# jamie8johnson/cqs

Measured on AMD Instinct MI355X. Metric: queries/sec @k=20 (brute-force cosine scan + top-k, 768-d fp32), higher is better.
Workload: dtype f32; 1 GPU; BASELINE configs[1]: 1000000 x 768 fp32 unit vectors, 1 query per step, brute-force cosine top-20; mode=single, rows_per_gpu=1000000, total_rows=1000000, dim=768, k=20, parallelism=single GPU, ranks_seen=1

## Files before the change

### cqs_amd/csrc/index.hip

```cpp
#include <hip/hip_runtime.h>

#include <algorithm>
#include <atomic>
#include <cmath>
#include <cerrno>
#include <chrono>
#include <cstdio>
#include <cstdlib>
#include <cstring>
#include <mutex>
#include <new>
#include <string>
#include <thread>
#include <vector>

#include <fcntl.h>
#include <libgen.h>
#include <sys/stat.h>
#include <unistd.h>

#include "abi_guard.h"
#include "roctx.h"
#include "index_internal.h"
#include "persist_util.h"
#include "scan_bf16.h"
#include "scan_i8.h"

using cqs::kMaxK;
using cqs::kRowsPerBlock;

namespace cqs_idx {

uint64_t pad_rows(uint64_t n) { return (n + kRowsPerBlock - 1) / kRowsPerBlock * kRowsPerBlock; }

int32_t fail(cqs_hip_index* idx, int32_t code, const char* what, hipError_t e) {
    char buf[512];
    if (e != hipSuccess)
        snprintf(buf, sizeof buf, "%s: %s (%s)", what, hipGetErrorString(e), hipGetErrorName(e));
    else
        snprintf(buf, sizeof buf, "%s", what);
    if (idx) {
        idx->last_error = buf;
        if (code == CQS_HIP_ERR_DEVICE) idx->poisoned.store(true, std::memory_order_release);
    }
    return code;
}

void free_scratch(cqs_hip_index* x) {
    hipFree(x->d_q); hipFree(x->d_scores); hipFree(x->d_gmax); hipFree(x->d_work); hipFree(x->d_gaux);
    x->d_work = nullptr; x->d_gaux = nullptr;
    hipFree(x->d_out_keys); hipFree(x->d_out_counts);
    hipHostFree(x->h_q); hipHostFree(x->h_out_keys); hipHostFree(x->h_out_counts);
    x->d_q = x->d_scores = nullptr; x->d_gmax = nullptr;
    x->d_out_keys = nullptr; x->d_out_counts = nullptr;
    x->h_q = nullptr; x->h_out_keys = nullptr; x->h_out_counts = nullptr;
    x->h_out_keys_dev = nullptr; x->h_out_counts_dev = nullptr;
    x->q_cap = 0; x->k_cap = 0; x->scr_n_pad = 0;
}

int32_t ensure_scratch(cqs_hip_index* x, uint32_t b, uint32_t k) {
    const uint64_t n_pad = pad_rows(x->n);
    if (b <= x->q_cap && k <= x->k_cap && n_pad == x->scr_n_pad) return CQS_HIP_OK;
    HIP_TRY(x, hipDeviceSynchronize());
    uint32_t qc = x->q_cap > b ? x->q_cap : b;
    uint32_t kc = x->k_cap > k ? x->k_cap : k;
    free_scratch(x);
    HIP_TRY(x, hipMalloc(&x->d_q, ((size_t)qc + 256) * x->dim * sizeof(float)));
    HIP_TRY(x, hipMalloc(&x->d_scores, (size_t)qc * n_pad * sizeof(float)));
    HIP_TRY(x, hipMalloc(&x->d_work, cqs::kWorkWords * sizeof(uint32_t)));
    HIP_TRY(x, hipMemset(x->d_work, 0, cqs::kWorkWords * sizeof(uint32_t)));
    HIP_TRY(x, hipMalloc(&x->d_gmax, (size_t)qc * (n_pad / cqs::kTaskRowsSmall) * sizeof(float)));
    HIP_TRY(x, hipMalloc(&x->d_gaux, (size_t)(qc < kGauxQueries ? qc : kGauxQueries) * (n_pad / cqs::kTaskRowsSmall) * sizeof(uint64_t)));
    HIP_TRY(x, hipMalloc(&x->d_out_keys, (size_t)qc * kc * sizeof(uint64_t)));
    HIP_TRY(x, hipMalloc(&x->d_out_counts, (size_t)qc * sizeof(uint32_t)));
    HIP_TRY(x, hipHostMalloc(&x->h_q, (size_t)qc * x->dim * sizeof(float), hipHostMallocDefault));
    HIP_TRY(x, hipHostMalloc(&x->h_out_keys, (size_t)qc * kc * sizeof(uint64_t), hipHostMallocDefault));
    HIP_TRY(x, hipHostMalloc(&x->h_out_counts, (size_t)qc * sizeof(uint32_t), hipHostMallocDefault));
    if (hipHostGetDevicePointer((void**)&x->h_out_keys_dev, x->h_out_keys, 0) != hipSuccess ||
        hipHostGetDevicePointer((void**)&x->h_out_counts_dev, x->h_out_counts, 0) != hipSuccess) {
        (void)hipGetLastError();
        x->h_out_keys_dev = nullptr; x->h_out_counts_dev = nullptr;
    }
    x->q_cap = qc; x->k_cap = kc; x->scr_n_pad = n_pad;
    return CQS_HIP_OK;
}

uint32_t max_query_block(const cqs_hip_index* x) {
    const uint64_t budget = 16ull << 30;
    const uint64_t per_q = pad_rows(x->n) * sizeof(float);
    uint64_t q = per_q ? budget / per_q : 1024;
    if (q < 1) q = 1;
    if (q > 1024) q = 1024;
    return (uint32_t)q;
}

cqs::ScanArgs scan_args(const cqs_hip_index* x, const float* d_q, uint32_t b, uint32_t k, const uint32_t* d_keep,
                        uint32_t mode, float thr, size_t elem_bytes, bool gemv_only, void* dbg, const uint32_t* gate) {
    cqs::ScanArgs a;
    a.rows = x->d_rows;
    a.n = (uint32_t)x->n;
    a.n_pad = (uint32_t)pad_rows(x->n);
    a.dim = x->dim;
    a.q = d_q;
    a.b = b;
    a.scores = x->d_scores;
    a.keep = d_keep;
    a.mode = mode;
    a.threshold = thr;
    a.nontemporal = x->n * x->dim * elem_bytes > kNtBytes;
    a.linear_bins = (x->metric == CQS_HIP_METRIC_COSINE) || (mode == CQS_HIP_MODE_PIPELINE);
    a.k = k;
    a.gmax = x->d_gmax;
    a.gaux = (b <= kGauxQueries && k >= kGauxMinK) ? x->d_gaux : nullptr;
    a.work = x->d_work;
    a.n_cu = x->n_cu;
    a.dbg = dbg;
    a.gemv_only = gemv_only;
    a.tiers = cqs::plan_tiers(a.n_pad, x->n_cu, !gemv_only && cqs::uniform_groups(b, x->dim));
    a.gate = gate;
    return a;
}

int32_t scan_select(cqs_hip_index* x, const cqs::ScanArgs& a, hipStream_t st, const ShadowRows* shadow,
                    uint64_t* out_keys, uint32_t* out_counts) {
    const bool timed = !a.gate && x->timing && x->ev_used + 2 <= kMaxTimingEvents;
    if (timed) {
        while (x->ev.size() < x->ev_used + 2) {
            hipEvent_t e = nullptr;
            HIP_TRY(x, hipEventCreate(&e));
            x->ev.push_back(e);
        }
        HIP_TRY(x, hipEventRecord(x->ev[x->ev_used], st));
    }
    if (shadow && shadow->bf16) HIP_TRY(x, cqs::launch_scan_bf16(a, shadow->bf16, shadow->bq, st));
    else if (shadow) HIP_TRY(x, cqs::launch_scan_i8(a, shadow->i8, shadow->i8_scale, shadow->bq, st));
    else HIP_TRY(x, cqs::launch_scan(a, st));
    if (timed) {
        HIP_TRY(x, hipEventRecord(x->ev[x->ev_used + 1], st));
        x->ev_used += 2;
    }
    if (out_keys) HIP_TRY(x, cqs::launch_select(a, (uint32_t)x->row_base, out_keys, out_counts, st));
    return CQS_HIP_OK;
}

int32_t enqueue_search(cqs_hip_index* x, const float* d_q, uint32_t b, uint32_t k, const uint32_t* d_keep,
                       uint32_t mode, float thr, uint64_t* d_out_keys, uint32_t* d_out_counts, hipStream_t st, bool gemv_only,
                       const uint32_t* gate) {
    HIP_TRY(x, order_after_last(x, st));
    if (!gemv_only && cqs::use_mfma(b, x->dim)) {
        const size_t qbytes = (size_t)b * x->dim * sizeof(float);
        if (d_q != x->d_q) HIP_TRY(x, hipMemcpyAsync(x->d_q, d_q, qbytes, hipMemcpyDeviceToDevice, st));
        HIP_TRY(x, hipMemsetAsync((char*)x->d_q + qbytes, 0, (size_t)256 * x->dim * sizeof(float), st));
        d_q = x->d_q;
    }
    cqs::ScanArgs a = scan_args(x, d_q, b, k, d_keep, mode, thr, sizeof(float), gemv_only, x->d_dbg, gate);
    static const bool use_gaux = [] { const char* e = getenv("CQS_HIP_SELECT_AUX"); return !(e && e[0] == '0'); }();
    if (!use_gaux) a.gaux = nullptr;
    const int32_t rc = scan_select(x, a, st, nullptr, d_out_keys, d_out_counts);
    if (rc == CQS_HIP_OK) HIP_TRY(x, record_done(x, st));
    return rc;
}

hipError_t quiesce(cqs_hip_index* x) {
    hipError_t e = x->stream ? hipStreamSynchronize(x->stream) : hipSuccess;
    if (e == hipSuccess && x->done_valid) e = hipEventSynchronize(x->done);
    return e;
}

int32_t stage_keep(cqs_hip_index* x, const uint32_t* host_words, uint64_t words) {
    if (words > x->keep_words_cap) {
        HIP_TRY(x, quiesce(x));
        hipFree(x->d_keep);
        x->d_keep = nullptr;
        x->keep_words_cap = 0;
        HIP_TRY(x, hipMalloc(&x->d_keep, words * sizeof(uint32_t)));
        x->keep_words_cap = words;
    }
    HIP_TRY(x, hipMemcpyAsync(x->d_keep, host_words, words * sizeof(uint32_t), hipMemcpyHostToDevice, x->stream));
    return CQS_HIP_OK;
}

void read_combine_env(cqs_hip_index* x) {
    if (const char* ce = getenv("CQS_HIP_COMBINE")) x->combine = ce[0] != '0';
    if (const char* cw = getenv("CQS_HIP_COMBINE_WAIT_US")) x->combine_wait_us = (uint32_t)atoi(cw);
    if (const char* cb = getenv("CQS_HIP_COMBINE_BITS")) x->combine_relaxed = cb[0] == 'r';
}

int32_t create_common(uint64_t n, uint32_t dim, uint32_t metric, int32_t device, uint64_t row_base,
                      cqs_hip_index** out, cqs_hip_index** made) {
    if (!out) return CQS_HIP_ERR_INVALID;
    *out = nullptr;
    if (!cqs::scan_dim_supported(dim) || metric > CQS_HIP_METRIC_DOT) return CQS_HIP_ERR_INVALID;
    if (n + row_base > 0xFFFFFFFEull) return CQS_HIP_ERR_INVALID;
    int cnt = 0;
    if (hipGetDeviceCount(&cnt) != hipSuccess || cnt <= 0) return CQS_HIP_ERR_NO_DEVICE;
    if (device < 0 || device >= cnt) return CQS_HIP_ERR_INVALID;
    cqs_hip_index* x = new (std::nothrow) cqs_hip_index();
    if (!x) return CQS_HIP_ERR_NOMEM;
    x->device = device; x->n = n; x->dim = dim; x->metric = metric; x->row_base = row_base;
    if (hipSetDevice(device) != hipSuccess || hipStreamCreateWithFlags(&x->stream, hipStreamNonBlocking) != hipSuccess ||
        hipEventCreateWithFlags(&x->done, hipEventDisableTiming) != hipSuccess) {
        if (x->stream) hipStreamDestroy(x->stream);
        delete x;
        return CQS_HIP_ERR_DEVICE;
    }
    read_combine_env(x);
    if (getenv("CQS_HIP_DEBUG_STAMPS")) {
        const size_t bytes = (16 + 2 * cqs::kDbgWaves) * sizeof(unsigned long long);
        if (hipMalloc(&x->d_dbg, bytes) == hipSuccess) (void)hipMemset(x->d_dbg, 0, bytes);
    }
    hipDeviceProp_t prop;
    if (hipGetDeviceProperties(&prop, device) == hipSuccess && prop.multiProcessorCount > 0)
        x->n_cu = (uint32_t)prop.multiProcessorCount;
    *made = x;
    return CQS_HIP_OK;
}

}

using namespace cqs_idx;

extern "C" {

const char* cqs_hip_version(void) CQS_ABI_TRY { return "cqs-hip 0.1.0 (gfx950)"; } CQS_ABI_CATCH_VAL("cqs-hip")

int32_t cqs_hip_device_count(void) CQS_ABI_TRY {
    int cnt = 0;
    if (hipGetDeviceCount(&cnt) != hipSuccess) return 0;
    return cnt;
} CQS_ABI_CATCH_NOHANDLE

int32_t cqs_hip_device_mem(int32_t device, uint64_t* free_bytes, uint64_t* total_bytes) CQS_ABI_TRY {
    if (hipSetDevice(device) != hipSuccess) return CQS_HIP_ERR_NO_DEVICE;
    size_t f = 0, t = 0;
    if (hipMemGetInfo(&f, &t) != hipSuccess) return CQS_HIP_ERR_DEVICE;
    if (free_bytes) *free_bytes = f;
    if (total_bytes) *total_bytes = t;
    return CQS_HIP_OK;
} CQS_ABI_CATCH_NOHANDLE

}

int32_t cqs_idx::create_owned(const float* rows, uint64_t n, uint32_t dim, uint32_t metric, int32_t device,
                              uint64_t row_base, cqs_hip_index** out) {
    if (n > 0 && !rows) return CQS_HIP_ERR_INVALID;
    cqs_hip_index* x = nullptr;
    int32_t rc = create_common(n, dim, metric, device, row_base, out, &x);
    if (rc != CQS_HIP_OK) return rc;
    x->cap_rows = n ? n : 1;
    hipError_t e = hipMalloc(&x->d_rows, (size_t)x->cap_rows * dim * sizeof(float));
    if (e == hipSuccess && n)
        e = hipMemcpyAsync(x->d_rows, rows, (size_t)n * dim * sizeof(float), hipMemcpyHostToDevice, x->stream);
    if (e == hipSuccess) e = hipStreamSynchronize(x->stream);
    if (e != hipSuccess) {
        cqs_hip_index_destroy(x);
        return e == hipErrorOutOfMemory ? CQS_HIP_ERR_NOMEM : CQS_HIP_ERR_DEVICE;
    }
    *out = x;
    return CQS_HIP_OK;
}

extern "C" {

int32_t cqs_hip_index_create(const float* rows, uint64_t n, uint32_t dim, uint32_t metric, int32_t device,
                             uint64_t row_base, cqs_hip_index** out) CQS_ABI_TRY {
    cqs_hip_index* x = nullptr;
    int32_t rc = create_owned(rows, n, dim, metric, device, row_base, &x);
    if (rc != CQS_HIP_OK) return rc;
    if ((rc = shadow_auto(x)) != CQS_HIP_OK) { cqs_hip_index_destroy(x); return rc; }
    *out = x;
    return CQS_HIP_OK;
} CQS_ABI_CATCH_NOHANDLE

int32_t cqs_hip_index_create_device(const void* d_rows, uint64_t n, uint32_t dim, uint32_t metric, int32_t device,
                                    uint64_t row_base, int32_t borrow, cqs_hip_index** out) CQS_ABI_TRY {
    if (n > 0 && !d_rows) return CQS_HIP_ERR_INVALID;
    if (((uintptr_t)d_rows & 15u) != 0) return CQS_HIP_ERR_INVALID;
    cqs_hip_index* x = nullptr;
    int32_t rc = create_common(n, dim, metric, device, row_base, out, &x);
    if (rc != CQS_HIP_OK) return rc;
    if (n && hipDeviceSynchronize() != hipSuccess) { cqs_hip_index_destroy(x); return CQS_HIP_ERR_DEVICE; }
    if (borrow) {
        x->borrow = true;
        x->d_rows = (float*)d_rows;
        x->cap_rows = n;
    } else {
        x->cap_rows = n ? n : 1;
        hipError_t e = hipMalloc(&x->d_rows, (size_t)x->cap_rows * dim * sizeof(float));
        if (e == hipSuccess && n)
            e = hipMemcpyAsync(x->d_rows, d_rows, (size_t)n * dim * sizeof(float), hipMemcpyDeviceToDevice, x->stream);
        if (e == hipSuccess) e = hipStreamSynchronize(x->stream);
        if (e != hipSuccess) {
            cqs_hip_index_destroy(x);
            return e == hipErrorOutOfMemory ? CQS_HIP_ERR_NOMEM : CQS_HIP_ERR_DEVICE;
        }
    }
    if ((rc = shadow_auto(x)) != CQS_HIP_OK) { cqs_hip_index_destroy(x); return rc; }
    *out = x;
    return CQS_HIP_OK;
} CQS_ABI_CATCH_NOHANDLE

int32_t cqs_hip_index_extend(cqs_hip_index* x, const float* rows, uint64_t n_new) CQS_ABI_TRY {
    if (!x) return CQS_HIP_ERR_INVALID;
    if (x->sh) return cqs_sharded::extend(x, rows, n_new);
    std::lock_guard<std::mutex> g(x->mu);
    if (x->poisoned.load(std::memory_order_acquire)) return CQS_HIP_ERR_POISONED;
    if (x->borrow) return fail(x, CQS_HIP_ERR_INVALID, "extend: index borrows its rows");
    if (n_new == 0) return CQS_HIP_OK;
    if (!rows) return fail(x, CQS_HIP_ERR_INVALID, "extend: null rows");
    if (x->n + n_new + x->row_base > 0xFFFFFFFEull) return fail(x, CQS_HIP_ERR_INVALID, "extend: row id overflow");
    HIP_TRY(x, hipSetDevice(x->device));
    HIP_TRY(x, quiesce(x));
    const size_t row_bytes = (size_t)x->dim * sizeof(float);
    if (x->n + n_new > x->cap_rows) {
        uint64_t cap = x->cap_rows * 2;
        if (cap < x->n + n_new) cap = x->n + n_new;
        float* nd = nullptr;
        HIP_TRY(x, hipMalloc(&nd, cap * row_bytes));
        hipError_t e = hipMemcpyAsync(nd, x->d_rows, x->n * row_bytes, hipMemcpyDeviceToDevice, x->stream);
        if (e == hipSuccess) e = hipStreamSynchronize(x->stream);
        if (e != hipSuccess) {
            hipFree(nd);
            return fail(x, CQS_HIP_ERR_DEVICE, "extend: copy", e);
        }
        hipFree(x->d_rows);
        x->d_rows = nd;
        x->cap_rows = cap;
    }
    HIP_TRY(x, hipMemcpyAsync(x->d_rows + x->n * x->dim, rows, n_new * row_bytes, hipMemcpyHostToDevice, x->stream));
    HIP_TRY(x, hipStreamSynchronize(x->stream));
    const uint64_t n_old = x->n;
    x->n += n_new;
    return shadow_extend(x, n_old);
} CQS_ABI_CATCH(x)

}

namespace {
using cqs_persist::Checksum;
using cqs_persist::exists;
using cqs_persist::fsync_parent;
using cqs_persist::read_all;
using cqs_persist::write_all;

struct FlatHeader {
    char magic[8];
    uint32_t version, dim, metric, pad;
    uint64_t rows, checksum;
    uint8_t reserved[24];
};
static_assert(sizeof(FlatHeader) == 64, "header is 64 bytes");
const char kFlatMagic[8] = {'C', 'Q', 'S', 'H', 'I', 'P', 'F', '1'};

constexpr size_t kIoPiece = 64ull << 20;

struct Piece { const cqs_idx::Segment* seg; size_t off, len; };
std::vector<Piece> cut_pieces(const std::vector<cqs_idx::Segment>& segs, uint32_t dim) {
    std::vector<Piece> out;
    for (const cqs_idx::Segment& sg : segs) {
        const size_t bytes = (size_t)sg.rows * dim * sizeof(float);
        for (size_t off = 0; off < bytes; off += kIoPiece) out.push_back({&sg, off, bytes - off < kIoPiece ? bytes - off : kIoPiece});
    }
    return out;
}
struct PinPair {
    uint8_t* p[2] = {nullptr, nullptr};
    hipError_t alloc(size_t bytes) {
        for (int i = 0; i < 2; ++i) {
            hipError_t e = hipHostMalloc((void**)&p[i], bytes ? bytes : 8, hipHostMallocPortable);
            if (e != hipSuccess) return e;
        }
        return hipSuccess;
    }
    ~PinPair() { if (p[0]) hipHostFree(p[0]); if (p[1]) hipHostFree(p[1]); }
};
}

namespace cqs_idx {

int32_t save_segments(cqs_hip_index* x, const std::vector<Segment>& segs, uint32_t dim, uint32_t metric, const char* path,
                      uint64_t* out_checksum) {
    const std::string live(path), bak = live + ".bak", tmp = live + ".tmp";
    if (exists(bak)) return fail(x, CQS_HIP_ERR_INVALID, "save: stale .bak from a prior failed save; manual recovery required");
    uint64_t rows = 0;
    for (const Segment& sg : segs) rows += sg.rows;
    const size_t bytes = (size_t)rows * dim * sizeof(float);
    const std::vector<Piece> pieces = cut_pieces(segs, dim);
    PinPair pin;
    hipError_t he = pin.alloc(bytes < kIoPiece ? bytes : kIoPiece);
    if (he != hipSuccess) return fail(x, CQS_HIP_ERR_NOMEM, "save: pinned staging", he);
    const int fd = open(tmp.c_str(), O_WRONLY | O_CREAT | O_TRUNC, 0644);
    if (fd < 0) return fail(x, CQS_HIP_ERR_INVALID, "save: cannot create temp file");
    FlatHeader h{};
    memcpy(h.magic, kFlatMagic, 8);
    h.version = 1; h.dim = dim; h.metric = metric; h.rows = rows;
    bool ok = write_all(fd, &h, sizeof h);
    Checksum ck(bytes);
    auto issue = [&](size_t i) -> hipError_t {
        const Piece& pc = pieces[i];
        hipError_t e = hipSetDevice(pc.seg->device);
        if (e != hipSuccess) return e;
        return hipMemcpyAsync(pin.p[i & 1], (const uint8_t*)pc.seg->d_rows + pc.off, pc.len, hipMemcpyDeviceToHost, pc.seg->stream);
    };
    if (ok && !pieces.empty()) he = issue(0);
    for (size_t i = 0; ok && he == hipSuccess && i < pieces.size(); ++i) {
        he = hipStreamSynchronize(pieces[i].seg->stream);
        if (he != hipSuccess) break;
        if (i + 1 < pieces.size() && (he = issue(i + 1)) != hipSuccess) break;
        ck.update(pin.p[i & 1], pieces[i].len, i + 1 == pieces.size());
        ok = write_all(fd, pin.p[i & 1], pieces[i].len);
    }
    if (pieces.empty()) ck.update(nullptr, 0, true);
    for (const Segment& sg : segs) (void)hipStreamSynchronize(sg.stream);
    h.checksum = ck.finish();
    ok = ok && he == hipSuccess && lseek(fd, 0, SEEK_SET) == 0 && write_all(fd, &h, sizeof h) && fsync(fd) == 0;
    close(fd);
    if (!ok) {
        unlink(tmp.c_str());
        return he != hipSuccess ? fail(x, CQS_HIP_ERR_DEVICE, "save: device copy", he) : fail(x, CQS_HIP_ERR_INVALID, "save: write failed");
    }
    const bool backed_up = exists(live);
    if (backed_up) {
        if (rename(live.c_str(), bak.c_str()) != 0) { unlink(tmp.c_str()); return fail(x, CQS_HIP_ERR_INVALID, "save: cannot back up the live blob"); }
        fsync_parent(live);
    }
    if (rename(tmp.c_str(), live.c_str()) != 0) {
        unlink(tmp.c_str());
        if (backed_up) {
            if (rename(bak.c_str(), live.c_str()) != 0) return fail(x, CQS_HIP_ERR_INVALID, "save failed and rollback failed: rename .bak back by hand");
            fsync_parent(live);
        }
        return fail(x, CQS_HIP_ERR_INVALID, "save: rename failed");
    }
    if (backed_up) unlink(bak.c_str());
    fsync_parent(live);
    if (out_checksum) *out_checksum = h.checksum;
    return CQS_HIP_OK;
}

int32_t open_blob(const char* path, uint32_t expected_dim, uint64_t expected_rows, int* fd_out, uint64_t* rows,
                  uint32_t* metric, uint64_t* checksum) {
    const int fd = open(path, O_RDONLY);
    if (fd < 0) return CQS_HIP_ERR_INVALID;
    FlatHeader h{};
    struct stat st;
    const bool ok = read_all(fd, &h, sizeof h) && memcmp(h.magic, kFlatMagic, 8) == 0 && h.version == 1 &&
                    h.dim == expected_dim && (expected_rows == 0 || h.rows == expected_rows) && h.metric <= CQS_HIP_METRIC_DOT &&
                    fstat(fd, &st) == 0 && h.dim != 0 && h.rows <= (UINT64_MAX - sizeof h) / ((uint64_t)h.dim * 4u) &&
                    (uint64_t)st.st_size == sizeof h + h.rows * h.dim * 4u;
    if (!ok) { close(fd); return CQS_HIP_ERR_INVALID; }
    *fd_out = fd; *rows = h.rows; *metric = h.metric; *checksum = h.checksum;
    return CQS_HIP_OK;
}

int32_t read_blob_into(int fd, uint64_t checksum, uint32_t dim, const std::vector<Segment>& segs) {
    uint64_t rows = 0;
    for (const Segment& sg : segs) rows += sg.rows;
    const size_t bytes = (size_t)rows * dim * sizeof(float);
    const std::vector<Piece> pieces = cut_pieces(segs, dim);
    PinPair pin;
    hipError_t he = pin.alloc(bytes < kIoPiece ? bytes : kIoPiece);
    Checksum ck(bytes);
    bool ok = true;
    for (size_t i = 0; ok && he == hipSuccess && i < pieces.size(); ++i) {
        const Piece& pc = pieces[i];
        if (i >= 2) he = hipStreamSynchronize(pieces[i - 2].seg->stream);
        if (he != hipSuccess) break;
        ok = read_all(fd, pin.p[i & 1], pc.len);
        if (!ok) break;
        ck.update(pin.p[i & 1], pc.len, i + 1 == pieces.size());
        he = hipSetDevice(pc.seg->device);
        if (he == hipSuccess) he = hipMemcpyAsync((uint8_t*)pc.seg->d_rows + pc.off, pin.p[i & 1], pc.len, hipMemcpyHostToDevice, pc.seg->stream);
    }
    if (pieces.empty()) ck.update(nullptr, 0, true);
    for (const Segment& sg : segs) {
        const hipError_t hs = hipStreamSynchronize(sg.stream);
        if (he == hipSuccess) he = hs;
    }
    close(fd);
    if (he != hipSuccess) return he == hipErrorOutOfMemory ? CQS_HIP_ERR_NOMEM : CQS_HIP_ERR_DEVICE;
    return ok && ck.finish() == checksum ? CQS_HIP_OK : CQS_HIP_ERR_INVALID;
}

}

extern "C" {

int32_t cqs_hip_index_save(cqs_hip_index* x, const char* path, uint64_t* out_checksum) CQS_ABI_TRY {
    if (!x || !path) return CQS_HIP_ERR_INVALID;
    if (x->sh) return cqs_sharded::save(x, path, out_checksum);
    std::lock_guard<std::mutex> g(x->mu);
    if (x->poisoned.load(std::memory_order_acquire)) return CQS_HIP_ERR_POISONED;
    HIP_TRY(x, hipSetDevice(x->device));
    HIP_TRY(x, quiesce(x));
    return save_segments(x, {Segment{x->device, x->d_rows, x->n, x->stream}}, x->dim, x->metric, path, out_checksum);
} CQS_ABI_CATCH(x)

int32_t cqs_hip_index_load(const char* path, uint32_t expected_dim, uint64_t expected_rows, int32_t device,
                           uint64_t row_base, cqs_hip_index** out) CQS_ABI_TRY {
    if (!path || !out) return CQS_HIP_ERR_INVALID;
    *out = nullptr;
    int fd = -1;
    uint64_t rows = 0, checksum = 0;
    uint32_t metric = 0;
    int32_t rc = open_blob(path, expected_dim, expected_rows, &fd, &rows, &metric, &checksum);
    if (rc != CQS_HIP_OK) return rc;
    cqs_hip_index* x = nullptr;
    rc = create_common(rows, expected_dim, metric, device, row_base, out, &x);
    if (rc != CQS_HIP_OK) { close(fd); return rc; }
    x->cap_rows = rows ? rows : 1;
    if (hipMalloc(&x->d_rows, (size_t)x->cap_rows * expected_dim * sizeof(float)) != hipSuccess) {
        close(fd);
        cqs_hip_index_destroy(x);
        return CQS_HIP_ERR_NOMEM;
    }
    rc = read_blob_into(fd, checksum, expected_dim, {Segment{device, x->d_rows, rows, x->stream}});
    if (rc == CQS_HIP_OK) rc = shadow_auto(x);
    if (rc != CQS_HIP_OK) { cqs_hip_index_destroy(x); return rc; }
    *out = x;
    return CQS_HIP_OK;
} CQS_ABI_CATCH_NOHANDLE

void cqs_hip_index_destroy(cqs_hip_index* x) CQS_ABI_TRY {
    if (!x) return;
    if (x->sh) { cqs_sharded::destroy(x); return; }
    hipSetDevice(x->device);
    (void)quiesce(x);
    free_scratch(x);
    shadow_free(x);
    hipFree(x->d_keep);
    hipFree(x->d_dbg);
    if (!x->borrow) hipFree(x->d_rows);
    for (hipEvent_t e : x->ev) hipEventDestroy(e);
    if (x->done) hipEventDestroy(x->done);
    if (x->stream) hipStreamDestroy(x->stream);
    delete x;
} CQS_ABI_CATCH_VOID

uint64_t cqs_hip_index_len(const cqs_hip_index* x) CQS_ABI_TRY { return x ? (x->sh ? cqs_sharded::len(x) : x->n) : 0; } CQS_ABI_CATCH_VAL(0)
uint32_t cqs_hip_index_dim(const cqs_hip_index* x) CQS_ABI_TRY { return x ? x->dim : 0; } CQS_ABI_CATCH_VAL(0)
uint32_t cqs_hip_index_metric(const cqs_hip_index* x) CQS_ABI_TRY { return x ? x->metric : 0; } CQS_ABI_CATCH_VAL(0)
uint32_t cqs_hip_index_max_k(const cqs_hip_index* x) CQS_ABI_TRY { (void)x; return kMaxK; } CQS_ABI_CATCH_VAL(0)
int32_t cqs_hip_index_poisoned(const cqs_hip_index* x) CQS_ABI_TRY {
    if (x && x->sh) return cqs_sharded::poisoned(x);
    return x && x->poisoned.load(std::memory_order_acquire) ? 1 : 0;
} CQS_ABI_CATCH_NOHANDLE
int32_t cqs_hip_index_device(const cqs_hip_index* x) CQS_ABI_TRY { return x ? x->device : -1; } CQS_ABI_CATCH_NOHANDLE
uint64_t cqs_hip_index_row_base(const cqs_hip_index* x) CQS_ABI_TRY { return x ? x->row_base : 0; } CQS_ABI_CATCH_VAL(0)

size_t cqs_hip_index_last_error(const cqs_hip_index* x, char* buf, size_t cap) CQS_ABI_TRY {
    if (!x || !buf || cap == 0) return 0;
    if (x->sh) return cqs_sharded::last_error(x, buf, cap);
    std::lock_guard<std::mutex> g(x->mu);
    size_t m = x->last_error.size() < cap - 1 ? x->last_error.size() : cap - 1;
    memcpy(buf, x->last_error.data(), m);
    buf[m] = 0;
    return m;
} CQS_ABI_CATCH_VAL(0)

void cqs_hip_unpack_keys(const uint64_t* keys, size_t count, uint64_t* rows, float* scores) CQS_ABI_TRY {
    for (size_t i = 0; i < count; ++i) {
        const uint32_t ok = (uint32_t)(keys[i] >> 32);
        const uint32_t bits = (ok & 0x80000000u) ? (ok ^ 0x80000000u) : ~ok;
        float f;
        memcpy(&f, &bits, 4);
        if (scores) scores[i] = f;
        if (rows) rows[i] = (uint64_t)(0xFFFFFFFFu - (uint32_t)keys[i]);
    }
} CQS_ABI_CATCH_VOID

size_t cqs_hip_merge_keys(const uint64_t* lists, const uint32_t* counts, size_t n_lists, size_t stride, size_t k,
                          uint64_t* out_keys) CQS_ABI_TRY {
    std::vector<size_t> pos(n_lists, 0);
    size_t outc = 0;
    while (outc < k) {
        size_t best = n_lists;
        uint64_t bk = 0;
        for (size_t l = 0; l < n_lists; ++l) {
            if (pos[l] < counts[l]) {
                const uint64_t v = lists[l * stride + pos[l]];
                if (best == n_lists || v > bk) { best = l; bk = v; }
            }
        }
        if (best == n_lists) break;
        out_keys[outc++] = bk;
        pos[best]++;
    }
    return outc;
} CQS_ABI_CATCH_VAL(0)

int32_t cqs_hip_index_search_device(cqs_hip_index* x, const float* d_queries, uint32_t b, uint32_t k,
                                    const uint32_t* d_keep_bitset, uint32_t mode, float threshold,
                                    uint64_t* d_out_keys, uint32_t* d_out_counts, void* stream) CQS_ABI_TRY {
    CQS_ROCTX_RANGE("cqs_hip_index_search_device");
    if (!x) return CQS_HIP_ERR_INVALID;
    if (x->sh) return CQS_HIP_ERR_INVALID;
    std::lock_guard<std::mutex> g(x->mu);
    if (x->poisoned.load(std::memory_order_acquire)) return CQS_HIP_ERR_POISONED;
    if (b == 0) return CQS_HIP_OK;
    if (!d_queries || !d_out_keys || !d_out_counts) return fail(x, CQS_HIP_ERR_INVALID, "search_device: null buffer");
    if (k == 0 || k > kMaxK) return fail(x, CQS_HIP_ERR_INVALID, "search_device: k out of range");
    if (mode > CQS_HIP_MODE_PIPELINE) return fail(x, CQS_HIP_ERR_INVALID, "search_device: bad mode");
    if (b > max_query_block(x)) return fail(x, CQS_HIP_ERR_INVALID, "search_device: batch exceeds scratch budget");
    HIP_TRY(x, hipSetDevice(x->device));
    hipStream_t st = (hipStream_t)stream;
    if (x->n == 0) {
        HIP_TRY(x, hipMemsetAsync(d_out_counts, 0, (size_t)b * sizeof(uint32_t), st));
        return CQS_HIP_OK;
    }
    int32_t rc = ensure_scratch(x, b, k);
    if (rc != CQS_HIP_OK) return rc;
    const uint32_t* gate = nullptr;
    if (shadow_takes(x, b, k, false) &&
        (rc = shadow_pass(x, d_queries, b, k, d_keep_bitset, mode, threshold, d_out_keys, d_out_counts, st, &gate)) != CQS_HIP_OK)
        return rc;
    return enqueue_search(x, d_queries, b, k, d_keep_bitset, mode, threshold, d_out_keys, d_out_counts, st, false, gate);
} CQS_ABI_CATCH(x)

}

namespace cqs_idx {

static void print_debug_stamps(cqs_hip_index* x) {
    unsigned long long h[16];
    if (hipMemcpy(h, x->d_dbg, sizeof h, hipMemcpyDeviceToHost) == hipSuccess)
        fprintf(stderr, "[cqs_hip] select_finish us: zero %.2f hist %.2f decide %.2f groups %.2f scores %.2f sort %.2f emit %.2f | groups=%llu cand=%llu\n",
                0.0, (h[1] - h[0]) / 100.0, (h[2] - h[1]) / 100.0, (h[3] - h[2]) / 100.0, (h[4] - h[3]) / 100.0,
                (h[5] - h[4]) / 100.0, (h[6] - h[5]) / 100.0, h[8], h[9]);
    std::vector<unsigned long long> w(2 * cqs::kDbgWaves);
    if (hipMemcpy(w.data(), x->d_dbg + 16, w.size() * sizeof(unsigned long long), hipMemcpyDeviceToHost) != hipSuccess) return;
    std::vector<double> st, en;
    unsigned long long t0 = ~0ull;
    for (uint32_t i = 0; i < cqs::kDbgWaves; ++i) if (w[2 * i] && w[2 * i] < t0) t0 = w[2 * i];
    for (uint32_t i = 0; i < cqs::kDbgWaves; ++i)
        if (w[2 * i] && w[2 * i + 1]) { st.push_back((w[2 * i] - t0) / 100.0); en.push_back((w[2 * i + 1] - t0) / 100.0); }
    if (!st.empty()) {
        std::sort(st.begin(), st.end());
        std::sort(en.begin(), en.end());
        auto pc = [](const std::vector<double>& v, double f) { return v[(size_t)(f * (v.size() - 1))]; };
        fprintf(stderr, "[cqs_hip] scan waves=%zu start us p0 %.1f p50 %.1f p90 %.1f p100 %.1f | end us p0 %.1f p10 %.1f p50 %.1f p90 %.1f p100 %.1f | select ends %.1f\n",
                st.size(), pc(st, 0), pc(st, .5), pc(st, .9), pc(st, 1), pc(en, 0), pc(en, .1), pc(en, .5), pc(en, .9), pc(en, 1),
                (h[6] - t0) / 100.0);
    }
    (void)hipMemset(x->d_dbg + 16, 0, w.size() * sizeof(unsigned long long));
}

static int32_t host_block(cqs_hip_index* x, const cqs_combine_req* const* qs, uint32_t nq, uint32_t k, const uint32_t* d_keep,
                          uint32_t mode, float thr, bool gemv_only, std::vector<const cqs_combine_req*>* redo) {
    HIP_TRY(x, hipMemcpyAsync(x->d_q, x->h_q, (size_t)nq * x->dim * sizeof(float), hipMemcpyHostToDevice, x->stream));
    const bool direct = x->h_out_keys_dev && x->h_out_counts_dev && (size_t)nq * k <= kDirectOutKeys;
    uint64_t* const keys = direct ? x->h_out_keys_dev : x->d_out_keys;
    uint32_t* const counts = direct ? x->h_out_counts_dev : x->d_out_counts;
    int32_t rc = redo ? shadow_pass(x, x->d_q, nq, k, d_keep, mode, thr, keys, counts, x->stream, nullptr)
                      : enqueue_search(x, x->d_q, nq, k, d_keep, mode, thr, keys, counts, x->stream, gemv_only);
    if (rc != CQS_HIP_OK) return rc;
    if (redo) HIP_TRY(x, record_done(x, x->stream));
    if (!direct) {
        HIP_TRY(x, hipMemcpyAsync(x->h_out_keys, x->d_out_keys, (size_t)nq * k * sizeof(uint64_t), hipMemcpyDeviceToHost, x->stream));
        HIP_TRY(x, hipMemcpyAsync(x->h_out_counts, x->d_out_counts, (size_t)nq * sizeof(uint32_t), hipMemcpyDeviceToHost, x->stream));
    }
    const uint32_t* cert = nullptr;
    if (redo) HIP_TRY(x, shadow_verdicts(x, nq, &cert));
    HIP_TRY(x, hipStreamSynchronize(x->stream));
    if (!redo && x->d_dbg) print_debug_stamps(x);
    if (redo) redo->clear();
    uint64_t certified = 0;
    for (uint32_t i = 0; i < nq; ++i) {
        if (!qs[i]) continue;
        if (cert && !cert[i]) {
            if (redo->size() != i) memcpy(x->h_q + redo->size() * x->dim, x->h_q + (size_t)i * x->dim, (size_t)x->dim * sizeof(float));
            redo->push_back(qs[i]);
            continue;
        }
        const uint32_t c = x->h_out_counts[i] < k ? x->h_out_counts[i] : k;
        cqs_hip_unpack_keys(x->h_out_keys + (size_t)i * k, c, qs[i]->out_rows, qs[i]->out_scores);
        *qs[i]->out_count = c;
        certified += cert ? 1 : 0;
    }
    x->stat_certified.fetch_add(certified, std::memory_order_relaxed);
    if (redo) x->stat_fallbacks.fetch_add(redo->size(), std::memory_order_relaxed);
    if (redo && shadow_uses_i8(x, nq, k)) {
        x->stat_i8_certified.fetch_add(certified, std::memory_order_relaxed);
        x->stat_i8_fallbacks.fetch_add(redo->size(), std::memory_order_relaxed);
    }
    return CQS_HIP_OK;
}

static int32_t search_host_locked(cqs_hip_index* x, const cqs_combine_req* qs, uint32_t b, uint32_t k, const uint32_t* keep_bitset,
                                  uint32_t mode, float threshold, bool gemv_only) {
    if (x->inject_fail.exchange(0, std::memory_order_acq_rel) != 0)
        return fail(x, CQS_HIP_ERR_DEVICE, "search: injected device failure (test hook)");
    if (x->n == 0 || k == 0) return CQS_HIP_OK;
    HIP_TRY(x, hipSetDevice(x->device));
    HIP_TRY(x, order_after_last(x, x->stream));
    const uint32_t* d_keep = nullptr;
    uint32_t k_eff = k;
    if (keep_bitset) {
        const uint64_t words = (x->n + 31) / 32;
        uint64_t included = 0;
        for (uint64_t w = 0; w < words; ++w) {
            uint32_t v = keep_bitset[w];
            if (w == words - 1 && (x->n % 32)) v &= (1u << (x->n % 32)) - 1u;
            included += (uint64_t)__builtin_popcount(v);
        }
        if (included == 0) return CQS_HIP_OK;
        if (included < x->n) {
            if (included < k_eff) k_eff = (uint32_t)included;
            int32_t rck = stage_keep(x, keep_bitset, words);
            if (rck != CQS_HIP_OK) return rck;
            d_keep = x->d_keep;
        }
    }

    const uint32_t blk = max_query_block(x);
    std::vector<const cqs_combine_req*> staged, redo;
    for (uint32_t done = 0; done < b;) {
        const uint32_t nb = (b - done) < blk ? (b - done) : blk;
        int32_t rc = ensure_scratch(x, nb, k_eff);
        if (rc != CQS_HIP_OK) return rc;
        staged.clear();
        for (uint32_t i = 0; i < nb; ++i) {
            const float* src = qs[done + i].q;
            float* dst = x->h_q + (size_t)i * x->dim;
            bool ok = true;
            for (uint32_t d = 0; d < x->dim; ++d) ok &= std::isfinite(src[d]);
            if (ok) memcpy(dst, src, (size_t)x->dim * sizeof(float));
            else memset(dst, 0, (size_t)x->dim * sizeof(float));
            staged.push_back(ok ? &qs[done + i] : nullptr);
        }
        if (shadow_takes(x, nb, k_eff, gemv_only)) {
            if ((rc = host_block(x, staged.data(), nb, k_eff, d_keep, mode, threshold, gemv_only, &redo)) != CQS_HIP_OK) return rc;
            staged.swap(redo);
        }
        if (!staged.empty() &&
            (rc = host_block(x, staged.data(), (uint32_t)staged.size(), k_eff, d_keep, mode, threshold, gemv_only, nullptr)) != CQS_HIP_OK)
            return rc;
        done += nb;
    }
    return CQS_HIP_OK;
}

constexpr uint32_t kCombineCap = 32;

static bool same_params(const cqs_combine_req* a, const cqs_combine_req* b) {
    return a->k == b->k && a->mode == b->mode && memcmp(&a->thr, &b->thr, sizeof(float)) == 0;
}
static uint32_t count_like_front(const cqs_hip_index* x) {
    uint32_t n = 0;
    for (const cqs_combine_req* r : x->pending) n += same_params(r, x->pending.front()) ? 1u : 0u;
    return n;
}

static int32_t combine_run_single(cqs_hip_index* x, cqs_combine_req* const* batch, uint32_t nb) {
    std::lock_guard<std::mutex> dev(x->mu);
    if (x->poisoned.load(std::memory_order_acquire)) return CQS_HIP_ERR_POISONED;
    cqs_combine_req rq[kCombineCap];
    for (uint32_t i = 0; i < nb; ++i) rq[i] = *batch[i];
    const bool gemv_only = !(x->combine_relaxed && nb >= cqs::kMfmaMinQueries);
    return search_host_locked(x, rq, nb, batch[0]->k, nullptr, batch[0]->mode, batch[0]->thr, gemv_only);
}

static void combine_lead(cqs_hip_index* x, std::unique_lock<std::mutex>& lk) {
    const uint32_t target = x->expect < kCombineCap ? x->expect : kCombineCap;
    if (x->combine_wait_us && count_like_front(x) < target) {
        const auto t_end = x->last_pass_end + std::chrono::microseconds(x->combine_wait_us);
        while (count_like_front(x) < target && std::chrono::steady_clock::now() < t_end) {
            lk.unlock();
            for (int i = 0; i < 64; ++i) __builtin_ia32_pause();
            lk.lock();
        }
    }
    cqs_combine_req* batch[kCombineCap];
    uint32_t nb = 0, left_like = 0;
    {
        const cqs_combine_req head = *x->pending.front();
        std::deque<cqs_combine_req*> keep;
        for (cqs_combine_req* r : x->pending) {
            if (same_params(r, &head)) {
                if (nb < kCombineCap) { batch[nb++] = r; continue; }
                ++left_like;
            }
            keep.push_back(r);
        }
        x->pending.swap(keep);
        x->n_pending.store((uint32_t)x->pending.size(), std::memory_order_relaxed);
    }
    x->expect = nb + left_like;
    lk.unlock();

    int32_t rc = CQS_HIP_OK;
    try {
        rc = x->sh ? cqs_sharded::search_combined(x, batch, nb) : combine_run_single(x, batch, nb);
    } catch (const std::bad_alloc&) {
        rc = fail(x, CQS_HIP_ERR_NOMEM, "search: out of host memory");
    } catch (...) {
        rc = fail(x, CQS_HIP_ERR_INVALID, "search: unexpected C++ exception");
    }
    x->stat_passes.fetch_add(1, std::memory_order_relaxed);
    x->stat_queries.fetch_add(nb, std::memory_order_relaxed);
    const bool poisoned = x->sh ? cqs_sharded::poisoned(x) != 0 : x->poisoned.load(std::memory_order_acquire);

    lk.lock();
    x->last_pass_end = std::chrono::steady_clock::now();
    for (uint32_t i = 0; i < nb; ++i) {
        batch[i]->rc = (rc != CQS_HIP_OK && i > 0 && poisoned) ? CQS_HIP_ERR_POISONED : rc;
        batch[i]->done = true;
    }
    if (poisoned) {
        for (cqs_combine_req* r : x->pending) { r->rc = CQS_HIP_ERR_POISONED; r->done = true; }
        x->pending.clear();
        x->n_pending.store(0, std::memory_order_relaxed);
    } else if (!x->pending.empty()) {
        uint32_t like = 0;
        for (const cqs_combine_req* r : x->pending) like += same_params(r, batch[0]) ? 1u : 0u;
        if (nb + like > x->expect) x->expect = nb + like;
    }
}

static int32_t combine_search(cqs_hip_index* x, cqs_combine_req& r) {
    std::unique_lock<std::mutex> lk(x->cmu);
    x->pending.push_back(&r);
    x->n_pending.store((uint32_t)x->pending.size(), std::memory_order_relaxed);
    while (!r.done) {
        if (!x->leader) {
            x->leader = true;
            struct Reset {
                cqs_hip_index* x; std::unique_lock<std::mutex>& lk;
                ~Reset() { if (!lk.owns_lock()) lk.lock(); x->leader = false; x->ccv.notify_all(); }
            } reset{x, lk};
            combine_lead(x, lk);
        } else {
            x->ccv.wait(lk);
        }
    }
    return r.rc;
}

}

extern "C" {

int32_t cqs_hip_index_search(cqs_hip_index* x, const float* queries, uint32_t b, uint32_t query_dim, uint32_t k,
                             const uint32_t* keep_bitset, uint32_t mode, float threshold, uint64_t* out_rows,
                             float* out_scores, uint32_t* out_counts) CQS_ABI_TRY {
    CQS_ROCTX_RANGE("cqs_hip_index_search");
    if (!x) return CQS_HIP_ERR_INVALID;
    if (x->combine && b == 1 && !keep_bitset && queries && out_counts && out_rows && out_scores && query_dim == x->dim &&
        k >= 1 && k <= kMaxK && mode <= CQS_HIP_MODE_PIPELINE) {
        if (x->sh ? cqs_sharded::poisoned(x) != 0 : x->poisoned.load(std::memory_order_acquire))
            return CQS_HIP_ERR_POISONED;
        out_counts[0] = 0;
        bool finite = true;
        for (uint32_t d = 0; d < query_dim; ++d) finite &= std::isfinite(queries[d]);
        if (!finite) return CQS_HIP_OK;
        cqs_combine_req r{queries, k, mode, threshold, out_rows, out_scores, out_counts};
        return combine_search(x, r);
    }
    if (x->sh) return cqs_sharded::search(x, queries, b, query_dim, k, keep_bitset, mode, threshold, out_rows, out_scores, out_counts);
    std::lock_guard<std::mutex> g(x->mu);
    if (x->poisoned.load(std::memory_order_acquire)) return CQS_HIP_ERR_POISONED;
    if (b == 0) return CQS_HIP_OK;
    if (!queries || !out_counts) return fail(x, CQS_HIP_ERR_INVALID, "search: null buffer");
    for (uint32_t i = 0; i < b; ++i) out_counts[i] = 0;
    if (x->n == 0 || k == 0) return CQS_HIP_OK;
    if (query_dim != x->dim) {
        x->last_error = "search: query dimension mismatch (empty result)";
        return CQS_HIP_OK;
    }
    if (k > kMaxK) return fail(x, CQS_HIP_ERR_INVALID, "search: k > max_k");
    if (mode > CQS_HIP_MODE_PIPELINE) return fail(x, CQS_HIP_ERR_INVALID, "search: bad mode");
    if (!out_rows || !out_scores) return fail(x, CQS_HIP_ERR_INVALID, "search: null output buffer");
    std::vector<cqs_combine_req> rq(b);
    for (uint32_t i = 0; i < b; ++i)
        rq[i] = cqs_combine_req{queries + (size_t)i * x->dim, k, mode, threshold, out_rows + (size_t)i * k, out_scores + (size_t)i * k, out_counts + i};
    return search_host_locked(x, rq.data(), b, k, keep_bitset, mode, threshold, false);
} CQS_ABI_CATCH(x)

void cqs_hip_index_combine_stats(const cqs_hip_index* x, uint64_t* passes, uint64_t* queries) CQS_ABI_TRY {
    if (passes) *passes = x ? x->stat_passes.load(std::memory_order_relaxed) : 0;
    if (queries) *queries = x ? x->stat_queries.load(std::memory_order_relaxed) : 0;
} CQS_ABI_CATCH_VOID

int32_t cqs_hip_index_neighbors(cqs_hip_index* x, uint64_t target_row, uint32_t limit, uint64_t* out_rows,
                                float* out_scores, uint32_t* out_count) CQS_ABI_TRY {
    CQS_ROCTX_RANGE("cqs_hip_index_neighbors");
    if (!x || !out_count) return CQS_HIP_ERR_INVALID;
    if (x->sh) return cqs_sharded::neighbors(x, target_row, limit, out_rows, out_scores, out_count);
    std::lock_guard<std::mutex> g(x->mu);
    *out_count = 0;
    if (x->poisoned.load(std::memory_order_acquire)) return CQS_HIP_ERR_POISONED;
    if (!out_rows || !out_scores) return fail(x, CQS_HIP_ERR_INVALID, "neighbors: null output buffer");
    if (target_row < x->row_base || target_row - x->row_base >= x->n)
        return fail(x, CQS_HIP_ERR_INVALID, "neighbors: target row not in this index");
    if (limit < 1u) limit = 1u;
    if (limit > CQS_HIP_NEIGHBORS_MAX) limit = CQS_HIP_NEIGHBORS_MAX;
    if (x->n <= 1) return CQS_HIP_OK;
    const uint32_t k = (uint64_t)limit + 1u < x->n ? limit + 1u : (uint32_t)x->n;
    HIP_TRY(x, hipSetDevice(x->device));
    HIP_TRY(x, order_after_last(x, x->stream));
    int32_t rc = ensure_scratch(x, 1, k);
    if (rc != CQS_HIP_OK) return rc;
    const float* d_target = x->d_rows + (size_t)(target_row - x->row_base) * x->dim;
    rc = enqueue_search(x, d_target, 1, k, nullptr, CQS_HIP_MODE_RAW, 0.f, x->d_out_keys, x->d_out_counts, x->stream);
    if (rc != CQS_HIP_OK) return rc;
    HIP_TRY(x, hipMemcpyAsync(x->h_out_keys, x->d_out_keys, (size_t)k * sizeof(uint64_t), hipMemcpyDeviceToHost, x->stream));
    HIP_TRY(x, hipMemcpyAsync(x->h_out_counts, x->d_out_counts, sizeof(uint32_t), hipMemcpyDeviceToHost, x->stream));
    HIP_TRY(x, hipStreamSynchronize(x->stream));
    uint32_t c = x->h_out_counts[0] < k ? x->h_out_counts[0] : k, outc = 0;
    for (uint32_t i = 0; i < c && outc < limit; ++i) {
        uint64_t row;
        float score;
        cqs_hip_unpack_keys(x->h_out_keys + i, 1, &row, &score);
        if (row == target_row) continue;
        out_rows[outc] = row;
        out_scores[outc] = score;
        ++outc;
    }
    *out_count = outc;
    return CQS_HIP_OK;
} CQS_ABI_CATCH(x)

void cqs_hip_index_set_timing(cqs_hip_index* x, int32_t enable) CQS_ABI_TRY {
    if (!x) return;
    if (x->sh) { cqs_sharded::set_timing(x, enable); return; }
    std::lock_guard<std::mutex> g(x->mu);
    x->timing = enable != 0;
    x->ev_used = 0;
} CQS_ABI_CATCH_VOID

int32_t cqs_hip_index_scan_time(cqs_hip_index* x, uint32_t* launches, double* total_ms) CQS_ABI_TRY {
    if (!x || !launches || !total_ms) return CQS_HIP_ERR_INVALID;
    if (x->sh) return cqs_sharded::scan_time(x, launches, total_ms);
    std::lock_guard<std::mutex> g(x->mu);
    *launches = 0;
    *total_ms = 0.0;
    HIP_TRY(x, hipSetDevice(x->device));
    for (size_t i = 0; i + 1 < x->ev_used; i += 2) {
        HIP_TRY(x, hipEventSynchronize(x->ev[i + 1]));
        float ms = 0.f;
        HIP_TRY(x, hipEventElapsedTime(&ms, x->ev[i], x->ev[i + 1]));
        *total_ms += ms;
        *launches += 1;
    }
    x->ev_used = 0;
    return CQS_HIP_OK;
} CQS_ABI_CATCH(x)


void cqs_hip_debug_index_fail_next(cqs_hip_index* x) CQS_ABI_TRY {
    if (x) x->inject_fail.store(1, std::memory_order_release);
} CQS_ABI_CATCH_VOID

double cqs_hip_debug_client_storm(cqs_hip_index* x, const float* queries, uint32_t n_queries, uint32_t dim, uint32_t k,
                                  uint32_t n_threads, uint32_t per_thread, uint64_t* out_rows, float* out_scores,
                                  uint32_t* out_counts) CQS_ABI_TRY {
    if (!x || !queries || !n_queries || !n_threads || !out_rows || !out_scores || !out_counts) return -1.0;
    std::atomic<int32_t> bad{0};
    std::atomic<uint32_t> ready{0};
    std::atomic<bool> go{false};
    std::vector<std::thread> th;
    th.reserve(n_threads);
    for (uint32_t t = 0; t < n_threads; ++t)
        th.emplace_back([&, t]() {
            ready.fetch_add(1);
            while (!go.load(std::memory_order_acquire)) std::this_thread::yield();
            uint32_t qi = t % n_queries;
            for (uint32_t i = 0; i < per_thread; ++i) {
                const int32_t rc = cqs_hip_index_search(x, queries + (size_t)qi * dim, 1, dim, k, nullptr, CQS_HIP_MODE_RAW, 0.f,
                                                        out_rows + (size_t)qi * k, out_scores + (size_t)qi * k, out_counts + qi);
                if (rc != CQS_HIP_OK) { bad.store(rc); break; }
                qi = (qi + n_threads) % n_queries;
            }
        });
    while (ready.load() < n_threads) std::this_thread::yield();
    const auto t0 = std::chrono::steady_clock::now();
    go.store(true, std::memory_order_release);
    for (std::thread& t : th) t.join();
    const double el = std::chrono::duration<double>(std::chrono::steady_clock::now() - t0).count();
    return bad.load() ? -1.0 : el;
} CQS_ABI_CATCH_VAL(-1.0)

}
```

### cqs_amd/csrc/index_internal.h

```cpp
#pragma once
#include <hip/hip_runtime.h>

#include <atomic>
#include <chrono>
#include <condition_variable>
#include <deque>
#include <mutex>
#include <string>
#include <vector>

#include "../../include/cqs_hip.h"
#include "scan_kernels.h"

namespace cqs_sharded { struct ShardSet; }
namespace cqs_idx { struct Shadow; }

struct cqs_combine_req {
    const float* q;
    uint32_t k, mode;
    float thr;
    uint64_t* out_rows;
    float* out_scores;
    uint32_t* out_count;
    int32_t rc = 0;
    bool done = false;
};

struct cqs_hip_index {
    int device = 0;
    uint64_t n = 0;
    uint64_t cap_rows = 0;
    uint32_t dim = 0;
    uint32_t metric = 0;
    uint64_t row_base = 0;
    bool borrow = false;
    float* d_rows = nullptr;
    hipStream_t stream = nullptr;

    uint32_t q_cap = 0;
    uint64_t scr_n_pad = 0;
    uint32_t k_cap = 0;
    float* d_q = nullptr;
    float* d_scores = nullptr;
    uint32_t* d_work = nullptr;
    unsigned long long* d_dbg = nullptr;
    uint32_t n_cu = 256;
    float* d_gmax = nullptr;
    uint64_t* d_gaux = nullptr;
    uint64_t* d_out_keys = nullptr;
    uint32_t* d_out_counts = nullptr;
    uint32_t* d_keep = nullptr;
    uint64_t keep_words_cap = 0;
    float* h_q = nullptr;
    uint64_t* h_out_keys = nullptr;
    uint32_t* h_out_counts = nullptr;
    uint64_t* h_out_keys_dev = nullptr;
    uint32_t* h_out_counts_dev = nullptr;

    hipEvent_t done = nullptr;
    hipStream_t done_stream = nullptr;
    bool done_valid = false;

    bool timing = false;
    std::vector<hipEvent_t> ev;
    size_t ev_used = 0;

    cqs_sharded::ShardSet* sh = nullptr;

    mutable std::mutex mu;
    std::atomic<bool> poisoned{false};
    std::string last_error;

    std::mutex cmu;
    std::condition_variable ccv;
    std::deque<cqs_combine_req*> pending;
    std::atomic<uint32_t> n_pending{0};
    bool leader = false;
    uint32_t expect = 1;
    bool combine = true;
    bool combine_relaxed = false;
    uint32_t combine_wait_us = 100;
    std::chrono::steady_clock::time_point last_pass_end{};
    std::atomic<uint64_t> stat_passes{0}, stat_queries{0};
    std::atomic<int32_t> inject_fail{0};

    cqs_idx::Shadow* shadow = nullptr;
    std::atomic<uint64_t> stat_certified{0}, stat_fallbacks{0};
    std::atomic<uint64_t> stat_i8_certified{0}, stat_i8_fallbacks{0};
};

namespace cqs_idx {

constexpr size_t kMaxTimingEvents = 8192;
constexpr uint64_t kNtBytes = 200ull << 20;
constexpr uint32_t kGauxQueries = 32;
constexpr uint32_t kGauxMinK = 100;
constexpr size_t kDirectOutKeys = 8192;

uint64_t pad_rows(uint64_t n);
int32_t fail(cqs_hip_index* idx, int32_t code, const char* what, hipError_t e = hipSuccess);
void free_scratch(cqs_hip_index* x);
int32_t ensure_scratch(cqs_hip_index* x, uint32_t b, uint32_t k);
uint32_t max_query_block(const cqs_hip_index* x);
cqs::ScanArgs scan_args(const cqs_hip_index* x, const float* d_q, uint32_t b, uint32_t k, const uint32_t* d_keep,
                        uint32_t mode, float thr, size_t elem_bytes, bool gemv_only, void* dbg, const uint32_t* gate);
struct ShadowRows { const uint16_t* bf16; const int8_t* i8; const float* i8_scale; const float* bq; };
int32_t scan_select(cqs_hip_index* x, const cqs::ScanArgs& a, hipStream_t st, const ShadowRows* shadow,
                    uint64_t* out_keys, uint32_t* out_counts);
inline hipError_t order_after_last(cqs_hip_index* x, hipStream_t st) {
    return x->done_valid && x->done_stream != st ? hipStreamWaitEvent(st, x->done, 0) : hipSuccess;
}
inline hipError_t record_done(cqs_hip_index* x, hipStream_t st) {
    const hipError_t e = hipEventRecord(x->done, st);
    if (e == hipSuccess) { x->done_stream = st; x->done_valid = true; }
    return e;
}
int32_t enqueue_search(cqs_hip_index* x, const float* d_q, uint32_t b, uint32_t k, const uint32_t* d_keep,
                       uint32_t mode, float thr, uint64_t* d_out_keys, uint32_t* d_out_counts, hipStream_t st,
                       bool gemv_only = false, const uint32_t* gate = nullptr);
hipError_t quiesce(cqs_hip_index* x);
int32_t create_owned(const float* rows, uint64_t n, uint32_t dim, uint32_t metric, int32_t device, uint64_t row_base,
                     cqs_hip_index** out);
int32_t stage_keep(cqs_hip_index* x, const uint32_t* host_words, uint64_t words);
int32_t create_common(uint64_t n, uint32_t dim, uint32_t metric, int32_t device, uint64_t row_base,
                      cqs_hip_index** out, cqs_hip_index** made);
void read_combine_env(cqs_hip_index* x);
int32_t shadow_auto(cqs_hip_index* x);
int32_t shadow_extend(cqs_hip_index* x, uint64_t n_old);
void shadow_free(cqs_hip_index* x);
bool shadow_takes(const cqs_hip_index* x, uint32_t b, uint32_t k, bool gemv_only);
bool shadow_uses_i8(const cqs_hip_index* x, uint32_t b, uint32_t k);
int32_t shadow_pass(cqs_hip_index* x, const float* d_q, uint32_t nb, uint32_t k, const uint32_t* d_keep, uint32_t mode,
                    float thr, uint64_t* out_keys, uint32_t* out_counts, hipStream_t st, const uint32_t** device_gate);
hipError_t shadow_verdicts(cqs_hip_index* x, uint32_t nb, const uint32_t** h_cert);

struct Segment { int device; float* d_rows; uint64_t rows; hipStream_t stream; };
int32_t save_segments(cqs_hip_index* err_owner, const std::vector<Segment>& segs, uint32_t dim, uint32_t metric,
                      const char* path, uint64_t* out_checksum);
int32_t open_blob(const char* path, uint32_t expected_dim, uint64_t expected_rows, int* fd_out, uint64_t* rows,
                  uint32_t* metric, uint64_t* checksum);
int32_t read_blob_into(int fd, uint64_t checksum, uint32_t dim, const std::vector<Segment>& segs);

}

namespace cqs_sharded {
void destroy(cqs_hip_index* parent);
int32_t search(cqs_hip_index* parent, const float* queries, uint32_t b, uint32_t query_dim, uint32_t k,
               const uint32_t* keep_bitset, uint32_t mode, float threshold, uint64_t* out_rows, float* out_scores,
               uint32_t* out_counts);
int32_t search_combined(cqs_hip_index* parent, cqs_combine_req* const* batch, uint32_t nb);
int32_t neighbors(cqs_hip_index* parent, uint64_t target_row, uint32_t limit, uint64_t* out_rows, float* out_scores,
                  uint32_t* out_count);
int32_t extend(cqs_hip_index* parent, const float* rows, uint64_t n_new);
int32_t save(cqs_hip_index* parent, const char* path, uint64_t* out_checksum);
uint64_t len(const cqs_hip_index* parent);
int32_t poisoned(const cqs_hip_index* parent);
size_t last_error(const cqs_hip_index* parent, char* buf, size_t cap);
void set_timing(cqs_hip_index* parent, int32_t enable);
int32_t scan_time(cqs_hip_index* parent, uint32_t* launches, double* total_ms);
}

#define HIP_TRY(idx, expr)                                                        \
    do {                                                                          \
        hipError_t _e = (expr);                                                   \
        if (_e != hipSuccess)                                                     \
            return cqs_idx::fail((idx), _e == hipErrorOutOfMemory ? CQS_HIP_ERR_NOMEM : CQS_HIP_ERR_DEVICE, #expr, _e); \
    } while (0)
```

### cqs_amd/csrc/index_shadow.hip

```cpp
#include <cstdlib>
#include <cstring>
#include <new>

#include "abi_guard.h"
#include "index_internal.h"
#include "scan_bf16.h"
#include "scan_i8.h"

namespace cqs_idx {

constexpr uint64_t kShadowAutoBytes = 1ull << 30;
constexpr uint64_t kShadowFreeMinBytes = 4ull << 30;
constexpr double kShadowFreeFrac = 0.10;
constexpr uint32_t kStatWords = 10, kStatCounts = 3, kStatI8 = 5, kStatI8Counts = 8;

struct Shadow {
    uint16_t* d_bf16 = nullptr;
    uint64_t cap = 0;
    int8_t* d_i8 = nullptr;
    float* d_i8_scale = nullptr;
    double r8 = 0.0, norm8 = 0.0;
    double r = 0.0;
    double norm = 0.0;
    unsigned long long* d_stats = nullptr;
    uint64_t* d_ekeys = nullptr;
    uint32_t* d_cert = nullptr;
    float* d_bq = nullptr;
    uint32_t* d_tickets = nullptr;
    uint32_t* h_cert = nullptr;
    uint32_t* h_cert_dev = nullptr;
};

static void shadow_device_counts(cqs_hip_index* x, uint32_t first, uint64_t* certified, uint64_t* fallbacks) {
    unsigned long long c[2];
    if (!x->shadow || !x->shadow->d_stats || quiesce(x) != hipSuccess) return;
    hipError_t e = hipMemcpyAsync(c, x->shadow->d_stats + first, sizeof c, hipMemcpyDeviceToHost, x->stream);
    if (e == hipSuccess) e = hipStreamSynchronize(x->stream);
    if (e != hipSuccess) { (void)hipGetLastError(); return; }
    *certified += c[0];
    *fallbacks += c[1];
}

static void i8_free(Shadow* s) {
    hipFree(s->d_i8); hipFree(s->d_i8_scale);
    s->d_i8 = nullptr; s->d_i8_scale = nullptr;
}

void shadow_free(cqs_hip_index* x) {
    Shadow* s = x->shadow;
    if (!s) return;
    uint64_t c = 0, f = 0;
    shadow_device_counts(x, kStatCounts, &c, &f);
    x->stat_certified.fetch_add(c, std::memory_order_relaxed);
    x->stat_fallbacks.fetch_add(f, std::memory_order_relaxed);
    c = f = 0;
    shadow_device_counts(x, kStatI8Counts, &c, &f);
    x->stat_i8_certified.fetch_add(c, std::memory_order_relaxed);
    x->stat_i8_fallbacks.fetch_add(f, std::memory_order_relaxed);
    i8_free(s);
    hipFree(s->d_bf16); hipFree(s->d_stats); hipFree(s->d_ekeys);
    hipFree(s->d_cert); hipFree(s->d_bq); hipFree(s->d_tickets); hipHostFree(s->h_cert);
    delete s;
    x->shadow = nullptr;
}

static int32_t shadow_convert(cqs_hip_index* x, uint64_t row0, bool* outlier) {
    Shadow* s = x->shadow;
    HIP_TRY(x, hipMemsetAsync(s->d_stats + 2, 0, sizeof(unsigned long long), x->stream));
    HIP_TRY(x, cqs::launch_shadow_build(x->d_rows, s->d_bf16, row0, x->n - row0, x->dim, cqs::shadow_gamma(x->dim),
                                        s->d_stats, x->stream));
    unsigned long long st[3];
    HIP_TRY(x, hipMemcpyAsync(st, s->d_stats, sizeof st, hipMemcpyDeviceToHost, x->stream));
    HIP_TRY(x, hipStreamSynchronize(x->stream));
    double r, m;
    memcpy(&r, &st[0], sizeof r);
    memcpy(&m, &st[1], sizeof m);
    s->r = r * (1.0 + 0x1p-30);
    s->norm = m * (1.0 + 0x1p-30);
    *outlier = st[2] != 0;
    return CQS_HIP_OK;
}

static int32_t i8_convert(cqs_hip_index* x, uint64_t row0) {
    Shadow* s = x->shadow;
    HIP_TRY(x, cqs::launch_i8_build(x->d_rows, s->d_i8, s->d_i8_scale, row0, x->n - row0, x->dim, cqs::i8_gamma(x->dim),
                                    s->d_stats + kStatI8, x->stream));
    unsigned long long st[2];
    HIP_TRY(x, hipMemcpyAsync(st, s->d_stats + kStatI8, sizeof st, hipMemcpyDeviceToHost, x->stream));
    HIP_TRY(x, hipStreamSynchronize(x->stream));
    double r, m;
    memcpy(&r, &st[0], sizeof r);
    memcpy(&m, &st[1], sizeof m);
    s->r8 = r * (1.0 + 0x1p-30);
    s->norm8 = m * (1.0 + 0x1p-30);
    return CQS_HIP_OK;
}

static uint64_t i8_bytes(uint64_t cap, uint32_t dim) { return cap * dim + cap * sizeof(float); }

static int32_t i8_enable(cqs_hip_index* x, bool* built) {
    Shadow* s = x->shadow;
    *built = false;
    if (hipMalloc(&s->d_i8, (size_t)s->cap * x->dim) != hipSuccess ||
        hipMalloc(&s->d_i8_scale, (size_t)s->cap * sizeof(float)) != hipSuccess) {
        (void)hipGetLastError();
        i8_free(s);
        return CQS_HIP_OK;
    }
    const int32_t rc = i8_convert(x, 0);
    if (rc != CQS_HIP_OK) { i8_free(s); return rc; }
    *built = true;
    return CQS_HIP_OK;
}

int32_t shadow_extend(cqs_hip_index* x, uint64_t n_old) {
    Shadow* s = x->shadow;
    if (!s) return CQS_HIP_OK;
    if (x->cap_rows > s->cap) {
        uint16_t* nd = nullptr;
        if (hipMalloc(&nd, (size_t)x->cap_rows * x->dim * sizeof(uint16_t)) != hipSuccess) {
            (void)hipGetLastError();
            shadow_free(x);
            x->last_error = "extend: no device memory to grow the bf16 shadow; shadow turned off";
            return CQS_HIP_OK;
        }
        hipError_t e = hipMemcpyAsync(nd, s->d_bf16, (size_t)n_old * x->dim * sizeof(uint16_t), hipMemcpyDeviceToDevice, x->stream);
        if (e == hipSuccess) e = hipStreamSynchronize(x->stream);
        if (e != hipSuccess) { hipFree(nd); return fail(x, CQS_HIP_ERR_DEVICE, "extend: shadow copy", e); }
        hipFree(s->d_bf16);
        s->d_bf16 = nd;
        if (s->d_i8) {
            int8_t* n8 = nullptr;
            float* ns = nullptr;
            if (hipMalloc(&n8, (size_t)x->cap_rows * x->dim) != hipSuccess || hipMalloc(&ns, (size_t)x->cap_rows * sizeof(float)) != hipSuccess) {
                (void)hipGetLastError();
                hipFree(n8);
                i8_free(s);
                x->last_error = "extend: no device memory to grow the int8 copy of the shadow; int8 copy turned off";
            } else {
                e = hipMemcpyAsync(n8, s->d_i8, (size_t)n_old * x->dim, hipMemcpyDeviceToDevice, x->stream);
                if (e == hipSuccess) e = hipMemcpyAsync(ns, s->d_i8_scale, (size_t)n_old * sizeof(float), hipMemcpyDeviceToDevice, x->stream);
                if (e == hipSuccess) e = hipStreamSynchronize(x->stream);
                if (e != hipSuccess) { hipFree(n8); hipFree(ns); return fail(x, CQS_HIP_ERR_DEVICE, "extend: int8 copy", e); }
                i8_free(s);
                s->d_i8 = n8;
                s->d_i8_scale = ns;
            }
        }
        s->cap = x->cap_rows;
    }
    bool outlier = false;
    int32_t rc = shadow_convert(x, n_old, &outlier);
    if (rc == CQS_HIP_OK && s->d_i8 && !outlier) rc = i8_convert(x, n_old);
    if (rc != CQS_HIP_OK) return rc;
    if (outlier) {
        shadow_free(x);
        x->last_error = "extend: a new row has a component of magnitude >= 2^64; bf16 shadow turned off";
    }
    return CQS_HIP_OK;
}

static bool dim_ok(uint32_t dim) { return dim % 8u == 0u && dim <= cqs::kShadowMaxDim; }
static const char* const kDimRule = ": dim must be a multiple of 8 and <= 2048";

static int32_t shadow_enable(cqs_hip_index* x, const char* what) {
    std::string pre(what);
    if (!dim_ok(x->dim)) return fail(x, CQS_HIP_ERR_INVALID, (pre + kDimRule).c_str());
    if (x->shadow) return CQS_HIP_OK;
    auto oom = [&](hipError_t e) { (void)hipGetLastError(); shadow_free(x); return fail(x, CQS_HIP_ERR_NOMEM, (pre + ": allocation").c_str(), e); };
    Shadow* s = x->shadow = new (std::nothrow) Shadow();
    if (!s) return oom(hipErrorOutOfMemory);
    const uint64_t cap = x->cap_rows ? x->cap_rows : 1;
    hipError_t e;
    if ((e = hipMalloc(&s->d_bf16, (size_t)cap * x->dim * sizeof(uint16_t))) != hipSuccess) return oom(e);
    s->cap = cap;
    unsigned long long* stats = nullptr;
    if ((e = hipMalloc(&stats, kStatWords * sizeof(unsigned long long))) != hipSuccess) return oom(e);
    if ((e = hipMemsetAsync(stats, 0, kStatWords * sizeof(unsigned long long), x->stream)) != hipSuccess) { hipFree(stats); return oom(e); }
    s->d_stats = stats;
    if ((e = hipMalloc(&s->d_ekeys, (size_t)cqs::kShadowMaxQ * (cqs::kMaxK - 1) * sizeof(uint64_t))) != hipSuccess) return oom(e);
    if ((e = hipMalloc(&s->d_cert, (size_t)cqs::kShadowMaxQ * sizeof(uint32_t))) != hipSuccess) return oom(e);
    if ((e = hipMalloc(&s->d_bq, (size_t)cqs::kShadowMaxQ * sizeof(float))) != hipSuccess) return oom(e);
    if ((e = hipMalloc(&s->d_tickets, (size_t)cqs::kShadowMaxQ * sizeof(uint32_t))) != hipSuccess) return oom(e);
    if ((e = hipMemsetAsync(s->d_tickets, 0, (size_t)cqs::kShadowMaxQ * sizeof(uint32_t), x->stream)) != hipSuccess) return oom(e);
    if ((e = hipHostMalloc(&s->h_cert, (size_t)cqs::kShadowMaxQ * sizeof(uint32_t), hipHostMallocDefault)) != hipSuccess) return oom(e);
    if (hipHostGetDevicePointer((void**)&s->h_cert_dev, s->h_cert, 0) != hipSuccess) {
        (void)hipGetLastError();
        s->h_cert_dev = nullptr;
    }
    bool outlier = false;
    const int32_t rc = shadow_convert(x, 0, &outlier);
    if (rc != CQS_HIP_OK) { shadow_free(x); return rc; }
    if (outlier) {
        shadow_free(x);
        return fail(x, CQS_HIP_ERR_INVALID, (pre + ": a finite row has a component of magnitude >= 2^64").c_str());
    }
    return CQS_HIP_OK;
}

static bool i8_dim_ok(uint32_t dim) { return cqs::i8_dim_ok(dim); }
static const char* const kI8DimRule = ": dim must be a multiple of 16 and <= 2048";
static int32_t i8_auto(cqs_hip_index* x) {
    Shadow* s = x->shadow;
    if (!s || s->d_i8) return CQS_HIP_OK;
    const char* env = getenv("CQS_HIP_SCAN_I8");
    if (env && env[0] == '0') return CQS_HIP_OK;
    if (!(env && env[0] == '1') && x->n * x->dim * sizeof(float) < kShadowAutoBytes) return CQS_HIP_OK;
    const std::string pre("int8 copy of the shadow not built (the bf16 copy serves every block)");
    if (!i8_dim_ok(x->dim)) { x->last_error = pre + kI8DimRule; return CQS_HIP_OK; }
    size_t free_b = 0, total_b = 0;
    if (hipMemGetInfo(&free_b, &total_b) != hipSuccess) {
        (void)hipGetLastError();
        x->last_error = pre + ": hipMemGetInfo failed";
        return CQS_HIP_OK;
    }
    const uint64_t need = i8_bytes(s->cap, x->dim);
    const uint64_t frac = (uint64_t)(kShadowFreeFrac * (double)total_b);
    const uint64_t reserve = frac > kShadowFreeMinBytes ? frac : kShadowFreeMinBytes;
    bool built = false;
    if (free_b >= need && free_b - need >= reserve) {
        const int32_t rc = i8_enable(x, &built);
        if (rc != CQS_HIP_OK) return rc;
    }
    if (!built) x->last_error = pre + ": the device would keep less than max(4 GiB, 10 %) of its memory free with both copies";
    return CQS_HIP_OK;
}

int32_t shadow_auto(cqs_hip_index* x) {
    const char* env = getenv("CQS_HIP_SCAN_BF16");
    if (env && env[0] == '0') return CQS_HIP_OK;
    const bool any_size = env && env[0] == '1';
    const uint64_t f32_bytes = x->n * x->dim * sizeof(float);
    if (!any_size && f32_bytes < kShadowAutoBytes) {
        x->last_error = "bf16 shadow not built: f32 corpus below 1 GiB (CQS_HIP_SCAN_BF16=1 builds it at any size)";
        return CQS_HIP_OK;
    }
    if (!dim_ok(x->dim)) {
        x->last_error = std::string("bf16 shadow not built") + kDimRule;
        return CQS_HIP_OK;
    }
    size_t free_b = 0, total_b = 0;
    if (hipMemGetInfo(&free_b, &total_b) != hipSuccess) {
        (void)hipGetLastError();
        x->last_error = "bf16 shadow not built: hipMemGetInfo failed";
        return CQS_HIP_OK;
    }
    const uint64_t cap = x->cap_rows ? x->cap_rows : 1;
    const uint64_t need = cap * x->dim * sizeof(uint16_t) + (cqs::kMaxK + 2ull) * cqs::kShadowMaxQ * sizeof(uint64_t);
    const uint64_t frac = (uint64_t)(kShadowFreeFrac * (double)total_b);
    const uint64_t reserve = frac > kShadowFreeMinBytes ? frac : kShadowFreeMinBytes;
    if (free_b < need || free_b - need < reserve) {
        x->last_error = "bf16 shadow not built: the device would keep less than max(4 GiB, 10 %) of its memory free";
        return CQS_HIP_OK;
    }
    int32_t rc = shadow_enable(x, "bf16 shadow not built");
    if (rc == CQS_HIP_OK) rc = i8_auto(x);
    return rc == CQS_HIP_ERR_DEVICE ? rc : CQS_HIP_OK;
}

bool shadow_takes(const cqs_hip_index* x, uint32_t b, uint32_t k, bool gemv_only) {
    return x->shadow && b <= cqs::kShadowMaxQ && (gemv_only || !cqs::use_mfma(b, x->dim)) && cqs::shadow_kprime(k) >= k;
}

bool shadow_uses_i8(const cqs_hip_index* x, uint32_t b, uint32_t k) {
    return x->shadow && x->shadow->d_i8 && b <= cqs::kI8MaxQ && cqs::i8_k_ok(k);
}

int32_t shadow_pass(cqs_hip_index* x, const float* d_q, uint32_t nb, uint32_t k, const uint32_t* d_keep, uint32_t mode,
                    float threshold, uint64_t* out_keys, uint32_t* out_counts, hipStream_t st, const uint32_t** device_gate) {
    const Shadow* s = x->shadow;
    uint32_t* const cert = device_gate || !s->h_cert_dev ? s->d_cert : s->h_cert_dev;
    if (device_gate) *device_gate = cert;
    if (device_gate) HIP_TRY(x, order_after_last(x, st));
    const bool i8 = shadow_uses_i8(x, nb, k);
    const uint32_t kp = i8 ? cqs::i8_kprime(k) : cqs::shadow_kprime(k);
    const double r_max = i8 ? s->r8 : s->r, norm_max = i8 ? s->norm8 : s->norm;
    const bool bound_first = mode == CQS_HIP_MODE_PIPELINE;
    if (bound_first) {
        if (i8) HIP_TRY(x, cqs::launch_i8_bound(d_q, nb, x->dim, r_max, norm_max, s->d_bq, st));
        else HIP_TRY(x, cqs::launch_shadow_bound(d_q, nb, x->dim, r_max, norm_max, s->d_bq, st));
    }
    const cqs::ScanArgs a = scan_args(x, d_q, nb, kp + 1u, d_keep, mode, threshold, i8 ? sizeof(int8_t) : sizeof(uint16_t), true, nullptr, nullptr);
    const ShadowRows rows{i8 ? nullptr : s->d_bf16, i8 ? s->d_i8 : nullptr, s->d_i8_scale, s->d_bq};
    const int32_t rc = scan_select(x, a, st, &rows, nullptr, nullptr);
    if (rc == CQS_HIP_OK)
        HIP_TRY(x, cqs::launch_rescore_certify(a, (uint32_t)x->row_base, k, kp, bound_first ? 0u : (i8 ? 2u : 1u), r_max, norm_max,
                                               s->d_bq, s->d_tickets, s->d_ekeys, out_keys, out_counts, cert,
                                               device_gate ? s->d_stats + kStatCounts : nullptr,
                                               device_gate && i8 ? s->d_stats + kStatI8Counts : nullptr, st));
    return rc;
}

hipError_t shadow_verdicts(cqs_hip_index* x, uint32_t nb, const uint32_t** h_cert) {
    const Shadow* s = x->shadow;
    *h_cert = s->h_cert;
    return s->h_cert_dev ? hipSuccess : hipMemcpyAsync(s->h_cert, s->d_cert, (size_t)nb * sizeof(uint32_t), hipMemcpyDeviceToHost, x->stream);
}

}

using namespace cqs_idx;

extern "C" {

int32_t cqs_hip_index_set_bf16_scan(cqs_hip_index* x, int32_t enable) CQS_ABI_TRY {
    if (!x || x->sh) return CQS_HIP_ERR_INVALID;
    std::lock_guard<std::mutex> g(x->mu);
    if (x->poisoned.load(std::memory_order_acquire)) return CQS_HIP_ERR_POISONED;
    HIP_TRY(x, hipSetDevice(x->device));
    HIP_TRY(x, quiesce(x));
    if (!enable) { shadow_free(x); return CQS_HIP_OK; }
    if (x->borrow) return fail(x, CQS_HIP_ERR_INVALID, "set_bf16_scan: index borrows its rows (they may change under the bound)");
    const int32_t rc = shadow_enable(x, "set_bf16_scan");
    return rc == CQS_HIP_OK ? i8_auto(x) : rc;
} CQS_ABI_CATCH(x)

void cqs_hip_index_bf16_stats(const cqs_hip_index* x, uint64_t* bytes, uint64_t* certified, uint64_t* fallbacks) CQS_ABI_TRY {
    uint64_t by = 0, c = 0, f = 0;
    if (x && !x->sh) {
        cqs_hip_index* m = const_cast<cqs_hip_index*>(x);
        std::lock_guard<std::mutex> g(m->mu);
        by = m->shadow ? m->shadow->cap * m->dim * sizeof(uint16_t) : 0;
        c = m->stat_certified.load(std::memory_order_relaxed);
        f = m->stat_fallbacks.load(std::memory_order_relaxed);
        if (m->shadow && hipSetDevice(m->device) == hipSuccess) shadow_device_counts(m, kStatCounts, &c, &f);
    }
    if (bytes) *bytes = by;
    if (certified) *certified = c;
    if (fallbacks) *fallbacks = f;
} CQS_ABI_CATCH_VOID

void cqs_hip_index_i8_stats(const cqs_hip_index* x, uint64_t* bytes, uint64_t* certified, uint64_t* fallbacks) CQS_ABI_TRY {
    uint64_t by = 0, c = 0, f = 0;
    if (x && !x->sh) {
        cqs_hip_index* m = const_cast<cqs_hip_index*>(x);
        std::lock_guard<std::mutex> g(m->mu);
        by = m->shadow && m->shadow->d_i8 ? i8_bytes(m->shadow->cap, m->dim) : 0;
        c = m->stat_i8_certified.load(std::memory_order_relaxed);
        f = m->stat_i8_fallbacks.load(std::memory_order_relaxed);
        if (m->shadow && hipSetDevice(m->device) == hipSuccess) shadow_device_counts(m, kStatI8Counts, &c, &f);
    }
    if (bytes) *bytes = by;
    if (certified) *certified = c;
    if (fallbacks) *fallbacks = f;
} CQS_ABI_CATCH_VOID

int32_t cqs_hip_debug_shadow_bound(cqs_hip_index* x, const float* queries, uint32_t b, float* out_device, float* out_host) CQS_ABI_TRY {
    if (!x || x->sh || !queries || !out_device || !out_host || b == 0) return CQS_HIP_ERR_INVALID;
    std::lock_guard<std::mutex> g(x->mu);
    const Shadow* s = x->shadow;
    if (!s || b > cqs::kShadowMaxQ) return CQS_HIP_ERR_INVALID;
    HIP_TRY(x, hipSetDevice(x->device));
    HIP_TRY(x, quiesce(x));
    float* d_q = nullptr;
    HIP_TRY(x, hipMalloc(&d_q, (size_t)b * x->dim * sizeof(float)));
    hipError_t e = hipMemcpyAsync(d_q, queries, (size_t)b * x->dim * sizeof(float), hipMemcpyHostToDevice, x->stream);
    if (e == hipSuccess) e = cqs::launch_shadow_bound(d_q, b, x->dim, s->r, s->norm, s->d_bq, x->stream);
    if (e == hipSuccess) e = hipMemcpyAsync(out_device, s->d_bq, (size_t)b * sizeof(float), hipMemcpyDeviceToHost, x->stream);
    if (e == hipSuccess) e = hipStreamSynchronize(x->stream);
    hipFree(d_q);
    HIP_TRY(x, e);
    for (uint32_t i = 0; i < b; ++i) {
        const float* q = queries + (size_t)i * x->dim;
        double s2 = 0.0;
        for (uint32_t d = 0; d < x->dim; ++d) s2 += (double)q[d] * (double)q[d];
        out_host[i] = cqs::shadow_query_bound(s2, s->r, s->norm, x->dim);
    }
    return CQS_HIP_OK;
} CQS_ABI_CATCH(x)

int32_t cqs_hip_debug_shadow_bound_i8(cqs_hip_index* x, const float* queries, uint32_t b, float* out_device, float* out_host) CQS_ABI_TRY {
    if (!x || x->sh || !queries || !out_device || !out_host || b == 0) return CQS_HIP_ERR_INVALID;
    std::lock_guard<std::mutex> g(x->mu);
    const Shadow* s = x->shadow;
    if (!s || !s->d_i8 || b > cqs::kShadowMaxQ) return CQS_HIP_ERR_INVALID;
    HIP_TRY(x, hipSetDevice(x->device));
    HIP_TRY(x, quiesce(x));
    float* d_q = nullptr;
    HIP_TRY(x, hipMalloc(&d_q, (size_t)b * x->dim * sizeof(float)));
    hipError_t e = hipMemcpyAsync(d_q, queries, (size_t)b * x->dim * sizeof(float), hipMemcpyHostToDevice, x->stream);
    if (e == hipSuccess) e = cqs::launch_i8_bound(d_q, b, x->dim, s->r8, s->norm8, s->d_bq, x->stream);
    if (e == hipSuccess) e = hipMemcpyAsync(out_device, s->d_bq, (size_t)b * sizeof(float), hipMemcpyDeviceToHost, x->stream);
    if (e == hipSuccess) e = hipStreamSynchronize(x->stream);
    hipFree(d_q);
    HIP_TRY(x, e);
    for (uint32_t i = 0; i < b; ++i) {
        const float* q = queries + (size_t)i * x->dim;
        double s2 = 0.0;
        for (uint32_t d = 0; d < x->dim; ++d) s2 += (double)q[d] * (double)q[d];
        out_host[i] = cqs::i8_query_bound(s2, s->r8, s->norm8, x->dim);
    }
    return CQS_HIP_OK;
} CQS_ABI_CATCH(x)

int32_t cqs_hip_debug_shadow_bq(cqs_hip_index* x, uint32_t b, float* out) CQS_ABI_TRY {
    if (!x || x->sh || !out || b == 0) return CQS_HIP_ERR_INVALID;
    std::lock_guard<std::mutex> g(x->mu);
    const Shadow* s = x->shadow;
    if (!s || b > cqs::kShadowMaxQ) return CQS_HIP_ERR_INVALID;
    HIP_TRY(x, hipSetDevice(x->device));
    HIP_TRY(x, quiesce(x));
    HIP_TRY(x, hipMemcpyAsync(out, s->d_bq, (size_t)b * sizeof(float), hipMemcpyDeviceToHost, x->stream));
    HIP_TRY(x, hipStreamSynchronize(x->stream));
    return CQS_HIP_OK;
} CQS_ABI_CATCH(x)

int32_t cqs_hip_debug_shadow_stats(cqs_hip_index* x, double* out) CQS_ABI_TRY {
    if (!x || x->sh || !out) return CQS_HIP_ERR_INVALID;
    std::lock_guard<std::mutex> g(x->mu);
    const Shadow* s = x->shadow;
    if (!s) return CQS_HIP_ERR_INVALID;
    out[0] = s->r; out[1] = s->norm;
    out[2] = s->d_i8 ? s->r8 : 0.0; out[3] = s->d_i8 ? s->norm8 : 0.0;
    return CQS_HIP_OK;
} CQS_ABI_CATCH(x)

int32_t cqs_hip_debug_shadow_rows(cqs_hip_index* x, uint32_t copy, uint64_t row0, uint64_t rows, void* out, float* out_scales) CQS_ABI_TRY {
    if (!x || x->sh || !out || (copy != 1u && copy != 2u) || (copy == 2u && !out_scales)) return CQS_HIP_ERR_INVALID;
    std::lock_guard<std::mutex> g(x->mu);
    const Shadow* s = x->shadow;
    if (!s || (copy == 2u && !s->d_i8) || row0 > x->n || rows > x->n - row0) return CQS_HIP_ERR_INVALID;
    if (rows == 0) return CQS_HIP_OK;
    HIP_TRY(x, hipSetDevice(x->device));
    HIP_TRY(x, quiesce(x));
    if (copy == 1u) {
        HIP_TRY(x, hipMemcpyAsync(out, s->d_bf16 + row0 * x->dim, (size_t)rows * x->dim * sizeof(uint16_t), hipMemcpyDeviceToHost, x->stream));
    } else {
        HIP_TRY(x, hipMemcpyAsync(out, s->d_i8 + row0 * x->dim, (size_t)rows * x->dim, hipMemcpyDeviceToHost, x->stream));
        HIP_TRY(x, hipMemcpyAsync(out_scales, s->d_i8_scale + row0, (size_t)rows * sizeof(float), hipMemcpyDeviceToHost, x->stream));
    }
    HIP_TRY(x, hipStreamSynchronize(x->stream));
    return CQS_HIP_OK;
} CQS_ABI_CATCH(x)

int32_t cqs_hip_debug_shadow_scores(cqs_hip_index* x, uint32_t copy, const float* queries, uint32_t b, uint32_t k,
                                    const uint32_t* keep_bitset, uint32_t mode, float threshold, float* out_scores,
                                    float* out_bq) CQS_ABI_TRY {
    if (!x || x->sh || !queries || !out_scores || !out_bq || b == 0 || copy > 2u || mode > CQS_HIP_MODE_PIPELINE) return CQS_HIP_ERR_INVALID;
    if (k == 0 || k > cqs::kMaxK) return CQS_HIP_ERR_INVALID;
    std::lock_guard<std::mutex> g(x->mu);
    if (x->poisoned.load(std::memory_order_acquire)) return CQS_HIP_ERR_POISONED;
    const Shadow* s = x->shadow;
    if (!s || x->n == 0 || b > cqs::kMaxGemvQ || !shadow_takes(x, b, k, false)) return CQS_HIP_ERR_INVALID;
    if (copy == 2u && !(s->d_i8 && b <= cqs::kI8MaxQ && cqs::i8_k_ok(k))) return CQS_HIP_ERR_INVALID;
    HIP_TRY(x, hipSetDevice(x->device));
    HIP_TRY(x, quiesce(x));
    const bool i8 = copy == 2u || (copy == 0u && shadow_uses_i8(x, b, k));
    const uint32_t kp = copy == 2u ? cqs::i8_kprime(k) : cqs::shadow_kprime(k);
    const uint32_t k_scan = copy == 0u ? k : kp + 1u;
    int32_t rc = ensure_scratch(x, b, k_scan);
    if (rc != CQS_HIP_OK) return rc;
    const uint32_t* d_keep = nullptr;
    if (keep_bitset) {
        if ((rc = stage_keep(x, keep_bitset, (x->n + 31) / 32)) != CQS_HIP_OK) return rc;
        d_keep = x->d_keep;
    }
    hipStream_t st = x->stream;
    HIP_TRY(x, hipMemcpyAsync(x->d_q, queries, (size_t)b * x->dim * sizeof(float), hipMemcpyHostToDevice, st));
    if (i8) HIP_TRY(x, cqs::launch_i8_bound(x->d_q, b, x->dim, s->r8, s->norm8, s->d_bq, st));
    else HIP_TRY(x, cqs::launch_shadow_bound(x->d_q, b, x->dim, s->r, s->norm, s->d_bq, st));
    if (copy == 0u) {
        const cqs::ScanArgs a = scan_args(x, x->d_q, b, k, d_keep, mode, threshold, sizeof(float), false, x->d_dbg, nullptr);
        HIP_TRY(x, cqs::launch_scan(a, st));
    } else {
        const cqs::ScanArgs a = scan_args(x, x->d_q, b, k_scan, d_keep, mode, threshold, i8 ? sizeof(int8_t) : sizeof(uint16_t), true, nullptr, nullptr);
        if (i8) HIP_TRY(x, cqs::launch_scan_i8(a, s->d_i8, s->d_i8_scale, s->d_bq, st));
        else HIP_TRY(x, cqs::launch_scan_bf16(a, s->d_bf16, s->d_bq, st));
    }
    HIP_TRY(x, hipMemsetAsync(x->d_work, 0, cqs::kWorkWords * sizeof(uint32_t), st));
    const size_t row_b = (size_t)x->n * sizeof(float);
    HIP_TRY(x, hipMemcpy2DAsync(out_scores, row_b, x->d_scores, (size_t)pad_rows(x->n) * sizeof(float), row_b, b, hipMemcpyDeviceToHost, st));
    HIP_TRY(x, hipMemcpyAsync(out_bq, s->d_bq, (size_t)b * sizeof(float), hipMemcpyDeviceToHost, st));
    HIP_TRY(x, hipStreamSynchronize(st));
    return CQS_HIP_OK;
} CQS_ABI_CATCH(x)

}
```

### cqs_amd/csrc/scan_bf16.h

```cpp
#pragma once
#include <math.h>
#include <stdint.h>

#if defined(__HIPCC__)
#include <hip/hip_runtime.h>
#include "scan_kernels.h"
#define CQS_HD __host__ __device__
#else
#define CQS_HD
#endif

namespace cqs {

constexpr uint32_t kShadowMaxQ = 32;
constexpr uint32_t kShadowMaxDim = 2048;
constexpr uint32_t kShadowKMax = 1024;

inline uint32_t shadow_kprime(uint32_t k) {
    const uint32_t kp = 2u * k + 32u;
    return kp < kShadowKMax - 1u ? kp : kShadowKMax - 1u;
}

CQS_HD inline double shadow_gamma(uint32_t dim) {
    const double du = (double)dim * 0x1p-24;
    return du / (1.0 - du);
}

CQS_HD inline float round_up_f32(double v) {
    float f = (float)v;
    if ((double)f < v) f = nextafterf(f, INFINITY);
    return f;
}

CQS_HD inline float shadow_query_bound(double q_norm2, double r_max, double norm_max, uint32_t dim) {
    const double qn = sqrt(q_norm2) * (1.0 + 0x1p-40);
    if (!(qn * norm_max * (1.0 + shadow_gamma(dim)) < 0x1p100)) return INFINITY;
    return round_up_f32(qn * r_max * (1.0 + 0x1p-40) + (double)dim * 0x1p-140);
}

#if defined(__HIPCC__)
__device__ __forceinline__ double wave_q_norm2(const float* qp, uint32_t dim, uint32_t lane) {
    double s2 = 0.0;
    for (uint32_t d = lane; d < dim; d += 64u) s2 += (double)qp[d] * (double)qp[d];
#pragma unroll
    for (int m = 32; m >= 1; m >>= 1) s2 += __shfl_xor(s2, m, 64);
    return s2;
}
__device__ __forceinline__ float wave_shadow_bound(const float* qp, uint32_t dim, double r_max, double norm_max, uint32_t lane) {
    return shadow_query_bound(wave_q_norm2(qp, dim, lane), r_max, norm_max, dim);
}

hipError_t launch_shadow_build(const float* rows, uint16_t* shadow, uint64_t row0, uint64_t n_rows, uint32_t dim,
                               double gamma, unsigned long long* stats, hipStream_t st);

hipError_t launch_shadow_bound(const float* q, uint32_t b, uint32_t dim, double r_max, double norm_max, float* bq,
                               hipStream_t st);

hipError_t launch_scan_bf16(const ScanArgs& a, const uint16_t* shadow, const float* bq, hipStream_t st);

hipError_t launch_rescore_certify(const ScanArgs& a, uint32_t row_base, uint32_t k, uint32_t kprime, uint32_t bound,
                                  double r_max, double norm_max, float* bq, uint32_t* tickets, uint64_t* ekeys,
                                  uint64_t* out_keys, uint32_t* out_counts, uint32_t* cert, unsigned long long* counters,
                                  unsigned long long* counters2, hipStream_t st);
#endif

}
```

### cqs_amd/csrc/scan_bf16.hip

```cpp
#include "scan_bf16.h"
#include "scan_i8.h"
#include "launch_util.h"
#include "rank_sort.h"
#include "scan_device.h"
#include "select_device.h"

namespace cqs {

static_assert(kShadowKMax == kMaxK, "shadow k' policy and the select agree on max k");

typedef float f4 __attribute__((ext_vector_type(4)));
typedef float f2 __attribute__((ext_vector_type(2)));
typedef unsigned u4 __attribute__((ext_vector_type(4)));
typedef __bf16 bf2 __attribute__((ext_vector_type(2)));

__device__ __forceinline__ float bf_lo(uint32_t w) { return __uint_as_float(w << 16); }
__device__ __forceinline__ float bf_hi(uint32_t w) { return __uint_as_float(w & 0xFFFF0000u); }
__device__ __forceinline__ float key_score(uint64_t key) {
    const uint32_t ok = (uint32_t)(key >> 32);
    return __uint_as_float((ok & 0x80000000u) ? (ok ^ 0x80000000u) : ~ok);
}

__global__ __launch_bounds__(256) void shadow_build_kernel(const float* __restrict__ rows, uint16_t* __restrict__ shadow,
                                                           uint64_t row0, uint64_t n_rows, uint32_t dim, double gamma,
                                                           unsigned long long* __restrict__ stats) {
    const int lane = threadIdx.x & 63;
    const uint64_t waves = (uint64_t)gridDim.x * (blockDim.x >> 6);
    for (uint64_t r = (uint64_t)blockIdx.x * (blockDim.x >> 6) + (threadIdx.x >> 6); r < n_rows; r += waves) {
        const float* xp = rows + (row0 + r) * dim;
        uint16_t* op = shadow + (row0 + r) * dim;
        double d2 = 0.0, n2 = 0.0, t2 = 0.0;
        bool fin = true, big = false;
        for (uint32_t i = (uint32_t)lane * 2u; i < dim; i += 128u) {
            const f2 v = *(const f2*)(xp + i);
            const bf2 h = __builtin_convertvector(v, bf2);
            const uint32_t w = __builtin_bit_cast(uint32_t, h);
            *(uint32_t*)(op + i) = w;
            const float t0 = bf_lo(w), t1 = bf_hi(w);
            fin = fin && __builtin_isfinite(v.x) && __builtin_isfinite(v.y);
            big = big || __builtin_fabsf(v.x) >= 0x1p64f || __builtin_fabsf(v.y) >= 0x1p64f;
            const double e0 = (double)v.x - (double)t0, e1 = (double)v.y - (double)t1;
            d2 += e0 * e0 + e1 * e1;
            n2 += (double)v.x * (double)v.x + (double)v.y * (double)v.y;
            t2 += (double)t0 * (double)t0 + (double)t1 * (double)t1;
        }
#pragma unroll
        for (int m = 32; m >= 1; m >>= 1) {
            d2 += __shfl_xor(d2, m, 64);
            n2 += __shfl_xor(n2, m, 64);
            t2 += __shfl_xor(t2, m, 64);
        }
        const bool all_fin = __ballot(!fin) == 0ull;
        const bool any_big = __ballot(big) != 0ull;
        if (lane == 0 && all_fin) {
            const double nx = sqrt(n2), nt = sqrt(t2);
            const double rb = sqrt(d2) + gamma * (nx + nt);
            atomicMax(&stats[0], (unsigned long long)__double_as_longlong(rb));
            atomicMax(&stats[1], (unsigned long long)__double_as_longlong(nx > nt ? nx : nt));
            if (any_big) atomicMax(&stats[2], 1ull);
        }
    }
}

hipError_t launch_shadow_build(const float* rows, uint16_t* shadow, uint64_t row0, uint64_t n_rows, uint32_t dim,
                               double gamma, unsigned long long* stats, hipStream_t st) {
    if (n_rows == 0) return hipSuccess;
    const uint64_t blocks = (n_rows + 3u) / 4u;
    hipLaunchKernelGGL(shadow_build_kernel, dim3((uint32_t)(blocks < 8192u ? blocks : 8192u)), dim3(256), 0, st, rows,
                       shadow, row0, n_rows, dim, gamma, stats);
    return hipGetLastError();
}

__global__ __launch_bounds__(64) void shadow_bound_kernel(const float* __restrict__ q, uint32_t dim, double r_max,
                                                          double norm_max, float* __restrict__ bq) {
    const uint32_t lane = threadIdx.x;
    const float v = wave_shadow_bound(q + (size_t)blockIdx.x * dim, dim, r_max, norm_max, lane);
    if (lane == 0) bq[blockIdx.x] = v;
}

hipError_t launch_shadow_bound(const float* q, uint32_t b, uint32_t dim, double r_max, double norm_max, float* bq,
                               hipStream_t st) {
    if (b == 0) return hipSuccess;
    if (b > kShadowMaxQ) return hipErrorInvalidValue;
    hipLaunchKernelGGL(shadow_bound_kernel, dim3(b), dim3(64), 0, st, q, dim, r_max, norm_max, bq);
    return hipGetLastError();
}

struct Bf16ScanParams {
    const uint16_t* rows;
    uint32_t n, n_pad, dim;
    const float* q;
    float* scores;
    const uint32_t* keep;
    uint32_t mode;
    float thr;
    uint32_t nq;
    uint32_t* work;
    TaskTiers tiers;
    uint32_t n_tasks;
    float* gmax;
    uint64_t* gaux;
    const float* bq;
};

template <int NCH, int BQ, int RI, bool NT, bool FULL>
__global__ __launch_bounds__(256) void scan_bf16_kernel(const Bf16ScanParams p) {
    constexpr int NV = RI * BQ;
    constexpr int LPV = 64 / NV;
    const int lane = threadIdx.x & 63;
    const uint32_t n = p.n, dim = p.dim;

    uint32_t coff[NCH];
    f4 qa[BQ][NCH], qb[BQ][NCH];
#pragma unroll
    for (int c = 0; c < NCH; ++c) {
        const uint32_t idx = (uint32_t)c * 512u + (uint32_t)lane * 8u;
        const bool in = FULL || idx < dim;
        coff[c] = in ? idx : dim - 8u;
#pragma unroll
        for (int b = 0; b < BQ; ++b) {
            const float* qp = p.q + (size_t)((uint32_t)b < p.nq ? b : 0) * dim + coff[c];
            const f4 va = *(const f4*)qp, vb = *(const f4*)(qp + 4);
            qa[b][c] = in ? va : (f4)(0.f);
            qb[b][c] = in ? vb : (f4)(0.f);
        }
    }

    const uint32_t last = n - 1u;
    const uint32_t nwords = (n + 31u) / 32u;
    const uint32_t n_tasks = p.n_tasks;
    const uint32_t wpb = blockDim.x >> 6;
    const uint32_t total_waves = gridDim.x * wpb;
    const uint32_t wave_id = (uint32_t)__builtin_amdgcn_readfirstlane((int)(blockIdx.x * wpb + (threadIdx.x >> 6)));
    const bool use_queue = n_tasks > total_waves;
    uint32_t opaque_zero;
    asm volatile("v_mov_b32 %0, 0" : "=v"(opaque_zero));

    const char* const rows_b = (const char*)p.rows;
    const uint32_t row_bytes = dim * 2u;
    auto load_rows = [&](uint32_t base, int j, u4 (&x)[RI][NCH]) {
#pragma unroll
        for (int r = 0; r < RI; ++r) {
            uint32_t row = base + (uint32_t)(RI * j + r);
            row = row > last ? last : row;
            const char* rp = rows_b + (uint64_t)row * row_bytes;
#pragma unroll
            for (int c = 0; c < NCH; ++c) {
                const u4* src = (const u4*)(rp + coff[c] * 2u);
                if (NT) x[r][c] = __builtin_nontemporal_load(src);
                else x[r][c] = *src;
            }
        }
        __builtin_amdgcn_sched_barrier(0);
    };
    auto reduce_rows = [&](int j, u4 (&x)[RI][NCH], float (&sc)[BQ]) {
        f2 acc2[NV];
#pragma unroll
        for (int i = 0; i < NV; ++i) acc2[i] = (f2)(0.f);
#pragma unroll
        for (int r = 0; r < RI; ++r)
#pragma unroll
            for (int c = 0; c < NCH; ++c) {
                const u4 w = x[r][c];
                const f2 x0 = {bf_lo(w.x), bf_hi(w.x)}, x1 = {bf_lo(w.y), bf_hi(w.y)};
                const f2 x2 = {bf_lo(w.z), bf_hi(w.z)}, x3 = {bf_lo(w.w), bf_hi(w.w)};
#pragma unroll
                for (int b = 0; b < BQ; ++b) {
                    f2 a = acc2[b * RI + r];
                    a = __builtin_elementwise_fma(x0, __builtin_shufflevector(qa[b][c], qa[b][c], 0, 1), a);
                    a = __builtin_elementwise_fma(x1, __builtin_shufflevector(qa[b][c], qa[b][c], 2, 3), a);
                    a = __builtin_elementwise_fma(x2, __builtin_shufflevector(qb[b][c], qb[b][c], 0, 1), a);
                    a = __builtin_elementwise_fma(x3, __builtin_shufflevector(qb[b][c], qb[b][c], 2, 3), a);
                    acc2[b * RI + r] = a;
                }
            }
        float acc[NV];
#pragma unroll
        for (int i = 0; i < NV; ++i) acc[i] = acc2[i].x + acc2[i].y;
        treduce<NV>(acc, lane);
#pragma unroll
        for (int b = 0; b < BQ; ++b) {
            const float t = __shfl(acc[0], (b * RI + (lane % RI)) * LPV, 64);
            if (lane / RI == j) sc[b] = t;
        }
    };
    auto epilogue = [&](uint32_t cur, uint32_t base, uint32_t trows, uint64_t mask, float (&sc)[BQ]) {
        const uint32_t row = base + (uint32_t)lane;
        const bool live = (uint32_t)lane < trows && ((mask >> lane) & 1ull);
#pragma unroll
        for (int b = 0; b < BQ; ++b) {
            float s = sc[b];
            if (!live || !(__builtin_fabsf(s) <= 3.4028234664e38f)) s = -INFINITY;
            else if (p.mode == 1u && (uint32_t)b < p.nq) {
                float t = s + p.bq[b];
                t = t < 0.f ? 0.f : (t > 1.f ? 1.f : t);
                if (!(t >= p.thr)) s = -INFINITY;
            }
            if ((uint32_t)b >= p.nq) continue;
            if ((uint32_t)lane < trows && row < p.n_pad) p.scores[(size_t)b * p.n_pad + row] = s;
            const float gm = wave_max64(s);
            if (lane == 0) p.gmax[(size_t)b * n_tasks + cur] = gm;
            if (p.gaux) {
                const uint32_t arg = (uint32_t)__builtin_ctzll(__ballot(s == gm));
                const float sec = wave_max64(((uint32_t)lane == arg) ? -INFINITY : s);
                if (lane == 0) p.gaux[(size_t)b * n_tasks + cur] = ((uint64_t)arg << 32) | (uint64_t)__float_as_uint(sec);
            }
        }
    };
    auto task_mask = [&](uint32_t base, uint32_t trows) -> uint64_t {
        const uint64_t all = trows == 64u ? ~0ull : ((1ull << trows) - 1ull);
        uint64_t mask = all;
        if (base + trows > n) mask = (base >= n) ? 0ull : (all >> (trows - (n - base)));
        if (p.keep) {
            const uint32_t w = base / 32u;
            const uint32_t w0 = (w < nwords) ? p.keep[w] : 0u;
            const uint32_t w1 = (w + 1u < nwords) ? p.keep[w + 1u] : 0u;
            mask &= (((uint64_t)w1 << 32) | (uint64_t)w0) >> (base & 31u);
        }
        const uint32_t mlo = __builtin_amdgcn_readfirstlane((uint32_t)mask);
        const uint32_t mhi = __builtin_amdgcn_readfirstlane((uint32_t)(mask >> 32));
        return ((uint64_t)mhi << 32) | mlo;
    };

    u4 x[RI][NCH];
    uint32_t cur = wave_id;
    while (cur < n_tasks) {
        uint32_t trows;
        const uint32_t base = p.tiers.locate(cur, trows);
        const uint64_t mask = task_mask(base, trows);
        uint32_t ticket = 0;
        if (use_queue && lane == 0) ticket = atomicAdd(p.work + opaque_zero, 1u);
        float sc[BQ];
#pragma unroll
        for (int b = 0; b < BQ; ++b) sc[b] = -INFINITY;
        const int nb = (int)(trows / (uint32_t)RI);
        for (int j = 0; j < nb; ++j) {
            const uint32_t m = (uint32_t)(mask >> (RI * j)) & ((1u << RI) - 1u);
            if (m == 0u) continue;
            load_rows(base, j, x);
            reduce_rows(j, x, sc);
        }
        epilogue(cur, base, trows, mask, sc);
        cur = use_queue ? total_waves + (uint32_t)__builtin_amdgcn_readfirstlane(ticket) : n_tasks;
    }
}

#ifndef CQS_BF16_ONE_SHOT
#define CQS_BF16_ONE_SHOT 24u
#endif
#ifndef CQS_BF16_BLOCKS_PER_CU
#define CQS_BF16_BLOCKS_PER_CU 2u
#endif

template <int NCH, int BQ, int RI>
static hipError_t launch_bf16(const ScanArgs& a, const uint16_t* shadow, const float* bq, uint32_t q0, uint32_t nq,
                              uint32_t work_slot, hipStream_t st) {
    Bf16ScanParams p;
    p.rows = shadow; p.n = a.n; p.n_pad = a.n_pad; p.dim = a.dim;
    p.q = a.q + (size_t)q0 * a.dim;
    p.scores = a.scores + (size_t)q0 * a.n_pad;
    p.keep = a.keep; p.mode = a.mode; p.thr = a.threshold;
    p.nq = nq;
    p.work = a.work + work_slot;
    p.tiers = a.tiers;
    p.n_tasks = a.tiers.total();
    p.gmax = a.gmax + (size_t)q0 * p.n_tasks;
    p.gaux = a.gaux ? a.gaux + (size_t)q0 * p.n_tasks : nullptr;
    p.bq = bq + q0;
    const bool one_shot = p.n_tasks <= a.n_cu * 4u * CQS_BF16_ONE_SHOT;
    const uint32_t wpb = 4u;
    const uint32_t blocks = one_shot ? (p.n_tasks + wpb - 1u) / wpb : a.n_cu * CQS_BF16_BLOCKS_PER_CU;
    const dim3 grid(blocks), block(64u * wpb);
    const bool full = (a.dim == (uint32_t)NCH * 512u);
    if (a.nontemporal) {
        if (full) hipLaunchKernelGGL((scan_bf16_kernel<NCH, BQ, RI, true, true>), grid, block, 0, st, p);
        else hipLaunchKernelGGL((scan_bf16_kernel<NCH, BQ, RI, true, false>), grid, block, 0, st, p);
    } else {
        if (full) hipLaunchKernelGGL((scan_bf16_kernel<NCH, BQ, RI, false, true>), grid, block, 0, st, p);
        else hipLaunchKernelGGL((scan_bf16_kernel<NCH, BQ, RI, false, false>), grid, block, 0, st, p);
    }
    return hipGetLastError();
}

template <int NCH>
static hipError_t launch_bf16_groups(const ScanArgs& a, const uint16_t* shadow, const float* bq, hipStream_t st) {
    uint32_t done = 0, slot = 0;
    while (done < a.b) {
        const uint32_t left = a.b - done;
        hipError_t e;
        uint32_t g;
        if constexpr (NCH <= 2) {
            if (left >= 5) { g = left < 8u ? left : 8u; e = launch_bf16<NCH, 8, 2>(a, shadow, bq, done, g, slot, st); }
            else if (left >= 4) { g = 4; e = launch_bf16<NCH, 4, 4>(a, shadow, bq, done, g, slot, st); }
            else if (left >= 2) { g = 2; e = launch_bf16<NCH, 2, 8>(a, shadow, bq, done, g, slot, st); }
            else { g = 1; e = launch_bf16<NCH, 1, 16>(a, shadow, bq, done, g, slot, st); }
        } else {
            if (left >= 2) { g = 2; e = launch_bf16<NCH, 2, 4>(a, shadow, bq, done, g, slot, st); }
            else { g = 1; e = launch_bf16<NCH, 1, 8>(a, shadow, bq, done, g, slot, st); }
        }
        if (e != hipSuccess) return e;
        done += g;
        slot = (slot + 1u) % kWorkWords;
    }
    return hipSuccess;
}

hipError_t launch_scan_bf16(const ScanArgs& a, const uint16_t* shadow, const float* bq, hipStream_t st) {
    if (a.b == 0 || a.n == 0) return hipSuccess;
    if (a.b > kShadowMaxQ || a.dim % 8u != 0u || a.dim > kShadowMaxDim) return hipErrorInvalidValue;
    switch ((a.dim + 511u) / 512u) {
        case 1: return launch_bf16_groups<1>(a, shadow, bq, st);
        case 2: return launch_bf16_groups<2>(a, shadow, bq, st);
        case 3: return launch_bf16_groups<3>(a, shadow, bq, st);
        case 4: return launch_bf16_groups<4>(a, shadow, bq, st);
        default: return hipErrorInvalidValue;
    }
}

struct TailParams {
    const float* rows;
    const float* q;
    uint32_t dim, k, kprime, mode, row_base;
    float thr;
    const float* scores;
    const float* gmax;
    const uint64_t* gaux;
    uint32_t n_pad;
    TaskTiers tiers;
    uint32_t bins;
    uint32_t* work;
    uint64_t* ekeys;
    float* bq;
    uint32_t* tickets;
    uint32_t bound;
    double r_max, norm_max;
    uint64_t* out_keys;
    uint32_t* out_counts;
    uint32_t* cert;
    unsigned long long* counters;
    unsigned long long* counters2;
};

constexpr uint32_t kTailWaves = 16;

template <int NCH>
__global__ __launch_bounds__(1024) void rescore_certify_kernel(const TailParams p) {
    __shared__ uint64_t s_keys[kShadowKMax];
    __shared__ uint64_t s_sorted[kShadowKMax];
    __shared__ __attribute__((aligned(16))) uint32_t s_ok[kShadowKMax + 4];
    __shared__ uint32_t s_cnt, s_flag, s_last;
    const uint32_t lane = threadIdx.x & 63u;
    const uint32_t qi = blockIdx.y;
    const uint32_t wave = (uint32_t)__builtin_amdgcn_readfirstlane((int)(blockIdx.x * kTailWaves + (threadIdx.x >> 6)));
    const uint32_t n_waves = gridDim.x * kTailWaves;
    const uint32_t dim = p.dim;
    const float* qp = p.q + (size_t)qi * dim;
    if (threadIdx.x == 0) s_cnt = 0u;
    if (qi == 0u && blockIdx.x == 0u)
        for (uint32_t i = threadIdx.x; i < kWorkWords; i += 1024u) p.work[i] = 0u;

    const uint32_t n_tasks = p.tiers.total();
    uint32_t found;
    const uint64_t* akeys = select_body(p.scores + (size_t)qi * p.n_pad, p.gmax + (size_t)qi * n_tasks,
                                        p.gaux ? p.gaux + (size_t)qi * n_tasks : nullptr, p.n_pad, p.tiers, p.kprime + 1u,
                                        p.row_base, p.bins, nullptr, found);
    const uint32_t ac = found < p.kprime + 1u ? found : p.kprime + 1u;
    const uint32_t nc = ac < p.kprime ? ac : p.kprime;
    const uint64_t key_next = ac > p.kprime ? akeys[p.kprime] : 0ull;

    for (uint32_t slot = wave; slot <= nc; slot += n_waves) {
        if (slot == 0u) {
            if (p.bound != 0u) {
                const float v = p.bound == 2u ? wave_i8_bound(qp, dim, p.r_max, p.norm_max, lane)
                                              : wave_shadow_bound(qp, dim, p.r_max, p.norm_max, lane);
                if (lane == 0u)
                    __hip_atomic_store((uint32_t*)p.bq + qi, __float_as_uint(v), __ATOMIC_RELAXED, __HIP_MEMORY_SCOPE_AGENT);
            }
            continue;
        }
        const uint32_t i = slot - 1u;
        const uint64_t key = akeys[i];
        const uint32_t grow = 0xFFFFFFFFu - (uint32_t)key;
        const float* rp = p.rows + (size_t)(grow - p.row_base) * dim;
        f4 x[NCH], qv[NCH];
#pragma unroll
        for (int c = 0; c < NCH; ++c) {
            const uint32_t idx = (uint32_t)c * 256u + lane * 4u;
            const bool in = idx < dim;
            const uint32_t off = in ? idx : dim - 4u;
            x[c] = *(const f4*)(rp + off);
            const f4 v = *(const f4*)(qp + off);
            qv[c] = in ? v : (f4)(0.f);
        }
        f2 acc2 = (f2)(0.f);
#pragma unroll
        for (int c = 0; c < NCH; ++c) {
            const f2 xlo = __builtin_shufflevector(x[c], x[c], 0, 1);
            const f2 xhi = __builtin_shufflevector(x[c], x[c], 2, 3);
            acc2 = __builtin_elementwise_fma(xlo, __builtin_shufflevector(qv[c], qv[c], 0, 1), acc2);
            acc2 = __builtin_elementwise_fma(xhi, __builtin_shufflevector(qv[c], qv[c], 2, 3), acc2);
        }
        float s = acc2.x + acc2.y;
#pragma unroll
        for (int m = 32; m >= 1; m >>= 1) s += __shfl_xor(s, m, 64);
        bool keep = __builtin_fabsf(s) <= 3.4028234664e38f;
        if (keep && p.mode == 1u) {
            s = s < 0.f ? 0.f : (s > 1.f ? 1.f : s);
            keep = s >= p.thr;
        }
        if (lane == 0u)
            __hip_atomic_store(p.ekeys + (size_t)qi * p.kprime + i, keep ? pack_key(okey(s), grow) : 0ull, __ATOMIC_RELAXED,
                               __HIP_MEMORY_SCOPE_AGENT);
    }
    asm volatile("s_waitcnt vmcnt(0)" ::: "memory");
    __syncthreads();
    if (threadIdx.x == 0) {
        const uint32_t t = __hip_atomic_fetch_add(p.tickets + qi, 1u, __ATOMIC_RELAXED, __HIP_MEMORY_SCOPE_AGENT);
        const bool last = t == gridDim.x - 1u;
        if (last) __hip_atomic_store(p.tickets + qi, 0u, __ATOMIC_RELAXED, __HIP_MEMORY_SCOPE_AGENT);
        s_last = last ? 1u : 0u;
    }
    __syncthreads();
    if (s_last == 0u) return;

    if (threadIdx.x < nc) {
        const uint64_t key = __hip_atomic_load(p.ekeys + (size_t)qi * p.kprime + threadIdx.x, __ATOMIC_RELAXED, __HIP_MEMORY_SCOPE_AGENT);
        if (key != 0ull) s_keys[atomicAdd(&s_cnt, 1u)] = key;
    }
    __syncthreads();
    const uint32_t m = s_cnt;
    rank_sort_keys(s_keys, m, s_sorted, s_ok, &s_flag);
    const uint32_t k = p.k;
    const uint32_t outc = m < k ? m : k;
    for (uint32_t i = threadIdx.x; i < k; i += 1024u) p.out_keys[(size_t)qi * k + i] = (i < outc) ? s_sorted[i] : 0ull;
    if (threadIdx.x == 0) {
        p.out_counts[qi] = outc;
        const float bq = __uint_as_float(__hip_atomic_load((uint32_t*)p.bq + qi, __ATOMIC_RELAXED, __HIP_MEMORY_SCOPE_AGENT));
        bool ok = false;
        if (__builtin_fabsf(bq) <= 3.4028234664e38f) {
            if (ac <= p.kprime) ok = true;
            else if (m >= k) {
                float t = key_score(key_next) + bq;
                if (p.mode == 1u) t = t < 0.f ? 0.f : (t > 1.f ? 1.f : t);
                ok = t < key_score(s_sorted[k - 1u]);
            }
        }
        p.cert[qi] = ok ? 1u : 0u;
        if (p.counters) atomicAdd(&p.counters[ok ? 0 : 1], 1ull);
        if (p.counters2) atomicAdd(&p.counters2[ok ? 0 : 1], 1ull);
    }
}

#ifndef CQS_TAIL_MAX_BLOCKS_PER_CU
#define CQS_TAIL_MAX_BLOCKS_PER_CU 1u
#endif

hipError_t launch_rescore_certify(const ScanArgs& a, uint32_t row_base, uint32_t k, uint32_t kprime, uint32_t bound,
                                  double r_max, double norm_max, float* bq, uint32_t* tickets, uint64_t* ekeys,
                                  uint64_t* out_keys, uint32_t* out_counts, uint32_t* cert, unsigned long long* counters,
                                  unsigned long long* counters2, hipStream_t st) {
    const uint32_t b = a.b, dim = a.dim;
    if (b == 0) return hipSuccess;
    if (b > kShadowMaxQ || k == 0 || kprime < k || kprime >= kShadowKMax || a.k != kprime + 1u || dim % 8u != 0u ||
        dim > kShadowMaxDim || bound > 2u)
        return hipErrorInvalidValue;
    const TailParams tp{a.rows, a.q, dim, k, kprime, a.mode, row_base, a.threshold, a.scores, a.gmax, a.gaux, a.n_pad, a.tiers,
                        a.range_bins ? 2u : (a.linear_bins ? 1u : 0u), a.work, ekeys, bq, tickets, bound, r_max, norm_max,
                        out_keys, out_counts, cert, counters, counters2};
    const uint32_t want = (kprime + 1u + kTailWaves - 1u) / kTailWaves;
    uint32_t cap = a.n_cu * CQS_TAIL_MAX_BLOCKS_PER_CU / b;
    if (cap < 1u) cap = 1u;
    const dim3 grid(want < cap ? want : cap, b), block(64u * kTailWaves);
    switch ((dim + 255u) / 256u) {
        case 1: hipLaunchKernelGGL(rescore_certify_kernel<1>, grid, block, 0, st, tp); break;
        case 2: hipLaunchKernelGGL(rescore_certify_kernel<2>, grid, block, 0, st, tp); break;
        case 3: hipLaunchKernelGGL(rescore_certify_kernel<3>, grid, block, 0, st, tp); break;
        case 4: hipLaunchKernelGGL(rescore_certify_kernel<4>, grid, block, 0, st, tp); break;
        case 5: hipLaunchKernelGGL(rescore_certify_kernel<5>, grid, block, 0, st, tp); break;
        case 6: hipLaunchKernelGGL(rescore_certify_kernel<6>, grid, block, 0, st, tp); break;
        case 7: hipLaunchKernelGGL(rescore_certify_kernel<7>, grid, block, 0, st, tp); break;
        case 8: hipLaunchKernelGGL(rescore_certify_kernel<8>, grid, block, 0, st, tp); break;
        default: return hipErrorInvalidValue;
    }
    return hipGetLastError();
}

}
```

### cqs_amd/csrc/scan_device.h

```cpp
#pragma once
#include <hip/hip_runtime.h>
#include <stdint.h>

namespace cqs {

__device__ __forceinline__ uint32_t okey(float x) {
    uint32_t b = __float_as_uint(x);
    return b ^ ((b >> 31) ? 0xFFFFFFFFu : 0x80000000u);
}
constexpr uint32_t kInvalidKey = 0x007FFFFFu;

__device__ __forceinline__ uint64_t pack_key(uint32_t ok, uint32_t global_row) {
    return ((uint64_t)ok << 32) | (uint64_t)(0xFFFFFFFFu - global_row);
}

template <int N, int M, int NV>
__device__ __forceinline__ void treduce_level(float (&v)[NV], int lane) {
    if constexpr (N > 1) {
        const bool hi = (lane & M) != 0;
#pragma unroll
        for (int i = 0; i < N / 2; ++i) {
            const float keep = hi ? v[i + N / 2] : v[i];
            const float send = hi ? v[i] : v[i + N / 2];
            v[i] = keep + __shfl_xor(send, M, 64);
        }
        treduce_level<N / 2, M / 2, NV>(v, lane);
    } else if constexpr (M >= 1) {
        v[0] += __shfl_xor(v[0], M, 64);
        treduce_level<1, M / 2, NV>(v, lane);
    }
}
template <int NV>
__device__ __forceinline__ void treduce(float (&v)[NV], int lane) {
    treduce_level<NV, 32, NV>(v, lane);
}

}
```

### cqs_amd/csrc/scan_i8.h

```cpp
#pragma once
#include "scan_bf16.h"

namespace cqs {

constexpr uint32_t kI8MaxQ = 4;

inline uint32_t i8_kprime(uint32_t k) { return 10u * k + 150u; }
inline bool i8_k_ok(uint32_t k) { return i8_kprime(k) <= kShadowKMax - 1u; }

inline bool i8_dim_ok(uint32_t dim) { return dim % 16u == 0u && dim <= kShadowMaxDim; }

CQS_HD inline double i8_gamma(uint32_t dim) { return shadow_gamma(dim + 2u); }

CQS_HD inline float i8_query_bound(double q_norm2, double r_max, double norm_max, uint32_t dim) {
    const double qn = sqrt(q_norm2) * (1.0 + 0x1p-40);
    if (!(qn * norm_max * (1.0 + i8_gamma(dim)) < 0x1p100)) return INFINITY;
    if (!(qn * 128.0 * sqrt((double)dim) < 0x1p100)) return INFINITY;
    return round_up_f32(qn * r_max * (1.0 + 0x1p-40) + (double)dim * 0x1p-140 * (1.0 + norm_max));
}

#if defined(__HIPCC__)
__device__ __forceinline__ float wave_i8_bound(const float* qp, uint32_t dim, double r_max, double norm_max, uint32_t lane) {
    return i8_query_bound(wave_q_norm2(qp, dim, lane), r_max, norm_max, dim);
}

hipError_t launch_i8_build(const float* rows, int8_t* codes, float* scales, uint64_t row0, uint64_t n_rows, uint32_t dim,
                           double gamma, unsigned long long* stats, hipStream_t st);

hipError_t launch_i8_bound(const float* q, uint32_t b, uint32_t dim, double r_max, double norm_max, float* bq, hipStream_t st);

hipError_t launch_scan_i8(const ScanArgs& a, const int8_t* codes, const float* scales, const float* bq, hipStream_t st);
#endif

}
```

### cqs_amd/csrc/scan_i8.hip

```cpp
#include "scan_i8.h"
#include "launch_util.h"
#include "scan_device.h"

namespace cqs {

typedef float f4 __attribute__((ext_vector_type(4)));
typedef float f2 __attribute__((ext_vector_type(2)));
typedef unsigned u4 __attribute__((ext_vector_type(4)));

template <int I>
__device__ __forceinline__ float code_f32(uint32_t w) { return (float)(int)(int8_t)(w >> (8 * I)); }

constexpr int kI8BuildVecs = (int)(kShadowMaxDim / 256u);

__global__ __launch_bounds__(256) void i8_build_kernel(const float* __restrict__ rows, int8_t* __restrict__ codes,
                                                       float* __restrict__ scales, uint64_t row0, uint64_t n_rows,
                                                       uint32_t dim, double gamma, unsigned long long* __restrict__ stats) {
    const uint32_t lane = threadIdx.x & 63u;
    const uint64_t waves = (uint64_t)gridDim.x * (blockDim.x >> 6);
    for (uint64_t r = (uint64_t)blockIdx.x * (blockDim.x >> 6) + (threadIdx.x >> 6); r < n_rows; r += waves) {
        const float* xp = rows + (row0 + r) * dim;
        int8_t* op = codes + (row0 + r) * dim;
        f4 v[kI8BuildVecs];
        float m = 0.f;
        bool fin = true;
#pragma unroll
        for (int j = 0; j < kI8BuildVecs; ++j) {
            const uint32_t i = (uint32_t)j * 256u + lane * 4u;
            v[j] = i < dim ? *(const f4*)(xp + i) : (f4)(0.f);
#pragma unroll
            for (int e = 0; e < 4; ++e) {
                fin = fin && __builtin_isfinite(v[j][e]);
                m = fmaxf(m, __builtin_fabsf(v[j][e]));
            }
        }
        m = wave_max64(m);
        const bool all_fin = __ballot(!fin) == 0ull;
        const float scale = all_fin ? m / 127.f : __builtin_nanf("");
        const bool zero = !(scale > 0.f);
        double d2 = 0.0, n2 = 0.0, t2 = 0.0;
#pragma unroll
        for (int j = 0; j < kI8BuildVecs; ++j) {
            const uint32_t i = (uint32_t)j * 256u + lane * 4u;
            if (i >= dim) continue;
            uint32_t w = 0u;
#pragma unroll
            for (int e = 0; e < 4; ++e) {
                float c = zero ? 0.f : __builtin_rintf(v[j][e] / scale);
                c = c < -127.f ? -127.f : (c > 127.f ? 127.f : c);
                w |= ((uint32_t)(int)c & 0xFFu) << (8 * e);
                const double t = (double)scale * (double)c;
                const double d = (double)v[j][e] - t;
                d2 += d * d;
                n2 += (double)v[j][e] * (double)v[j][e];
                t2 += t * t;
            }
            *(uint32_t*)(op + i) = w;
        }
#pragma unroll
        for (int s = 32; s >= 1; s >>= 1) {
            d2 += __shfl_xor(d2, s, 64);
            n2 += __shfl_xor(n2, s, 64);
            t2 += __shfl_xor(t2, s, 64);
        }
        if (lane == 0u) {
            scales[row0 + r] = scale;
            if (all_fin) {
                const double nx = sqrt(n2), nt = sqrt(t2);
                atomicMax(&stats[0], (unsigned long long)__double_as_longlong(sqrt(d2) + gamma * (nx + nt)));
                atomicMax(&stats[1], (unsigned long long)__double_as_longlong(nx > nt ? nx : nt));
                if (m >= 0x1p64f) atomicMax(&stats[2], 1ull);
            }
        }
    }
}

hipError_t launch_i8_build(const float* rows, int8_t* codes, float* scales, uint64_t row0, uint64_t n_rows, uint32_t dim,
                           double gamma, unsigned long long* stats, hipStream_t st) {
    if (n_rows == 0) return hipSuccess;
    if (!i8_dim_ok(dim)) return hipErrorInvalidValue;
    const uint64_t blocks = (n_rows + 3u) / 4u;
    hipLaunchKernelGGL(i8_build_kernel, dim3((uint32_t)(blocks < 8192u ? blocks : 8192u)), dim3(256), 0, st, rows, codes,
                       scales, row0, n_rows, dim, gamma, stats);
    return hipGetLastError();
}

__global__ __launch_bounds__(64) void i8_bound_kernel(const float* __restrict__ q, uint32_t dim, double r_max,
                                                      double norm_max, float* __restrict__ bq) {
    const uint32_t lane = threadIdx.x;
    const float v = wave_i8_bound(q + (size_t)blockIdx.x * dim, dim, r_max, norm_max, lane);
    if (lane == 0) bq[blockIdx.x] = v;
}

hipError_t launch_i8_bound(const float* q, uint32_t b, uint32_t dim, double r_max, double norm_max, float* bq, hipStream_t st) {
    if (b == 0) return hipSuccess;
    if (b > kShadowMaxQ) return hipErrorInvalidValue;
    hipLaunchKernelGGL(i8_bound_kernel, dim3(b), dim3(64), 0, st, q, dim, r_max, norm_max, bq);
    return hipGetLastError();
}

struct I8ScanParams {
    const int8_t* rows;
    const float* scales;
    uint32_t n, n_pad, dim;
    const float* q;
    float* scores;
    const uint32_t* keep;
    uint32_t mode;
    float thr;
    uint32_t nq;
    TaskTiers tiers;
    uint32_t n_tasks;
    float* gmax;
    uint64_t* gaux;
    const float* bq;
};

template <int NCH, int BQ, int RI, bool NT, bool FULL>
__global__ __launch_bounds__(256) void scan_i8_kernel(const I8ScanParams p) {
    constexpr int NV = RI * BQ;
    constexpr int LPV = 64 / NV;
    const int lane = threadIdx.x & 63;
    const uint32_t n = p.n, dim = p.dim;

    uint32_t coff[NCH];
    f4 qv[BQ][NCH][4];
#pragma unroll
    for (int c = 0; c < NCH; ++c) {
        const uint32_t idx = (uint32_t)c * 1024u + (uint32_t)lane * 16u;
        const bool in = FULL || idx < dim;
        coff[c] = in ? idx : dim - 16u;
#pragma unroll
        for (int b = 0; b < BQ; ++b) {
            const float* qp = p.q + (size_t)((uint32_t)b < p.nq ? b : 0) * dim + coff[c];
#pragma unroll
            for (int w = 0; w < 4; ++w) {
                const f4 t = *(const f4*)(qp + 4 * w);
                qv[b][c][w] = in ? t : (f4)(0.f);
            }
        }
    }

    const uint32_t last = n - 1u;
    const uint32_t nwords = (n + 31u) / 32u;
    const uint32_t n_tasks = p.n_tasks;
    const uint32_t wpb = blockDim.x >> 6;
    const uint32_t cur = (uint32_t)__builtin_amdgcn_readfirstlane((int)(blockIdx.x * wpb + (threadIdx.x >> 6)));
    if (cur >= n_tasks) return;

    const char* const rows_b = (const char*)p.rows;
    auto load_rows = [&](uint32_t base, int j, u4 (&x)[RI][NCH]) {
#pragma unroll
        for (int r = 0; r < RI; ++r) {
            uint32_t row = base + (uint32_t)(RI * j + r);
            row = row > last ? last : row;
            const char* rp = rows_b + (uint64_t)row * dim;
#pragma unroll
            for (int c = 0; c < NCH; ++c) {
                const u4* src = (const u4*)(rp + coff[c]);
                if (NT) x[r][c] = __builtin_nontemporal_load(src);
                else x[r][c] = *src;
            }
        }
        __builtin_amdgcn_sched_barrier(0);
    };
    auto reduce_rows = [&](int j, u4 (&x)[RI][NCH], float (&sc)[BQ]) {
        f2 acc2[NV];
#pragma unroll
        for (int i = 0; i < NV; ++i) acc2[i] = (f2)(0.f);
#pragma unroll
        for (int r = 0; r < RI; ++r)
#pragma unroll
            for (int c = 0; c < NCH; ++c)
#pragma unroll
                for (int w = 0; w < 4; ++w) {
                    const uint32_t u = x[r][c][w];
                    const f2 lo = {code_f32<0>(u), code_f32<1>(u)}, hi = {code_f32<2>(u), code_f32<3>(u)};
#pragma unroll
                    for (int b = 0; b < BQ; ++b) {
                        const f4 qq = qv[b][c][w];
                        f2 a = acc2[b * RI + r];
                        a = __builtin_elementwise_fma(lo, __builtin_shufflevector(qq, qq, 0, 1), a);
                        a = __builtin_elementwise_fma(hi, __builtin_shufflevector(qq, qq, 2, 3), a);
                        acc2[b * RI + r] = a;
                    }
                }
        float acc[NV];
#pragma unroll
        for (int i = 0; i < NV; ++i) acc[i] = acc2[i].x + acc2[i].y;
        treduce<NV>(acc, lane);
#pragma unroll
        for (int b = 0; b < BQ; ++b) {
            const float t = __shfl(acc[0], (b * RI + (lane % RI)) * LPV, 64);
            if (lane / RI == j) sc[b] = t;
        }
    };
    auto epilogue = [&](uint32_t cur, uint32_t base, uint32_t trows, uint64_t mask, float scale, float (&sc)[BQ]) {
        const uint32_t row = base + (uint32_t)lane;
        const bool live = (uint32_t)lane < trows && ((mask >> lane) & 1ull);
#pragma unroll
        for (int b = 0; b < BQ; ++b) {
            float s = sc[b] * scale;
            if (!live || !(__builtin_fabsf(s) <= 3.4028234664e38f)) s = -INFINITY;
            else if (p.mode == 1u && (uint32_t)b < p.nq) {
                float t = s + p.bq[b];
                t = t < 0.f ? 0.f : (t > 1.f ? 1.f : t);
                if (!(t >= p.thr)) s = -INFINITY;
            }
            if ((uint32_t)b >= p.nq) continue;
            if ((uint32_t)lane < trows && row < p.n_pad) p.scores[(size_t)b * p.n_pad + row] = s;
            const float gm = wave_max64(s);
            if (lane == 0) p.gmax[(size_t)b * n_tasks + cur] = gm;
            if (p.gaux) {
                const uint32_t arg = (uint32_t)__builtin_ctzll(__ballot(s == gm));
                const float sec = wave_max64(((uint32_t)lane == arg) ? -INFINITY : s);
                if (lane == 0) p.gaux[(size_t)b * n_tasks + cur] = ((uint64_t)arg << 32) | (uint64_t)__float_as_uint(sec);
            }
        }
    };
    auto task_mask = [&](uint32_t base, uint32_t trows) -> uint64_t {
        const uint64_t all = trows == 64u ? ~0ull : ((1ull << trows) - 1ull);
        uint64_t mask = all;
        if (base + trows > n) mask = (base >= n) ? 0ull : (all >> (trows - (n - base)));
        if (p.keep) {
            const uint32_t w = base / 32u;
            const uint32_t w0 = (w < nwords) ? p.keep[w] : 0u;
            const uint32_t w1 = (w + 1u < nwords) ? p.keep[w + 1u] : 0u;
            mask &= (((uint64_t)w1 << 32) | (uint64_t)w0) >> (base & 31u);
        }
        const uint32_t mlo = __builtin_amdgcn_readfirstlane((uint32_t)mask);
        const uint32_t mhi = __builtin_amdgcn_readfirstlane((uint32_t)(mask >> 32));
        return ((uint64_t)mhi << 32) | mlo;
    };

    u4 x[RI][NCH];
    uint32_t trows;
    const uint32_t base = p.tiers.locate(cur, trows);
    const uint64_t mask = task_mask(base, trows);
    const uint32_t srow = base + (uint32_t)lane;
    const float scale = p.scales[srow > last ? last : srow];
    float sc[BQ];
#pragma unroll
    for (int b = 0; b < BQ; ++b) sc[b] = -INFINITY;
    const int nb = (int)(trows / (uint32_t)RI);
    for (int j = 0; j < nb; ++j) {
        const uint32_t m = (uint32_t)(mask >> (RI * j)) & ((1u << RI) - 1u);
        if (m == 0u) continue;
        load_rows(base, j, x);
        reduce_rows(j, x, sc);
    }
    epilogue(cur, base, trows, mask, scale, sc);
}

constexpr int kI8RowsPerBatch = 16;

template <int NCH, int BQ, int RI>
static hipError_t launch_i8(const ScanArgs& a, const int8_t* codes, const float* scales, const float* bq, uint32_t q0,
                            uint32_t nq, hipStream_t st) {
    I8ScanParams p;
    p.rows = codes; p.scales = scales; p.n = a.n; p.n_pad = a.n_pad; p.dim = a.dim;
    p.q = a.q + (size_t)q0 * a.dim;
    p.scores = a.scores + (size_t)q0 * a.n_pad;
    p.keep = a.keep; p.mode = a.mode; p.thr = a.threshold;
    p.nq = nq;
    p.tiers = a.tiers;
    p.n_tasks = a.tiers.total();
    p.gmax = a.gmax + (size_t)q0 * p.n_tasks;
    p.gaux = a.gaux ? a.gaux + (size_t)q0 * p.n_tasks : nullptr;
    p.bq = bq + q0;
    const uint32_t wpb = 4u;
    const dim3 grid((p.n_tasks + wpb - 1u) / wpb), block(64u * wpb);
    const bool full = (a.dim == (uint32_t)NCH * 1024u);
    if (a.nontemporal) {
        if (full) hipLaunchKernelGGL((scan_i8_kernel<NCH, BQ, RI, true, true>), grid, block, 0, st, p);
        else hipLaunchKernelGGL((scan_i8_kernel<NCH, BQ, RI, true, false>), grid, block, 0, st, p);
    } else {
        if (full) hipLaunchKernelGGL((scan_i8_kernel<NCH, BQ, RI, false, true>), grid, block, 0, st, p);
        else hipLaunchKernelGGL((scan_i8_kernel<NCH, BQ, RI, false, false>), grid, block, 0, st, p);
    }
    return hipGetLastError();
}

template <int NCH>
static hipError_t launch_i8_groups(const ScanArgs& a, const int8_t* codes, const float* scales, const float* bq, hipStream_t st) {
    uint32_t done = 0;
    while (done < a.b) {
        const uint32_t left = a.b - done;
        hipError_t e;
        uint32_t g;
        if (left >= 3) { g = left < 4u ? left : 4u; e = launch_i8<NCH, 4, 4>(a, codes, scales, bq, done, g, st); }
        else if (left >= 2) { g = 2; e = launch_i8<NCH, 2, 8>(a, codes, scales, bq, done, g, st); }
        else { g = 1; e = launch_i8<NCH, 1, kI8RowsPerBatch>(a, codes, scales, bq, done, g, st); }
        if (e != hipSuccess) return e;
        done += g;
    }
    return hipSuccess;
}

hipError_t launch_scan_i8(const ScanArgs& a, const int8_t* codes, const float* scales, const float* bq, hipStream_t st) {
    if (a.b == 0 || a.n == 0) return hipSuccess;
    if (a.b > kShadowMaxQ || !i8_dim_ok(a.dim)) return hipErrorInvalidValue;
    switch ((a.dim + 1023u) / 1024u) {
        case 1: return launch_i8_groups<1>(a, codes, scales, bq, st);
        case 2: return launch_i8_groups<2>(a, codes, scales, bq, st);
        default: return hipErrorInvalidValue;
    }
}

}
```

### cqs_amd/csrc/scan_kernels.h

```cpp
#pragma once
#include <hip/hip_runtime.h>
#include <stdint.h>

namespace cqs {

constexpr uint32_t kTaskRows = 64;
constexpr uint32_t kTaskRowsSmall = 16;
constexpr uint32_t kRowsPerBlock = 256;
constexpr uint32_t kHistBins = 4096;
constexpr uint32_t kCandCap = 8192;
constexpr uint32_t kMaxK = 1024;
constexpr uint32_t kMaxGemvQ = 8;
constexpr uint32_t kDbgWaves = 4096;
constexpr uint32_t kWorkWords = 64;

struct TaskTiers {
    uint32_t nA, nB, nC;
    __host__ __device__ uint32_t total() const { return nA + nB + nC; }
    __host__ __device__ uint32_t locate(uint32_t t, uint32_t& rows) const {
        if (t < nA) { rows = 64u; return t * 64u; }
        if (t < nA + nB) { rows = 32u; return nA * 64u + (t - nA) * 32u; }
        rows = 16u;
        return nA * 64u + nB * 32u + (t - nA - nB) * 16u;
    }
};
TaskTiers plan_tiers(uint32_t n_pad, uint32_t n_cu, bool uniform64);

struct ScanArgs {
    const float* rows;
    uint32_t n;
    uint32_t n_pad;
    uint32_t dim;
    const float* q;
    uint32_t b;
    float* scores;
    const uint32_t* keep;
    uint32_t mode;
    float threshold;
    bool nontemporal;
    bool linear_bins;
    bool range_bins = false;
    uint32_t k;
    float* gmax;
    uint64_t* gaux = nullptr;
    TaskTiers tiers;
    uint32_t* work;
    uint32_t n_cu;
    bool gemv_only = false;
    void* dbg;
    const uint32_t* gate = nullptr;
};

hipError_t launch_scan(const ScanArgs& a, hipStream_t stream);

hipError_t launch_select(const ScanArgs& a, uint32_t row_base, uint64_t* out_keys, uint32_t* out_counts,
                         hipStream_t stream);

hipError_t launch_scan_mfma(const ScanArgs& a, uint32_t q0, uint32_t nq, uint32_t work_slot, hipStream_t stream);
uint32_t mfma_query_tile(uint32_t nq);
constexpr uint32_t kMfmaMinQueries = 9;
inline bool use_mfma(uint32_t b, uint32_t dim) { return b >= kMfmaMinQueries && dim % 32u == 0; }
inline bool uniform_groups(uint32_t b, uint32_t dim) { return use_mfma(b, dim); }

bool scan_dim_supported(uint32_t dim);

#if defined(__HIPCC__)
__device__ __forceinline__ bool gate_closed(const uint32_t* gate, uint32_t b) {
    uint32_t all = 1u;
    for (uint32_t i = 0; i < b; ++i) all &= gate[i];
    return all != 0u;
}

template <int CTRL>
__device__ __forceinline__ float wave_dpp(float v) {
    return __builtin_bit_cast(float, __builtin_amdgcn_update_dpp(0, __builtin_bit_cast(int, v), CTRL, 0xF, 0xF, false));
}
__device__ __forceinline__ float wave_max16(float m) {
    m = fmaxf(m, wave_dpp<0xB1>(m));
    m = fmaxf(m, wave_dpp<0x4E>(m));
    m = fmaxf(m, wave_dpp<0x141>(m));
    m = fmaxf(m, wave_dpp<0x140>(m));
    return m;
}
__device__ __forceinline__ float wave_max64(float m) {
    typedef unsigned wm_u2 __attribute__((ext_vector_type(2)));
    m = wave_max16(m);
    const wm_u2 a = __builtin_amdgcn_permlane16_swap(__float_as_uint(m), __float_as_uint(m), false, false);
    m = fmaxf(__uint_as_float(a[0]), __uint_as_float(a[1]));
    const wm_u2 b = __builtin_amdgcn_permlane32_swap(__float_as_uint(m), __float_as_uint(m), false, false);
    return fmaxf(__uint_as_float(b[0]), __uint_as_float(b[1]));
}
#endif

}
```

### cqs_amd/csrc/select_device.h

```cpp
#pragma once
#include <hip/hip_runtime.h>
#include <stdint.h>

#include "rank_sort.h"
#include "scan_device.h"
#include "scan_kernels.h"

namespace cqs {

__device__ __forceinline__ uint32_t bin_of(float s, bool linear) {
    if (linear) {
        const float t = (s + 1.0f) * 2048.0f;
        const int b = (int)t;
        return (uint32_t)(b < 0 ? 0 : (b > 4095 ? 4095 : b));
    }
    return okey(s) >> 20;
}
__device__ __forceinline__ uint32_t bin_of_range(float s, float lo, float scale) {
    if (!(scale > 0.f)) return 0u;
    const float t = (s - lo) * scale;
    if (!(t < 4095.0f)) return 4095u;
    return t > 0.f ? (uint32_t)(int)t : 0u;
}
__device__ __forceinline__ uint32_t bin_any(float s, uint32_t mode, float lo, float scale) {
    return mode == 2u ? bin_of_range(s, lo, scale) : bin_of(s, mode != 0u);
}

template <int THREADS>
__device__ void block_decide(const uint32_t* hist, uint32_t k_rem, uint32_t* s_part ,
                             uint32_t* res ) {
    constexpr int BPT = kHistBins / THREADS;
    constexpr int NW = THREADS / 64;
    const int t = threadIdx.x, lane = t & 63, w = t >> 6;
    uint32_t h[BPT];
    uint32_t sum = 0;
#pragma unroll
    for (int i = 0; i < BPT; ++i) {
        h[i] = hist[t * BPT + i];
        sum += h[i];
    }
    uint32_t incl = sum;
#pragma unroll
    for (int off = 1; off < 64; off <<= 1) {
        const uint32_t v = __shfl_down(incl, off, 64);
        if (lane + off < 64) incl += v;
    }
    if (lane == 0) s_part[w] = incl;
    __syncthreads();
    for (int ww = w + 1; ww < NW; ++ww) incl += s_part[ww];
    uint32_t above = incl - sum;
    if (t == 0) {
        res[3] = incl;
        if (incl < k_rem) {
            res[0] = 0;
            res[1] = incl - h[0];
            res[2] = h[0];
        }
    }
    if (above < k_rem && incl >= k_rem) {
#pragma unroll
        for (int i = BPT - 1; i >= 0; --i) {
            if (above < k_rem && above + h[i] >= k_rem) {
                res[0] = (uint32_t)(t * BPT + i);
                res[1] = above;
                res[2] = h[i];
            }
            above += h[i];
        }
    }
    __syncthreads();
}

static __device__ uint32_t slow_select(const float* __restrict__ s, uint32_t n_pad, uint32_t k, uint32_t row_base,
                                uint64_t* s_keys, uint32_t* s_hist, uint32_t* s_part, uint32_t* s_res,
                                uint32_t* s_cnt) {
    uint64_t prefix = 0;
    int bits_done = 0;
    uint32_t k_rem = k, sel_above = 0;
    uint64_t lb = 0;
    while (bits_done < 64) {
        const int w = (64 - bits_done) >= 12 ? 12 : (64 - bits_done);
        for (int i = threadIdx.x; i < (int)kHistBins; i += 1024) s_hist[i] = 0;
        __syncthreads();
        for (uint32_t i = threadIdx.x; i < n_pad; i += 1024u) {
            const uint32_t kk = okey(s[i]);
            if (kk <= kInvalidKey) continue;
            const uint64_t key = pack_key(kk, row_base + i);
            if (bits_done == 0 || (key >> (64 - bits_done)) == prefix)
                atomicAdd(&s_hist[(uint32_t)(key >> (64 - bits_done - w)) & ((1u << w) - 1u)], 1u);
        }
        __syncthreads();
        block_decide<1024>(s_hist, k_rem, s_part, s_res);
        const uint32_t T = s_res[0], above = s_res[1], cnt = s_res[2], total = s_res[3];
        __syncthreads();
        if (bits_done == 0 && total <= k) { lb = 0; break; }
        prefix = (prefix << w) | T;
        bits_done += w;
        sel_above += above;
        k_rem -= above;
        lb = prefix << (64 - bits_done);
        if (sel_above + cnt <= kCandCap) break;
    }
    if (threadIdx.x == 0) *s_cnt = 0;
    __syncthreads();
    for (uint32_t i = threadIdx.x; i < n_pad; i += 1024u) {
        const uint32_t kk = okey(s[i]);
        if (kk <= kInvalidKey) continue;
        const uint64_t key = pack_key(kk, row_base + i);
        if (key >= lb) {
            const uint32_t slot = atomicAdd(s_cnt, 1u);
            if (slot < kCandCap) s_keys[slot] = key;
        }
    }
    __syncthreads();
    const uint32_t c = *s_cnt;
    return c < kCandCap ? c : kCandCap;
}

constexpr uint32_t kGroupCap = 8192;
constexpr int kGB = 16;

__device__ __forceinline__ const uint64_t* select_body(const float* __restrict__ s, const float* __restrict__ gm,
                                                       const uint64_t* __restrict__ ga, uint32_t n_pad,
                                                       const TaskTiers& tiers, uint32_t k, uint32_t row_base,
                                                       uint32_t linear, unsigned long long* __restrict__ dbg,
                                                       uint32_t& count_out) {
    __shared__ uint64_t s_keys[kCandCap];
    __shared__ uint32_t s_groups[kGroupCap];
    __shared__ __attribute__((aligned(16))) uint32_t s_hist[kHistBins];
    __shared__ uint32_t s_part[1024];
    __shared__ uint32_t s_res[4];
    __shared__ uint32_t s_cnt, s_ng, s_ng2;
    const uint32_t n_tasks = tiers.total();
    const int lane = threadIdx.x & 63;
    float r_lo = 0.f, r_scale = 0.f;

#define CQS_STAMP(i) do { if (dbg && threadIdx.x == 0 && blockIdx.x == 0) dbg[i] = __builtin_amdgcn_s_memrealtime(); } while (0)
    CQS_STAMP(0);
    for (uint32_t i = threadIdx.x; i < kHistBins; i += 1024u) s_hist[i] = 0u;
    if (threadIdx.x == 0) { s_cnt = 0; s_ng = 0; s_ng2 = 0; }
    __syncthreads();
    if (linear == 2u) {
        float lo = INFINITY, hi = -INFINITY;
        for (uint32_t t0 = 0; t0 < n_tasks; t0 += 1024u * kGB) {
            float v[kGB];
#pragma unroll
            for (int u = 0; u < kGB; ++u) {
                const uint32_t t = t0 + (uint32_t)u * 1024u + threadIdx.x;
                v[u] = gm[t < n_tasks ? t : n_tasks - 1u];
            }
#pragma unroll
            for (int u = 0; u < kGB; ++u)
                if (v[u] != -INFINITY) { lo = fminf(lo, v[u]); hi = fmaxf(hi, v[u]); }
        }
#pragma unroll
        for (int off = 32; off >= 1; off >>= 1) {
            lo = fminf(lo, __shfl_xor(lo, off, 64));
            hi = fmaxf(hi, __shfl_xor(hi, off, 64));
        }
        float* const f_part = reinterpret_cast<float*>(s_part);
        if (lane == 0) { f_part[threadIdx.x >> 6] = lo; f_part[16 + (threadIdx.x >> 6)] = hi; }
        __syncthreads();
        lo = f_part[0]; hi = f_part[16];
        for (int w = 1; w < 16; ++w) { lo = fminf(lo, f_part[w]); hi = fmaxf(hi, f_part[16 + w]); }
        __syncthreads();
        r_lo = lo;
        r_scale = (hi > lo) ? 4096.0f / (hi - lo) : 0.f;
        if (!(r_scale < INFINITY)) r_scale = 0.f;
    }

    float m[kGB];
    const bool one_pass = n_tasks <= 1024u * kGB;
    for (uint32_t t0 = 0; t0 < n_tasks; t0 += 1024u * kGB) {
#pragma unroll
        for (int u = 0; u < kGB; ++u) {
            const uint32_t t = t0 + (uint32_t)u * 1024u + threadIdx.x;
            const float v = gm[t < n_tasks ? t : n_tasks - 1u];
            m[u] = t < n_tasks ? v : -INFINITY;
        }
#pragma unroll
        for (int u = 0; u < kGB; ++u)
            if (m[u] != -INFINITY) atomicAdd(&s_hist[bin_any(m[u], linear, r_lo, r_scale)], 1u);
    }
    __syncthreads();
    CQS_STAMP(1);
    block_decide<1024>(s_hist, k, s_part, s_res);
    const uint32_t T = (s_res[3] < k) ? 0u : s_res[0];
    __syncthreads();
    CQS_STAMP(2);

    for (uint32_t t0 = 0; t0 < n_tasks; t0 += 1024u * kGB) {
        if (!one_pass) {
#pragma unroll
            for (int u = 0; u < kGB; ++u) {
                const uint32_t t = t0 + (uint32_t)u * 1024u + threadIdx.x;
                const float v = gm[t < n_tasks ? t : n_tasks - 1u];
                m[u] = t < n_tasks ? v : -INFINITY;
            }
        }
        bool take[kGB];
        uint64_t mk[kGB];
        uint32_t pre[kGB], tot = 0;
#pragma unroll
        for (int u = 0; u < kGB; ++u) {
            take[u] = (m[u] != -INFINITY) && (bin_any(m[u], linear, r_lo, r_scale) >= T);
            mk[u] = __ballot(take[u]);
            pre[u] = tot;
            tot += (uint32_t)__popcll(mk[u]);
        }
        uint32_t base = 0;
        if (tot) {
            if (lane == 0) base = atomicAdd(&s_ng, tot);
            base = (uint32_t)__builtin_amdgcn_readfirstlane((int)base);
        }
#pragma unroll
        for (int u = 0; u < kGB; ++u) {
            const uint32_t slot = base + pre[u] + __builtin_amdgcn_mbcnt_hi((uint32_t)(mk[u] >> 32), __builtin_amdgcn_mbcnt_lo((uint32_t)mk[u], 0u));
            if (take[u] && slot < kGroupCap) s_groups[slot] = t0 + (uint32_t)u * 1024u + threadIdx.x;
        }
    }
    __syncthreads();
    CQS_STAMP(3);
    const uint32_t ng = s_ng;
    uint32_t count = kCandCap + 1u;
    if (ng <= kGroupCap) {
        const uint32_t* glist = s_groups;
        uint32_t n2 = ng;
        if (ga) {
            uint32_t* const s_list2 = s_hist;
            for (uint32_t i0 = 0; i0 < ng; i0 += 1024u) {
                const uint32_t i = i0 + threadIdx.x;
                const bool valid = i < ng;
                const uint32_t t = s_groups[valid ? i : ng - 1u];
                const uint64_t ax = ga[t];
                const float mx = gm[t];
                const float sec = __uint_as_float((uint32_t)ax);
                const bool need = valid && (sec != -INFINITY) && (bin_any(sec, linear, r_lo, r_scale) >= T);
                const bool direct = valid && !need;
                const uint64_t mn = __ballot(need), md = __ballot(direct);
                uint32_t bn = 0, bd = 0;
                if (lane == 0) {
                    if (mn) bn = atomicAdd(&s_ng2, (uint32_t)__popcll(mn));
                    if (md) bd = atomicAdd(&s_cnt, (uint32_t)__popcll(md));
                }
                bn = (uint32_t)__builtin_amdgcn_readfirstlane((int)bn);
                bd = (uint32_t)__builtin_amdgcn_readfirstlane((int)bd);
                if (need) {
                    const uint32_t slot = bn + __builtin_amdgcn_mbcnt_hi((uint32_t)(mn >> 32), __builtin_amdgcn_mbcnt_lo((uint32_t)mn, 0u));
                    if (slot < kHistBins) s_list2[slot] = t;
                }
                if (direct) {
                    const uint32_t slot = bd + __builtin_amdgcn_mbcnt_hi((uint32_t)(md >> 32), __builtin_amdgcn_mbcnt_lo((uint32_t)md, 0u));
                    uint32_t grows;
                    const uint32_t gbase = tiers.locate(t, grows);
                    if (slot < kCandCap) s_keys[slot] = pack_key(okey(mx), row_base + gbase + (uint32_t)(ax >> 32));
                }
            }
            __syncthreads();
            if (s_ng2 <= kHistBins) { glist = s_list2; n2 = s_ng2; }
            else {
                __syncthreads();
                if (threadIdx.x == 0) s_cnt = 0;
                __syncthreads();
            }
        }
        constexpr int kGU = 8;
        const uint32_t wv = threadIdx.x >> 6;
        for (uint32_t g0 = wv * kGU; g0 < n2; g0 += 16u * kGU) {
            float v[kGU];
            uint32_t idx[kGU];
            bool in[kGU];
#pragma unroll
            for (int u = 0; u < kGU; ++u) {
                const uint32_t g = g0 + (uint32_t)u;
                uint32_t grows;
                const uint32_t gbase = tiers.locate((uint32_t)__builtin_amdgcn_readfirstlane((int)glist[g < n2 ? g : n2 - 1u]), grows);
                in[u] = g < n2 && (uint32_t)lane < grows;
                idx[u] = gbase + (in[u] ? (uint32_t)lane : 0u);
            }
#pragma unroll
            for (int u = 0; u < kGU; ++u) v[u] = s[idx[u]];
            uint64_t mask[kGU];
            uint32_t pre[kGU], tot = 0;
            bool take[kGU];
#pragma unroll
            for (int u = 0; u < kGU; ++u) {
                take[u] = in[u] && (v[u] != -INFINITY) && (bin_any(v[u], linear, r_lo, r_scale) >= T);
                mask[u] = __ballot(take[u]);
                pre[u] = tot;
                tot += (uint32_t)__popcll(mask[u]);
            }
            uint32_t base = 0;
            if (tot) {
                if (lane == 0) base = atomicAdd(&s_cnt, tot);
                base = (uint32_t)__builtin_amdgcn_readfirstlane((int)base);
            }
#pragma unroll
            for (int u = 0; u < kGU; ++u) {
                const uint32_t slot = base + pre[u] +
                    __builtin_amdgcn_mbcnt_hi((uint32_t)(mask[u] >> 32), __builtin_amdgcn_mbcnt_lo((uint32_t)mask[u], 0u));
                if (take[u] && slot < kCandCap) s_keys[slot] = pack_key(okey(v[u]), row_base + idx[u]);
            }
        }
        __syncthreads();
        count = s_cnt;
    }
    if (count > kCandCap)
        count = slow_select(s, n_pad, k, row_base, s_keys, s_hist, s_part, s_res, &s_cnt);

    CQS_STAMP(4);
    if (dbg && threadIdx.x == 0 && blockIdx.x == 0) { dbg[8] = ng; dbg[9] = count; }
    const uint64_t* sorted = s_keys;
    if (count <= 1024u) {
        uint64_t* s_sorted = reinterpret_cast<uint64_t*>(s_groups);
        uint32_t* s_ok = s_hist;
        rank_sort_keys(s_keys, count, s_sorted, s_ok, s_res);
        sorted = s_sorted;
    } else {
        uint32_t P = 2048;
        while (P < count) P <<= 1;
        for (uint32_t i = count + threadIdx.x; i < P; i += 1024u) s_keys[i] = 0ull;
        __syncthreads();
        for (uint32_t size = 2; size <= P; size <<= 1) {
            for (uint32_t stride = size >> 1; stride > 0; stride >>= 1) {
                for (uint32_t t = threadIdx.x; t < P / 2; t += 1024u) {
                    const uint32_t i = 2u * t - (t & (stride - 1u));
                    const uint32_t j = i + stride;
                    const uint64_t a = s_keys[i], b = s_keys[j];
                    const bool desc = ((i & size) == 0u);
                    if ((a < b) == desc) {
                        s_keys[i] = b;
                        s_keys[j] = a;
                    }
                }
                __syncthreads();
            }
        }
    }

    CQS_STAMP(5);
#undef CQS_STAMP
    count_out = count;
    return sorted;
}

}
```

Before: 6761 queries/s.

## Build group-max histogram during shadow scan and use it in rescore tail

The bf16 and int8 shadow scan kernels now atomically add each wave's group maximum into a per-query global histogram. The rescore/certify tail gets the histogram plus candidate buffers, so it can pick a threshold and gather candidates without rebuilding a histogram over all group maxima. This adds global atomics to the scan and new scratch buffers. The histogram must be cleared after use, and on failure it is cleared explicitly.

Measured after the change: 6123 queries/s. -9.4%, worse.

```diff
diff --git a/cqs_amd/csrc/index.hip b/cqs_amd/csrc/index.hip
--- a/cqs_amd/csrc/index.hip
+++ b/cqs_amd/csrc/index.hip
@@ -132,8 +132,8 @@
         }
         HIP_TRY(x, hipEventRecord(x->ev[x->ev_used], st));
     }
-    if (shadow && shadow->bf16) HIP_TRY(x, cqs::launch_scan_bf16(a, shadow->bf16, shadow->bq, st));
-    else if (shadow) HIP_TRY(x, cqs::launch_scan_i8(a, shadow->i8, shadow->i8_scale, shadow->bq, st));
+    if (shadow && shadow->bf16) HIP_TRY(x, cqs::launch_scan_bf16(a, shadow->bf16, shadow->bq, shadow->hist, st));
+    else if (shadow) HIP_TRY(x, cqs::launch_scan_i8(a, shadow->i8, shadow->i8_scale, shadow->bq, shadow->hist, st));
     else HIP_TRY(x, cqs::launch_scan(a, st));
     if (timed) {
         HIP_TRY(x, hipEventRecord(x->ev[x->ev_used + 1], st));
diff --git a/cqs_amd/csrc/index_internal.h b/cqs_amd/csrc/index_internal.h
--- a/cqs_amd/csrc/index_internal.h
+++ b/cqs_amd/csrc/index_internal.h
@@ -104,7 +104,7 @@
 uint32_t max_query_block(const cqs_hip_index* x);
 cqs::ScanArgs scan_args(const cqs_hip_index* x, const float* d_q, uint32_t b, uint32_t k, const uint32_t* d_keep,
                         uint32_t mode, float thr, size_t elem_bytes, bool gemv_only, void* dbg, const uint32_t* gate);
-struct ShadowRows { const uint16_t* bf16; const int8_t* i8; const float* i8_scale; const float* bq; };
+struct ShadowRows { const uint16_t* bf16; const int8_t* i8; const float* i8_scale; const float* bq; uint32_t* hist; };
 int32_t scan_select(cqs_hip_index* x, const cqs::ScanArgs& a, hipStream_t st, const ShadowRows* shadow,
                     uint64_t* out_keys, uint32_t* out_counts);
 inline hipError_t order_after_last(cqs_hip_index* x, hipStream_t st) {
diff --git a/cqs_amd/csrc/index_shadow.hip b/cqs_amd/csrc/index_shadow.hip
--- a/cqs_amd/csrc/index_shadow.hip
+++ b/cqs_amd/csrc/index_shadow.hip
@@ -27,6 +27,9 @@
     uint32_t* d_cert = nullptr;
     float* d_bq = nullptr;
     uint32_t* d_tickets = nullptr;
+    uint32_t* d_hist = nullptr;
+    uint32_t* d_ccnt = nullptr;
+    uint64_t* d_cand = nullptr;
     uint32_t* h_cert = nullptr;
     uint32_t* h_cert_dev = nullptr;
 };
@@ -59,7 +62,8 @@
     x->stat_i8_fallbacks.fetch_add(f, std::memory_order_relaxed);
     i8_free(s);
     hipFree(s->d_bf16); hipFree(s->d_stats); hipFree(s->d_ekeys);
-    hipFree(s->d_cert); hipFree(s->d_bq); hipFree(s->d_tickets); hipHostFree(s->h_cert);
+    hipFree(s->d_cert); hipFree(s->d_bq); hipFree(s->d_tickets); hipFree(s->d_hist);
+    hipFree(s->d_ccnt); hipFree(s->d_cand); hipHostFree(s->h_cert);
     delete s;
     x->shadow = nullptr;
 }
@@ -183,6 +187,12 @@
     if ((e = hipMalloc(&s->d_bq, (size_t)cqs::kShadowMaxQ * sizeof(float))) != hipSuccess) return oom(e);
     if ((e = hipMalloc(&s->d_tickets, (size_t)cqs::kShadowMaxQ * sizeof(uint32_t))) != hipSuccess) return oom(e);
     if ((e = hipMemsetAsync(s->d_tickets, 0, (size_t)cqs::kShadowMaxQ * sizeof(uint32_t), x->stream)) != hipSuccess) return oom(e);
+    const size_t hist_b = (size_t)cqs::kShadowMaxQ * cqs::kHistBins * sizeof(uint32_t), ccnt_b = 2u * cqs::kShadowMaxQ * sizeof(uint32_t);
+    if ((e = hipMalloc(&s->d_hist, hist_b)) != hipSuccess) return oom(e);
+    if ((e = hipMemsetAsync(s->d_hist, 0, hist_b, x->stream)) != hipSuccess) return oom(e);
+    if ((e = hipMalloc(&s->d_ccnt, ccnt_b)) != hipSuccess) return oom(e);
+    if ((e = hipMemsetAsync(s->d_ccnt, 0, ccnt_b, x->stream)) != hipSuccess) return oom(e);
+    if ((e = hipMalloc(&s->d_cand, (size_t)cqs::kShadowMaxQ * cqs::kTailCandCap * 2u * sizeof(uint64_t))) != hipSuccess) return oom(e);
     if ((e = hipHostMalloc(&s->h_cert, (size_t)cqs::kShadowMaxQ * sizeof(uint32_t), hipHostMallocDefault)) != hipSuccess) return oom(e);
     if (hipHostGetDevicePointer((void**)&s->h_cert_dev, s->h_cert, 0) != hipSuccess) {
         (void)hipGetLastError();
@@ -281,13 +291,17 @@
         else HIP_TRY(x, cqs::launch_shadow_bound(d_q, nb, x->dim, r_max, norm_max, s->d_bq, st));
     }
     const cqs::ScanArgs a = scan_args(x, d_q, nb, kp + 1u, d_keep, mode, threshold, i8 ? sizeof(int8_t) : sizeof(uint16_t), true, nullptr, nullptr);
-    const ShadowRows rows{i8 ? nullptr : s->d_bf16, i8 ? s->d_i8 : nullptr, s->d_i8_scale, s->d_bq};
+    const ShadowRows rows{i8 ? nullptr : s->d_bf16, i8 ? s->d_i8 : nullptr, s->d_i8_scale, s->d_bq, s->d_hist};
     const int32_t rc = scan_select(x, a, st, &rows, nullptr, nullptr);
+    hipError_t e = hipSuccess;
     if (rc == CQS_HIP_OK)
-        HIP_TRY(x, cqs::launch_rescore_certify(a, (uint32_t)x->row_base, k, kp, bound_first ? 0u : (i8 ? 2u : 1u), r_max, norm_max,
-                                               s->d_bq, s->d_tickets, s->d_ekeys, out_keys, out_counts, cert,
-                                               device_gate ? s->d_stats + kStatCounts : nullptr,
-                                               device_gate && i8 ? s->d_stats + kStatI8Counts : nullptr, st));
+        e = cqs::launch_rescore_certify(a, (uint32_t)x->row_base, k, kp, bound_first ? 0u : (i8 ? 2u : 1u), r_max, norm_max,
+                                        s->d_bq, s->d_tickets, s->d_ekeys, s->d_hist, s->d_ccnt, s->d_cand, out_keys, out_counts,
+                                        cert, device_gate ? s->d_stats + kStatCounts : nullptr,
+                                        device_gate && i8 ? s->d_stats + kStatI8Counts : nullptr, st);
+    if (rc != CQS_HIP_OK || e != hipSuccess)
+        (void)hipMemsetAsync(s->d_hist, 0, (size_t)cqs::kShadowMaxQ * cqs::kHistBins * sizeof(uint32_t), st);
+    HIP_TRY(x, e);
     return rc;
 }
 
@@ -405,6 +419,18 @@
     return CQS_HIP_OK;
 } CQS_ABI_CATCH(x)
 
+int32_t cqs_hip_debug_shadow_listed(cqs_hip_index* x, uint32_t b, uint32_t* out) CQS_ABI_TRY {
+    if (!x || x->sh || !out || b == 0) return CQS_HIP_ERR_INVALID;
+    std::lock_guard<std::mutex> g(x->mu);
+    const Shadow* s = x->shadow;
+    if (!s || b > cqs::kShadowMaxQ) return CQS_HIP_ERR_INVALID;
+    HIP_TRY(x, hipSetDevice(x->device));
+    HIP_TRY(x, quiesce(x));
+    HIP_TRY(x, hipMemcpyAsync(out, s->d_ccnt + cqs::kShadowMaxQ, (size_t)b * sizeof(uint32_t), hipMemcpyDeviceToHost, x->stream));
+    HIP_TRY(x, hipStreamSynchronize(x->stream));
+    return CQS_HIP_OK;
+} CQS_ABI_CATCH(x)
+
 int32_t cqs_hip_debug_shadow_stats(cqs_hip_index* x, double* out) CQS_ABI_TRY {
     if (!x || x->sh || !out) return CQS_HIP_ERR_INVALID;
     std::lock_guard<std::mutex> g(x->mu);
@@ -464,8 +490,8 @@
         HIP_TRY(x, cqs::launch_scan(a, st));
     } else {
         const cqs::ScanArgs a = scan_args(x, x->d_q, b, k_scan, d_keep, mode, threshold, i8 ? sizeof(int8_t) : sizeof(uint16_t), true, nullptr, nullptr);
-        if (i8) HIP_TRY(x, cqs::launch_scan_i8(a, s->d_i8, s->d_i8_scale, s->d_bq, st));
-        else HIP_TRY(x, cqs::launch_scan_bf16(a, s->d_bf16, s->d_bq, st));
+        if (i8) HIP_TRY(x, cqs::launch_scan_i8(a, s->d_i8, s->d_i8_scale, s->d_bq, nullptr, st));
+        else HIP_TRY(x, cqs::launch_scan_bf16(a, s->d_bf16, s->d_bq, nullptr, st));
     }
     HIP_TRY(x, hipMemsetAsync(x->d_work, 0, cqs::kWorkWords * sizeof(uint32_t), st));
     const size_t row_b = (size_t)x->n * sizeof(float);
diff --git a/cqs_amd/csrc/scan_bf16.h b/cqs_amd/csrc/scan_bf16.h
--- a/cqs_amd/csrc/scan_bf16.h
+++ b/cqs_amd/csrc/scan_bf16.h
@@ -15,6 +15,7 @@
 constexpr uint32_t kShadowMaxQ = 32;
 constexpr uint32_t kShadowMaxDim = 2048;
 constexpr uint32_t kShadowKMax = 1024;
+constexpr uint32_t kTailCandCap = 2048;
 
 inline uint32_t shadow_kprime(uint32_t k) {
     const uint32_t kp = 2u * k + 32u;
@@ -56,12 +57,12 @@
 hipError_t launch_shadow_bound(const float* q, uint32_t b, uint32_t dim, double r_max, double norm_max, float* bq,
                                hipStream_t st);
 
-hipError_t launch_scan_bf16(const ScanArgs& a, const uint16_t* shadow, const float* bq, hipStream_t st);
+hipError_t launch_scan_bf16(const ScanArgs& a, const uint16_t* shadow, const float* bq, uint32_t* hist, hipStream_t st);
 
 hipError_t launch_rescore_certify(const ScanArgs& a, uint32_t row_base, uint32_t k, uint32_t kprime, uint32_t bound,
                                   double r_max, double norm_max, float* bq, uint32_t* tickets, uint64_t* ekeys,
-                                  uint64_t* out_keys, uint32_t* out_counts, uint32_t* cert, unsigned long long* counters,
-                                  unsigned long long* counters2, hipStream_t st);
+                                  uint32_t* hist, uint32_t* ccnt, uint64_t* cand, uint64_t* out_keys, uint32_t* out_counts,
+                                  uint32_t* cert, unsigned long long* counters, unsigned long long* counters2, hipStream_t st);
 #endif
 
 }
diff --git a/cqs_amd/csrc/scan_bf16.hip b/cqs_amd/csrc/scan_bf16.hip
--- a/cqs_amd/csrc/scan_bf16.hip
+++ b/cqs_amd/csrc/scan_bf16.hip
@@ -101,6 +101,8 @@
     float* gmax;
     uint64_t* gaux;
     const float* bq;
+    uint32_t* hist;
+    uint32_t bins;
 };
 
 template <int NCH, int BQ, int RI, bool NT, bool FULL>
@@ -200,6 +202,9 @@
             if ((uint32_t)lane < trows && row < p.n_pad) p.scores[(size_t)b * p.n_pad + row] = s;
             const float gm = wave_max64(s);
             if (lane == 0) p.gmax[(size_t)b * n_tasks + cur] = gm;
+            if (lane == 0 && p.hist && gm != -INFINITY)
+                (void)__hip_atomic_fetch_add(p.hist + (size_t)b * kHistBins + bin_of(gm, p.bins != 0u), 1u, __ATOMIC_RELAXED,
+                                             __HIP_MEMORY_SCOPE_AGENT);
             if (p.gaux) {
                 const uint32_t arg = (uint32_t)__builtin_ctzll(__ballot(s == gm));
                 const float sec = wave_max64(((uint32_t)lane == arg) ? -INFINITY : s);
@@ -253,7 +258,7 @@
 #endif
 
 template <int NCH, int BQ, int RI>
-static hipError_t launch_bf16(const ScanArgs& a, const uint16_t* shadow, const float* bq, uint32_t q0, uint32_t nq,
+static hipError_t launch_bf16(const ScanArgs& a, const uint16_t* shadow, const float* bq, uint32_t* hist, uint32_t q0, uint32_t nq,
                               uint32_t work_slot, hipStream_t st) {
     Bf16ScanParams p;
     p.rows = shadow; p.n = a.n; p.n_pad = a.n_pad; p.dim = a.dim;
@@ -267,6 +272,8 @@
     p.gmax = a.gmax + (size_t)q0 * p.n_tasks;
     p.gaux = a.gaux ? a.gaux + (size_t)q0 * p.n_tasks : nullptr;
     p.bq = bq + q0;
+    p.hist = (hist && !a.range_bins) ? hist + (size_t)q0 * kHistBins : nullptr;
+    p.bins = a.linear_bins ? 1u : 0u;
     const bool one_shot = p.n_tasks <= a.n_cu * 4u * CQS_BF16_ONE_SHOT;
     const uint32_t wpb = 4u;
     const uint32_t blocks = one_shot ? (p.n_tasks + wpb - 1u) / wpb : a.n_cu * CQS_BF16_BLOCKS_PER_CU;
@@ -283,20 +290,20 @@
 }
 
 template <int NCH>
-static hipError_t launch_bf16_groups(const ScanArgs& a, const uint16_t* shadow, const float* bq, hipStream_t st) {
+static hipError_t launch_bf16_groups(const ScanArgs& a, const uint16_t* shadow, const float* bq, uint32_t* hist, hipStream_t st) {
     uint32_t done = 0, slot = 0;
     while (done < a.b) {
         const uint32_t left = a.b - done;
         hipError_t e;
         uint32_t g;
         if constexpr (NCH <= 2) {
-            if (left >= 5) { g = left < 8u ? left : 8u; e = launch_bf16<NCH, 8, 2>(a, shadow, bq, done, g, slot, st); }
-            else if (left >= 4) { g = 4; e = launch_bf16<NCH, 4, 4>(a, shadow, bq, done, g, slot, st); }
-            else if (left >= 2) { g = 2; e = launch_bf16<NCH, 2, 8>(a, shadow, bq, done, g, slot, st); }
-            else { g = 1; e = launch_bf16<NCH, 1, 16>(a, shadow, bq, done, g, slot, st); }
+            if (left >= 5) { g = left < 8u ? left : 8u; e = launch_bf16<NCH, 8, 2>(a, shadow, bq, hist, done, g, slot, st); }
+            else if (left >= 4) { g = 4; e = launch_bf16<NCH, 4, 4>(a, shadow, bq, hist, done, g, slot, st); }
+            else if (left >= 2) { g = 2; e = launch_bf16<NCH, 2, 8>(a, shadow, bq, hist, done, g, slot, st); }
+            else { g = 1; e = launch_bf16<NCH, 1, 16>(a, shadow, bq, hist, done, g, slot, st); }
         } else {
-            if (left >= 2) { g = 2; e = launch_bf16<NCH, 2, 4>(a, shadow, bq, done, g, slot, st); }
-            else { g = 1; e = launch_bf16<NCH, 1, 8>(a, shadow, bq, done, g, slot, st); }
+            if (left >= 2) { g = 2; e = launch_bf16<NCH, 2, 4>(a, shadow, bq, hist, done, g, slot, st); }
+            else { g = 1; e = launch_bf16<NCH, 1, 8>(a, shadow, bq, hist, done, g, slot, st); }
         }
         if (e != hipSuccess) return e;
         done += g;
@@ -305,14 +312,14 @@
     return hipSuccess;
 }
 
-hipError_t launch_scan_bf16(const ScanArgs& a, const uint16_t* shadow, const float* bq, hipStream_t st) {
+hipError_t launch_scan_bf16(const ScanArgs& a, const uint16_t* shadow, const float* bq, uint32_t* hist, hipStream_t st) {
     if (a.b == 0 || a.n == 0) return hipSuccess;
     if (a.b > kShadowMaxQ || a.dim % 8u != 0u || a.dim > kShadowMaxDim) return hipErrorInvalidValue;
     switch ((a.dim + 511u) / 512u) {
-        case 1: return launch_bf16_groups<1>(a, shadow, bq, st);
-        case 2: return launch_bf16_groups<2>(a, shadow, bq, st);
-        case 3: return launch_bf16_groups<3>(a, shadow, bq, st);
-        case 4: return launch_bf16_groups<4>(a, shadow, bq, st);
+        case 1: return launch_bf16_groups<1>(a, shadow, bq, hist, st);
+        case 2: return launch_bf16_groups<2>(a, shadow, bq, hist, st);
+        case 3: return launch_bf16_groups<3>(a, shadow, bq, hist, st);
+        case 4: return launch_bf16_groups<4>(a, shadow, bq, hist, st);
         default: return hipErrorInvalidValue;
     }
 }
@@ -339,78 +346,205 @@
     uint32_t* cert;
     unsigned long long* counters;
     unsigned long long* counters2;
+    uint32_t* hist;
+    uint32_t* ccnt;
+    uint64_t* cand;
 };
 
 constexpr uint32_t kTailWaves = 16;
+
+template <int NCH>
+__device__ __forceinline__ uint64_t rescore_key(const float* rows, uint32_t row_base, uint32_t dim, uint32_t mode, float thr,
+                                                const float* qp, uint64_t key, uint32_t lane) {
+    const uint32_t grow = 0xFFFFFFFFu - (uint32_t)key;
+    const float* rp = rows + (size_t)(grow - row_base) * dim;
+    f4 x[NCH], qv[NCH];
+#pragma unroll
+    for (int c = 0; c < NCH; ++c) {
+        const uint32_t idx = (uint32_t)c * 256u + lane * 4u;
+        const bool in = idx < dim;
+        const uint32_t off = in ? idx : dim - 4u;
+        x[c] = *(const f4*)(rp + off);
+        const f4 v = *(const f4*)(qp + off);
+        qv[c] = in ? v : (f4)(0.f);
+    }
+    f2 acc2 = (f2)(0.f);
+#pragma unroll
+    for (int c = 0; c < NCH; ++c) {
+        const f2 xlo = __builtin_shufflevector(x[c], x[c], 0, 1);
+        const f2 xhi = __builtin_shufflevector(x[c], x[c], 2, 3);
+        acc2 = __builtin_elementwise_fma(xlo, __builtin_shufflevector(qv[c], qv[c], 0, 1), acc2);
+        acc2 = __builtin_elementwise_fma(xhi, __builtin_shufflevector(qv[c], qv[c], 2, 3), acc2);
+    }
+    float s = acc2.x + acc2.y;
+#pragma unroll
+    for (int m = 32; m >= 1; m >>= 1) s += __shfl_xor(s, m, 64);
+    bool keep = __builtin_fabsf(s) <= 3.4028234664e38f;
+    if (keep && mode == 1u) {
+        s = s < 0.f ? 0.f : (s > 1.f ? 1.f : s);
+        keep = s >= thr;
+    }
+    return keep ? pack_key(okey(s), grow) : 0ull;
+}
+
+__device__ __forceinline__ void rank_sort_pairs(const uint64_t* a, const uint64_t* e, uint32_t count, uint64_t* sa,
+                                                uint64_t* se, uint32_t* ok, uint32_t* s_flag) {
+    __syncthreads();
+    const uint32_t cpad = (count + 3u) & ~3u;
+    const uint32_t i0 = threadIdx.x, i1 = threadIdx.x + 1024u;
+    for (uint32_t i = threadIdx.x; i < cpad; i += 1024u) ok[i] = i < count ? (uint32_t)(a[i] >> 32) : 0u;
+    if (i0 < count) sa[i0] = 0ull;
+    if (i1 < count) sa[i1] = 0ull;
+    if (threadIdx.x == 0) s_flag[0] = 0u;
+    __syncthreads();
+    if (i0 < count) {
+        const bool two = i1 < count;
+        const uint64_t m0 = a[i0], m1 = two ? a[i1] : ~0ull;
+        const uint32_t h0 = (uint32_t)(m0 >> 32), h1 = (uint32_t)(m1 >> 32);
+        uint32_t r0 = 0, r1 = 0;
+#pragma unroll 8
+        for (uint32_t j = 0; j < cpad; j += 4u) {
+            const uint4 o = *reinterpret_cast<const uint4*>(&ok[j]);
+            r0 += (o.x > h0) ? 1u : 0u; r1 += (o.x > h1) ? 1u : 0u;
+            r0 += (o.y > h0) ? 1u : 0u; r1 += (o.y > h1) ? 1u : 0u;
+            r0 += (o.z > h0) ? 1u : 0u; r1 += (o.z > h1) ? 1u : 0u;
+            r0 += (o.w > h0) ? 1u : 0u; r1 += (o.w > h1) ? 1u : 0u;
+        }
+        sa[r0] = m0; se[r0] = e[i0];
+        if (two) { sa[r1] = m1; se[r1] = e[i1]; }
+    }
+    __syncthreads();
+    if ((i0 < count && sa[i0] == 0ull) || (i1 < count && sa[i1] == 0ull)) s_flag[0] = 1u;
+    __syncthreads();
+    if (s_flag[0] != 0u) {
+        for (uint32_t i = threadIdx.x; i < count; i += 1024u) {
+            const uint64_t mine = a[i];
+            uint32_t rank = 0;
+            for (uint32_t j = 0; j < count; ++j) rank += (a[j] > mine) ? 1u : 0u;
+            sa[rank] = mine; se[rank] = e[i];
+        }
+        __syncthreads();
+    }
+}
 
 template <int NCH>
 __global__ __launch_bounds__(1024) void rescore_certify_kernel(const TailParams p) {
     __shared__ uint64_t s_keys[kShadowKMax];
     __shared__ uint64_t s_sorted[kShadowKMax];
     __shared__ __attribute__((aligned(16))) uint32_t s_ok[kShadowKMax + 4];
-    __shared__ uint32_t s_cnt, s_flag, s_last;
+    __shared__ uint32_t s_cnt, s_flag, s_last, s_ng, s_nc, s_base;
+    const SelectLds lds = select_lds();
     const uint32_t lane = threadIdx.x & 63u;
     const uint32_t qi = blockIdx.y;
-    const uint32_t wave = (uint32_t)__builtin_amdgcn_readfirstlane((int)(blockIdx.x * kTailWaves + (threadIdx.x >> 6)));
-    const uint32_t n_waves = gridDim.x * kTailWaves;
+    const uint32_t wv = (uint32_t)__builtin_amdgcn_readfirstlane((int)(threadIdx.x >> 6));
     const uint32_t dim = p.dim;
     const float* qp = p.q + (size_t)qi * dim;
-    if (threadIdx.x == 0) s_cnt = 0u;
+    if (threadIdx.x == 0) { s_cnt = 0u; s_ng = 0u; s_nc = 0u; }
     if (qi == 0u && blockIdx.x == 0u)
         for (uint32_t i = threadIdx.x; i < kWorkWords; i += 1024u) p.work[i] = 0u;
 
-    const uint32_t n_tasks = p.tiers.total();
-    uint32_t found;
-    const uint64_t* akeys = select_body(p.scores + (size_t)qi * p.n_pad, p.gmax + (size_t)qi * n_tasks,
-                                        p.gaux ? p.gaux + (size_t)qi * n_tasks : nullptr, p.n_pad, p.tiers, p.kprime + 1u,
-                                        p.row_base, p.bins, nullptr, found);
-    const uint32_t ac = found < p.kprime + 1u ? found : p.kprime + 1u;
-    const uint32_t nc = ac < p.kprime ? ac : p.kprime;
-    const uint64_t key_next = ac > p.kprime ? akeys[p.kprime] : 0ull;
-
-    for (uint32_t slot = wave; slot <= nc; slot += n_waves) {
-        if (slot == 0u) {
+    const TaskTiers tiers = p.tiers;
+    const uint32_t n_tasks = tiers.total();
+    const uint32_t kk = p.kprime + 1u;
+    const float* const srow = p.scores + (size_t)qi * p.n_pad;
+    const float* const gm = p.gmax + (size_t)qi * n_tasks;
+    const uint64_t* const ga = p.gaux ? p.gaux + (size_t)qi * n_tasks : nullptr;
+
+    bool dist = false;
+    uint32_t T = 0;
+    if (p.hist) {
+        reinterpret_cast<uint4*>(lds.hist)[threadIdx.x] = reinterpret_cast<const uint4*>(p.hist + (size_t)qi * kHistBins)[threadIdx.x];
+        __syncthreads();
+        block_decide<1024>(lds.hist, kk, lds.part, lds.res);
+        dist = lds.res[3] >= kk;
+        T = lds.res[0];
+    }
+    __syncthreads();
+
+    uint32_t ac = 0, nc = 0;
+    uint64_t key_next = 0ull;
+    if (dist) {
+        const bool linear = p.bins != 0u;
+        const uint32_t per = (n_tasks + gridDim.x - 1u) / gridDim.x;
+        const uint32_t t_lo = blockIdx.x * per < n_tasks ? blockIdx.x * per : n_tasks;
+        const uint32_t t_hi = n_tasks - t_lo < per ? n_tasks : t_lo + per;
+        for (uint32_t t = t_lo + threadIdx.x; t < t_hi; t += 1024u) {
+            const float v = gm[t];
+            if (v != -INFINITY && bin_of(v, linear) >= T) {
+                const uint32_t slot = atomicAdd(&s_ng, 1u);
+                if (slot < kGroupCap) lds.groups[slot] = t;
+            }
+        }
+        __syncthreads();
+        const uint32_t ng = s_ng;
+        bool over = ng > kGroupCap;
+        if (!over) {
+            for (uint32_t g = wv; g < ng; g += kTailWaves) {
+                uint32_t grows;
+                const uint32_t gbase = tiers.locate((uint32_t)__builtin_amdgcn_readfirstlane((int)lds.groups[g]), grows);
+                const bool in = lane < grows;
+                const uint32_t idx = gbase + (in ? lane : 0u);
+                const float v = srow[idx];
+                const bool take = in && v != -INFINITY && bin_of(v, linear) >= T;
+                const uint64_t mask = __ballot(take);
+                if (mask) {
+                    uint32_t base = 0;
+                    if (lane == 0u) base = atomicAdd(&s_nc, (uint32_t)__popcll(mask));
+                    base = (uint32_t)__builtin_amdgcn_readfirstlane((int)base);
+                    const uint32_t slot = base + __builtin_amdgcn_mbcnt_hi((uint32_t)(mask >> 32), __builtin_amdgcn_mbcnt_lo((uint32_t)mask, 0u));
+                    if (take && slot < kTailCandCap) lds.keys[slot] = pack_key(okey(v), p.row_base + idx);
+                }
+            }
+        }
+        __syncthreads();
+        const uint32_t ncl = s_nc;
+        over = over || ncl > kTailCandCap;
+        if (threadIdx.x == 0)
+            s_base = __hip_atomic_fetch_add(p.ccnt + qi, over ? kTailCandCap + 1u : ncl, __ATOMIC_RELAXED, __HIP_MEMORY_SCOPE_AGENT);
+        __syncthreads();
+        const uint32_t base = s_base;
+        uint32_t first = wv;
+        if (blockIdx.x == 0u && wv == kTailWaves - 1u) {
             if (p.bound != 0u) {
                 const float v = p.bound == 2u ? wave_i8_bound(qp, dim, p.r_max, p.norm_max, lane)
                                               : wave_shadow_bound(qp, dim, p.r_max, p.norm_max, lane);
                 if (lane == 0u)
                     __hip_atomic_store((uint32_t*)p.bq + qi, __float_as_uint(v), __ATOMIC_RELAXED, __HIP_MEMORY_SCOPE_AGENT);
             }
-            continue;
-        }
-        const uint32_t i = slot - 1u;
-        const uint64_t key = akeys[i];
-        const uint32_t grow = 0xFFFFFFFFu - (uint32_t)key;
-        const float* rp = p.rows + (size_t)(grow - p.row_base) * dim;
-        f4 x[NCH], qv[NCH];
-#pragma unroll
-        for (int c = 0; c < NCH; ++c) {
-            const uint32_t idx = (uint32_t)c * 256u + lane * 4u;
-            const bool in = idx < dim;
-            const uint32_t off = in ? idx : dim - 4u;
-            x[c] = *(const f4*)(rp + off);
-            const f4 v = *(const f4*)(qp + off);
-            qv[c] = in ? v : (f4)(0.f);
-        }
-        f2 acc2 = (f2)(0.f);
-#pragma unroll
-        for (int c = 0; c < NCH; ++c) {
-            const f2 xlo = __builtin_shufflevector(x[c], x[c], 0, 1);
-            const f2 xhi = __builtin_shufflevector(x[c], x[c], 2, 3);
-            acc2 = __builtin_elementwise_fma(xlo, __builtin_shufflevector(qv[c], qv[c], 0, 1), acc2);
-            acc2 = __builtin_elementwise_fma(xhi, __builtin_shufflevector(qv[c], qv[c], 2, 3), acc2);
-        }
-        float s = acc2.x + acc2.y;
-#pragma unroll
-        for (int m = 32; m >= 1; m >>= 1) s += __shfl_xor(s, m, 64);
-        bool keep = __builtin_fabsf(s) <= 3.4028234664e38f;
-        if (keep && p.mode == 1u) {
-            s = s < 0.f ? 0.f : (s > 1.f ? 1.f : s);
-            keep = s >= p.thr;
-        }
-        if (lane == 0u)
-            __hip_atomic_store(p.ekeys + (size_t)qi * p.kprime + i, keep ? pack_key(okey(s), grow) : 0ull, __ATOMIC_RELAXED,
-                               __HIP_MEMORY_SCOPE_AGENT);
+        }
+        if (over || base + ncl > kTailCandCap) first = ncl;
+        for (uint32_t i = first; i < ncl; i += kTailWaves) {
+            const uint64_t key = lds.keys[i];
+            const uint64_t ek = rescore_key<NCH>(p.rows, p.row_base, dim, p.mode, p.thr, qp, key, lane);
+            if (lane == 0u) {
+                uint64_t* const dst = p.cand + ((size_t)qi * kTailCandCap + base + i) * 2u;
+                __hip_atomic_store(dst, key, __ATOMIC_RELAXED, __HIP_MEMORY_SCOPE_AGENT);
+                __hip_atomic_store(dst + 1, ek, __ATOMIC_RELAXED, __HIP_MEMORY_SCOPE_AGENT);
+            }
+        }
+    } else {
+        const uint32_t wave = blockIdx.x * kTailWaves + wv;
+        const uint32_t n_waves = gridDim.x * kTailWaves;
+        uint32_t found;
+        const uint64_t* akeys = select_body(srow, gm, ga, p.n_pad, tiers, kk, p.row_base, p.bins, nullptr, found);
+        ac = found < kk ? found : kk;
+        nc = ac < p.kprime ? ac : p.kprime;
+        key_next = ac > p.kprime ? akeys[p.kprime] : 0ull;
+        for (uint32_t slot = wave; slot <= nc; slot += n_waves) {
+            if (slot == 0u) {
+                if (p.bound != 0u) {
+                    const float v = p.bound == 2u ? wave_i8_bound(qp, dim, p.r_max, p.norm_max, lane)
+                                                  : wave_shadow_bound(qp, dim, p.r_max, p.norm_max, lane);
+                    if (lane == 0u)
+                        __hip_atomic_store((uint32_t*)p.bq + qi, __float_as_uint(v), __ATOMIC_RELAXED, __HIP_MEMORY_SCOPE_AGENT);
+                }
+                continue;
+            }
+            const uint32_t i = slot - 1u;
+            const uint64_t ek = rescore_key<NCH>(p.rows, p.row_base, dim, p.mode, p.thr, qp, akeys[i], lane);
+            if (lane == 0u)
+                __hip_atomic_store(p.ekeys + (size_t)qi * p.kprime + i, ek, __ATOMIC_RELAXED, __HIP_MEMORY_SCOPE_AGENT);
+        }
     }
     asm volatile("s_waitcnt vmcnt(0)" ::: "memory");
     __syncthreads();
@@ -419,13 +553,43 @@
         const bool last = t == gridDim.x - 1u;
         if (last) __hip_atomic_store(p.tickets + qi, 0u, __ATOMIC_RELAXED, __HIP_MEMORY_SCOPE_AGENT);
         s_last = last ? 1u : 0u;
+        if (last && dist) s_base = __hip_atomic_load(p.ccnt + qi, __ATOMIC_RELAXED, __HIP_MEMORY_SCOPE_AGENT);
     }
     __syncthreads();
     if (s_last == 0u) return;
 
-    if (threadIdx.x < nc) {
-        const uint64_t key = __hip_atomic_load(p.ekeys + (size_t)qi * p.kprime + threadIdx.x, __ATOMIC_RELAXED, __HIP_MEMORY_SCOPE_AGENT);
-        if (key != 0ull) s_keys[atomicAdd(&s_cnt, 1u)] = key;
+    uint32_t listed = 0;
+    if (!dist) {
+        if (threadIdx.x < nc) {
+            const uint64_t key = __hip_atomic_load(p.ekeys + (size_t)qi * p.kprime + threadIdx.x, __ATOMIC_RELAXED, __HIP_MEMORY_SCOPE_AGENT);
+            if (key != 0ull) s_keys[atomicAdd(&s_cnt, 1u)] = key;
+        }
+    } else if ((listed = s_base) <= kTailCandCap) {
+        uint64_t* const a = lds.keys;
+        uint64_t* const e = lds.keys + kTailCandCap;
+        uint64_t* const sa = lds.keys + 2u * kTailCandCap;
+        uint64_t* const se = lds.keys + 3u * kTailCandCap;
+        __syncthreads();
+        for (uint32_t i = threadIdx.x; i < listed; i += 1024u) {
+            const uint64_t* const src = p.cand + ((size_t)qi * kTailCandCap + i) * 2u;
+            a[i] = __hip_atomic_load(src, __ATOMIC_RELAXED, __HIP_MEMORY_SCOPE_AGENT);
+            e[i] = __hip_atomic_load(src + 1, __ATOMIC_RELAXED, __HIP_MEMORY_SCOPE_AGENT);
+        }
+        rank_sort_pairs(a, e, listed, sa, se, lds.hist, &s_flag);
+        ac = listed < kk ? listed : kk;
+        nc = ac < p.kprime ? ac : p.kprime;
+        key_next = ac > p.kprime ? sa[p.kprime] : 0ull;
+        if (threadIdx.x < nc && se[threadIdx.x] != 0ull) s_keys[atomicAdd(&s_cnt, 1u)] = se[threadIdx.x];
+    } else {
+        uint32_t found;
+        const uint64_t* akeys = select_body(srow, gm, ga, p.n_pad, tiers, kk, p.row_base, p.bins, nullptr, found);
+        ac = found < kk ? found : kk;
+        nc = ac < p.kprime ? ac : p.kprime;
+        key_next = ac > p.kprime ? akeys[p.kprime] : 0ull;
+        for (uint32_t i = wv; i < nc; i += kTailWaves) {
+            const uint64_t ek = rescore_key<NCH>(p.rows, p.row_base, dim, p.mode, p.thr, qp, akeys[i], lane);
+            if (lane == 0u && ek != 0ull) s_keys[atomicAdd(&s_cnt, 1u)] = ek;
+        }
     }
     __syncthreads();
     const uint32_t m = s_cnt;
@@ -433,6 +597,13 @@
     const uint32_t k = p.k;
     const uint32_t outc = m < k ? m : k;
     for (uint32_t i = threadIdx.x; i < k; i += 1024u) p.out_keys[(size_t)qi * k + i] = (i < outc) ? s_sorted[i] : 0ull;
+    if (p.hist) {
+        reinterpret_cast<uint4*>(p.hist + (size_t)qi * kHistBins)[threadIdx.x] = uint4{0u, 0u, 0u, 0u};
+        if (threadIdx.x == 0) {
+            __hip_atomic_store(p.ccnt + qi, 0u, __ATOMIC_RELAXED, __HIP_MEMORY_SCOPE_AGENT);
+            p.ccnt[kShadowMaxQ + qi] = dist ? listed : 0xFFFFFFFFu;
+        }
+    }
     if (threadIdx.x == 0) {
         p.out_counts[qi] = outc;
         const float bq = __uint_as_float(__hip_atomic_load((uint32_t*)p.bq + qi, __ATOMIC_RELAXED, __HIP_MEMORY_SCOPE_AGENT));
@@ -454,20 +625,26 @@
 #ifndef CQS_TAIL_MAX_BLOCKS_PER_CU
 #define CQS_TAIL_MAX_BLOCKS_PER_CU 1u
 #endif
+#ifndef CQS_TAIL_SLICE
+#define CQS_TAIL_SLICE 1024u
+#endif
 
 hipError_t launch_rescore_certify(const ScanArgs& a, uint32_t row_base, uint32_t k, uint32_t kprime, uint32_t bound,
                                   double r_max, double norm_max, float* bq, uint32_t* tickets, uint64_t* ekeys,
-                                  uint64_t* out_keys, uint32_t* out_counts, uint32_t* cert, unsigned long long* counters,
-                                  unsigned long long* counters2, hipStream_t st) {
+                                  uint32_t* hist, uint32_t* ccnt, uint64_t* cand, uint64_t* out_keys, uint32_t* out_counts,
+                                  uint32_t* cert, unsigned long long* counters, unsigned long long* counters2, hipStream_t st) {
     const uint32_t b = a.b, dim = a.dim;
     if (b == 0) return hipSuccess;
     if (b > kShadowMaxQ || k == 0 || kprime < k || kprime >= kShadowKMax || a.k != kprime + 1u || dim % 8u != 0u ||
-        dim > kShadowMaxDim || bound > 2u)
+        dim > kShadowMaxDim || bound > 2u || (hist && (!ccnt || !cand)))
         return hipErrorInvalidValue;
     const TailParams tp{a.rows, a.q, dim, k, kprime, a.mode, row_base, a.threshold, a.scores, a.gmax, a.gaux, a.n_pad, a.tiers,
                         a.range_bins ? 2u : (a.linear_bins ? 1u : 0u), a.work, ekeys, bq, tickets, bound, r_max, norm_max,
-                        out_keys, out_counts, cert, counters, counters2};
-    const uint32_t want = (kprime + 1u + kTailWaves - 1u) / kTailWaves;
+                        out_keys, out_counts, cert, counters, counters2, a.range_bins ? nullptr : hist, ccnt, cand};
+    const uint32_t n_tasks = a.tiers.total();
+    uint32_t want = (kprime + 1u + kTailWaves - 1u) / kTailWaves;
+    const uint32_t slices = (n_tasks + CQS_TAIL_SLICE - 1u) / CQS_TAIL_SLICE;
+    if (tp.hist && n_tasks > kprime && slices > want) want = slices;
     uint32_t cap = a.n_cu * CQS_TAIL_MAX_BLOCKS_PER_CU / b;
     if (cap < 1u) cap = 1u;
     const dim3 grid(want < cap ? want : cap, b), block(64u * kTailWaves);
diff --git a/cqs_amd/csrc/scan_device.h b/cqs_amd/csrc/scan_device.h
--- a/cqs_amd/csrc/scan_device.h
+++ b/cqs_amd/csrc/scan_device.h
@@ -12,6 +12,24 @@
 
 __device__ __forceinline__ uint64_t pack_key(uint32_t ok, uint32_t global_row) {
     return ((uint64_t)ok << 32) | (uint64_t)(0xFFFFFFFFu - global_row);
+}
+
+__device__ __forceinline__ uint32_t bin_of(float s, bool linear) {
+    if (linear) {
+        const float t = (s + 1.0f) * 2048.0f;
+        const int b = (int)t;
+        return (uint32_t)(b < 0 ? 0 : (b > 4095 ? 4095 : b));
+    }
+    return okey(s) >> 20;
+}
+__device__ __forceinline__ uint32_t bin_of_range(float s, float lo, float scale) {
+    if (!(scale > 0.f)) return 0u;
+    const float t = (s - lo) * scale;
+    if (!(t < 4095.0f)) return 4095u;
+    return t > 0.f ? (uint32_t)(int)t : 0u;
+}
+__device__ __forceinline__ uint32_t bin_any(float s, uint32_t mode, float lo, float scale) {
+    return mode == 2u ? bin_of_range(s, lo, scale) : bin_of(s, mode != 0u);
 }
 
 template <int N, int M, int NV>
diff --git a/cqs_amd/csrc/scan_i8.h b/cqs_amd/csrc/scan_i8.h
--- a/cqs_amd/csrc/scan_i8.h
+++ b/cqs_amd/csrc/scan_i8.h
@@ -29,7 +29,7 @@
 
 hipError_t launch_i8_bound(const float* q, uint32_t b, uint32_t dim, double r_max, double norm_max, float* bq, hipStream_t st);
 
-hipError_t launch_scan_i8(const ScanArgs& a, const int8_t* codes, const float* scales, const float* bq, hipStream_t st);
+hipError_t launch_scan_i8(const ScanArgs& a, const int8_t* codes, const float* scales, const float* bq, uint32_t* hist, hipStream_t st);
 #endif
 
 }
diff --git a/cqs_amd/csrc/scan_i8.hip b/cqs_amd/csrc/scan_i8.hip
--- a/cqs_amd/csrc/scan_i8.hip
+++ b/cqs_amd/csrc/scan_i8.hip
@@ -114,6 +114,8 @@
     float* gmax;
     uint64_t* gaux;
     const float* bq;
+    uint32_t* hist;
+    uint32_t bins;
 };
 
 template <int NCH, int BQ, int RI, bool NT, bool FULL>
@@ -211,6 +213,9 @@
             if ((uint32_t)lane < trows && row < p.n_pad) p.scores[(size_t)b * p.n_pad + row] = s;
             const float gm = wave_max64(s);
             if (lane == 0) p.gmax[(size_t)b * n_tasks + cur] = gm;
+            if (lane == 0 && p.hist && gm != -INFINITY)
+                (void)__hip_atomic_fetch_add(p.hist + (size_t)b * kHistBins + bin_of(gm, p.bins != 0u), 1u, __ATOMIC_RELAXED,
+                                             __HIP_MEMORY_SCOPE_AGENT);
             if (p.gaux) {
                 const uint32_t arg = (uint32_t)__builtin_ctzll(__ballot(s == gm));
                 const float sec = wave_max64(((uint32_t)lane == arg) ? -INFINITY : s);
@@ -255,7 +260,7 @@
 constexpr int kI8RowsPerBatch = 16;
 
 template <int NCH, int BQ, int RI>
-static hipError_t launch_i8(const ScanArgs& a, const int8_t* codes, const float* scales, const float* bq, uint32_t q0,
+static hipError_t launch_i8(const ScanArgs& a, const int8_t* codes, const float* scales, const float* bq, uint32_t* hist, uint32_t q0,
                             uint32_t nq, hipStream_t st) {
     I8ScanParams p;
     p.rows = codes; p.scales = scales; p.n = a.n; p.n_pad = a.n_pad; p.dim = a.dim;
@@ -268,6 +273,8 @@
     p.gmax = a.gmax + (size_t)q0 * p.n_tasks;
     p.gaux = a.gaux ? a.gaux + (size_t)q0 * p.n_tasks : nullptr;
     p.bq = bq + q0;
+    p.hist = (hist && !a.range_bins) ? hist + (size_t)q0 * kHistBins : nullptr;
+    p.bins = a.linear_bins ? 1u : 0u;
     const uint32_t wpb = 4u;
     const dim3 grid((p.n_tasks + wpb - 1u) / wpb), block(64u * wpb);
     const bool full = (a.dim == (uint32_t)NCH * 1024u);
@@ -282,27 +289,27 @@
 }
 
 template <int NCH>
-static hipError_t launch_i8_groups(const ScanArgs& a, const int8_t* codes, const float* scales, const float* bq, hipStream_t st) {
+static hipError_t launch_i8_groups(const ScanArgs& a, const int8_t* codes, const float* scales, const float* bq, uint32_t* hist, hipStream_t st) {
     uint32_t done = 0;
     while (done < a.b) {
         const uint32_t left = a.b - done;
         hipError_t e;
         uint32_t g;
-        if (left >= 3) { g = left < 4u ? left : 4u; e = launch_i8<NCH, 4, 4>(a, codes, scales, bq, done, g, st); }
-        else if (left >= 2) { g = 2; e = launch_i8<NCH, 2, 8>(a, codes, scales, bq, done, g, st); }
-        else { g = 1; e = launch_i8<NCH, 1, kI8RowsPerBatch>(a, codes, scales, bq, done, g, st); }
+        if (left >= 3) { g = left < 4u ? left : 4u; e = launch_i8<NCH, 4, 4>(a, codes, scales, bq, hist, done, g, st); }
+        else if (left >= 2) { g = 2; e = launch_i8<NCH, 2, 8>(a, codes, scales, bq, hist, done, g, st); }
+        else { g = 1; e = launch_i8<NCH, 1, kI8RowsPerBatch>(a, codes, scales, bq, hist, done, g, st); }
         if (e != hipSuccess) return e;
         done += g;
     }
     return hipSuccess;
 }
 
-hipError_t launch_scan_i8(const ScanArgs& a, const int8_t* codes, const float* scales, const float* bq, hipStream_t st) {
+hipError_t launch_scan_i8(const ScanArgs& a, const int8_t* codes, const float* scales, const float* bq, uint32_t* hist, hipStream_t st) {
     if (a.b == 0 || a.n == 0) return hipSuccess;
     if (a.b > kShadowMaxQ || !i8_dim_ok(a.dim)) return hipErrorInvalidValue;
     switch ((a.dim + 1023u) / 1024u) {
-        case 1: return launch_i8_groups<1>(a, codes, scales, bq, st);
-        case 2: return launch_i8_groups<2>(a, codes, scales, bq, st);
+        case 1: return launch_i8_groups<1>(a, codes, scales, bq, hist, st);
+        case 2: return launch_i8_groups<2>(a, codes, scales, bq, hist, st);
         default: return hipErrorInvalidValue;
     }
 }
diff --git a/cqs_amd/csrc/scan_kernels.h b/cqs_amd/csrc/scan_kernels.h
--- a/cqs_amd/csrc/scan_kernels.h
+++ b/cqs_amd/csrc/scan_kernels.h
@@ -17,7 +17,7 @@
 struct TaskTiers {
     uint32_t nA, nB, nC;
     __host__ __device__ uint32_t total() const { return nA + nB + nC; }
-    __host__ __device__ uint32_t locate(uint32_t t, uint32_t& rows) const {
+    __host__ __device__ __attribute__((always_inline)) uint32_t locate(uint32_t t, uint32_t& rows) const {
         if (t < nA) { rows = 64u; return t * 64u; }
         if (t < nA + nB) { rows = 32u; return nA * 64u + (t - nA) * 32u; }
         rows = 16u;
diff --git a/cqs_amd/csrc/select_device.h b/cqs_amd/csrc/select_device.h
--- a/cqs_amd/csrc/select_device.h
+++ b/cqs_amd/csrc/select_device.h
@@ -8,26 +8,9 @@
 
 namespace cqs {
 
-__device__ __forceinline__ uint32_t bin_of(float s, bool linear) {
-    if (linear) {
-        const float t = (s + 1.0f) * 2048.0f;
-        const int b = (int)t;
-        return (uint32_t)(b < 0 ? 0 : (b > 4095 ? 4095 : b));
-    }
-    return okey(s) >> 20;
-}
-__device__ __forceinline__ uint32_t bin_of_range(float s, float lo, float scale) {
-    if (!(scale > 0.f)) return 0u;
-    const float t = (s - lo) * scale;
-    if (!(t < 4095.0f)) return 4095u;
-    return t > 0.f ? (uint32_t)(int)t : 0u;
-}
-__device__ __forceinline__ uint32_t bin_any(float s, uint32_t mode, float lo, float scale) {
-    return mode == 2u ? bin_of_range(s, lo, scale) : bin_of(s, mode != 0u);
-}
 
 template <int THREADS>
-__device__ void block_decide(const uint32_t* hist, uint32_t k_rem, uint32_t* s_part ,
+__device__ __forceinline__ void block_decide(const uint32_t* hist, uint32_t k_rem, uint32_t* s_part ,
                              uint32_t* res ) {
     constexpr int BPT = kHistBins / THREADS;
     constexpr int NW = THREADS / 64;
@@ -120,16 +103,33 @@
 constexpr uint32_t kGroupCap = 8192;
 constexpr int kGB = 16;
 
+struct SelectLds {
+    uint64_t* keys;
+    uint32_t* groups;
+    uint32_t* hist;
+    uint32_t* part;
+    uint32_t* res;
+};
+__device__ __forceinline__ SelectLds select_lds() {
+    __shared__ uint64_t s_keys[kCandCap];
+    __shared__ uint32_t s_groups[kGroupCap];
+    __shared__ __attribute__((aligned(16))) uint32_t s_hist[kHistBins];
+    __shared__ uint32_t s_part[1024];
+    __shared__ uint32_t s_res[4];
+    return SelectLds{s_keys, s_groups, s_hist, s_part, s_res};
+}
+
 __device__ __forceinline__ const uint64_t* select_body(const float* __restrict__ s, const float* __restrict__ gm,
                                                        const uint64_t* __restrict__ ga, uint32_t n_pad,
                                                        const TaskTiers& tiers, uint32_t k, uint32_t row_base,
                                                        uint32_t linear, unsigned long long* __restrict__ dbg,
                                                        uint32_t& count_out) {
-    __shared__ uint64_t s_keys[kCandCap];
-    __shared__ uint32_t s_groups[kGroupCap];
-    __shared__ __attribute__((aligned(16))) uint32_t s_hist[kHistBins];
-    __shared__ uint32_t s_part[1024];
-    __shared__ uint32_t s_res[4];
+    const SelectLds lds = select_lds();
+    uint64_t* const s_keys = lds.keys;
+    uint32_t* const s_groups = lds.groups;
+    uint32_t* const s_hist = lds.hist;
+    uint32_t* const s_part = lds.part;
+    uint32_t* const s_res = lds.res;
     __shared__ uint32_t s_cnt, s_ng, s_ng2;
     const uint32_t n_tasks = tiers.total();
     const int lane = threadIdx.x & 63;
```
